# JuliaDiff/FiniteDiff.jl

Hardware: AMD Instinct MI355X
Metric: Jacobian columns/s (coloured sparse finite-difference Jacobian; headline config N=10^7 tridiagonal forward) (higher is better)
Workload: dtype f64; 1 GPU; N=10000000 tridiagonal CSC (nnz=3N-2), colorvec=mod1(i,3), forward, f!=second difference, x~U(0,1) seed 4; fdtype=forward, colors=3, parallelism=columns x1, output=nzval in HBM, eps_reduction=replicated, x_layout=replicated, gather_in_step=False

## Files before the change

### finitediff.jl_amd/csrc/fdjac_api.hip

```cpp
#include <algorithm>
#include <cmath>
#include <cstring>
#include <limits>
#include <new>

#include <atomic>
#include <thread>
#include <string>

#include "fdjac_internal.h"
#include "fdjac_eps_dev.h"

namespace fdjac {

#ifndef FDJAC_F32
static thread_local char g_err[512] = "";
#endif

int launch_eps(fd_plan *p, const real_t *x, double relstep, double absstep, double dir);
int launch_eps_groups(fd_plan *p, const real_t *x, int g0, int ng, bool final, double relstep, double absstep, double dir);
int launch_eps_final(fd_plan *p, double relstep, double absstep, double dir);
int launch_eps_flags(fd_plan *p, const real_t *x, const FusedEps &fz);
constexpr int kMaxEpsShards = kEpsGroups;
int launch_eps_perturb_small(fd_plan *p, const real_t *x, double relstep, double absstep, double dir, int pmode,
                             int base_row);
int launch_perturb(fd_plan *p, const real_t *x, int c_lo, int B);
int launch_decompress(fd_plan *p, const real_t *fx, int c_lo, int c_hi, real_t *const *outs, int mode);
int launch_fill(fd_ctx *ctx, real_t *ptr, int64_t n, real_t v);
int launch_scale(fd_ctx *ctx, real_t *dst, const real_t *src, int64_t n, real_t factor);
int launch_stream_copy(fd_ctx *ctx, const void *src, void *dst, int64_t n16);
int balanced_grid(int64_t tiles, int64_t cap);

static inline int64_t load_idx(const void *p, int bytes, int64_t i)
{
    return bytes == 8 ? ((const int64_t *)p)[i] : (int64_t)((const int32_t *)p)[i];
}

static inline int64_t round_up(int64_t v, int64_t m) { return (v + m - 1) / m * m; }

template <typename T> static int dev_upload(T **dst, const std::vector<T> &src)
{
    *dst = nullptr;
    if (src.empty()) return FD_OK;
    FD_HIP_CHECK(hipMalloc((void **)dst, sizeof(T) * src.size()));
    FD_HIP_CHECK(hipMemcpy(*dst, src.data(), sizeof(T) * src.size(), hipMemcpyHostToDevice));
    return FD_OK;
}

template <typename T> static int dev_alloc(T **dst, int64_t nelem)
{
    *dst = nullptr;
    if (nelem <= 0) nelem = 1;
    hipError_t e = hipMalloc((void **)dst, sizeof(T) * (size_t)nelem);
    if (e == hipErrorOutOfMemory) {
        set_error("hipMalloc of %lld bytes failed: out of memory", (long long)(nelem * (int64_t)sizeof(T)));
        return FD_ERR_NOMEM;
    }
    FD_HIP_CHECK(e);
    return FD_OK;
}

static int ingest_colors(fd_plan *p, const void *colorvec, int color_bytes, std::vector<int32_t> &col0)
{
    FD_REQUIRE(colorvec != nullptr, FD_ERR_ARG, "colorvec is NULL");
    FD_REQUIRE(color_bytes == 4 || color_bytes == 8, FD_ERR_ARG, "color_bytes must be 4 or 8");
    const int64_t N = p->N;
    col0.resize((size_t)N);
    int64_t C = 0;
    for (int64_t j = 0; j < N; ++j) {
        const int64_t c = load_idx(colorvec, color_bytes, j);
        if (c > C) C = c;
        FD_REQUIRE(c <= std::numeric_limits<int32_t>::max(), FD_ERR_ARG, "colour %lld too large", (long long)c);
        col0[(size_t)j] = c >= 1 ? (int32_t)(c - 1) : -1;
    }
    p->C = C;
    p->color8 = C <= 253;
    return FD_OK;
}

static int upload_colors(fd_plan *p, const std::vector<int32_t> &col0, const std::vector<int32_t> &nzc)
{
    if (p->color8) {
        std::vector<uint8_t> a(col0.size()), b(nzc.size());
        for (size_t i = 0; i < col0.size(); ++i) a[i] = col0[i] < 0 ? 0xFF : (uint8_t)col0[i];
        for (size_t i = 0; i < nzc.size(); ++i) b[i] = nzc[i] == -2 ? 0xFE : nzc[i] < 0 ? 0xFF : (uint8_t)nzc[i];
        uint8_t *d = nullptr;
        int rc = dev_upload(&d, a);
        if (rc) return rc;
        p->d_color = d;
        rc = dev_upload(&d, b);
        if (rc) return rc;
        p->d_nzcolor = d;
    } else {
        int32_t *d = nullptr;
        int rc = dev_upload(&d, col0);
        if (rc) return rc;
        p->d_color = d;
        rc = dev_upload(&d, nzc);
        if (rc) return rc;
        p->d_nzcolor = d;
    }
    return FD_OK;
}

static thread_local bool t_lowered_cx = false;
struct LoweredScope {
    LoweredScope() { t_lowered_cx = true; }
    ~LoweredScope() { t_lowered_cx = false; }
};
constexpr int32_t kPlanKnownFlags = FD_PLAN_EPS_CONTIGUOUS | FD_PLAN_COMPLEX_X | FD_PLAN_FINGERPRINT | FD_PLAN_STORE_CSC | FD_PLAN_STORE_CSC_ALWAYS | FD_PLAN_STORE_CSC_ROWS | FD_PLAN_HANDOVER_ROWS;

static int apply_opts(fd_plan *p, const fd_plan_opts *opts)
{
    FD_REQUIRE(opts != nullptr, FD_ERR_ARG, "opts is NULL");
    FD_REQUIRE(opts->fdtype == FD_FORWARD || opts->fdtype == FD_CENTRAL || opts->fdtype == FD_COMPLEX,
               FD_ERR_UNSUPPORTED,
               "Unrecognized fdtype: valid values are Val{:forward}, Val{:central} and Val{:complex}.");
    FD_REQUIRE((opts->flags & ~kPlanKnownFlags) == 0, FD_ERR_ARG, "unknown fd_plan_opts.flags bits 0x%x (zero the struct before filling it)",
               (unsigned)(opts->flags & ~kPlanKnownFlags));
    FD_REQUIRE(!(opts->flags & FD_PLAN_HANDOVER_ROWS) || (opts->flags & FD_PLAN_STORE_CSC_ROWS), FD_ERR_ARG,
               "fd_plan_opts.flags bits 0x%x: FD_PLAN_HANDOVER_ROWS needs FD_PLAN_STORE_CSC_ROWS (the row-wise hand-over kernel walks the plan's row lists)",
               (unsigned)opts->flags);
    FD_REQUIRE(!(opts->flags & FD_PLAN_COMPLEX_X), FD_ERR_UNSUPPORTED,
               "complex-valued x (FD_PLAN_COMPLEX_X) reaches this plan kind through its lowering only");
    p->fdtype = opts->fdtype;
    p->col0 = 0;
    p->col1 = p->N;
    if (!(opts->col_begin == 0 && opts->col_end == 0)) {
        FD_REQUIRE(opts->col_begin >= 0 && opts->col_begin <= opts->col_end && opts->col_end <= p->N, FD_ERR_ARG,
                   "column window [%lld,%lld) outside [0,%lld)", (long long)opts->col_begin,
                   (long long)opts->col_end, (long long)p->N);
        p->col0 = opts->col_begin;
        p->col1 = opts->col_end;
    }
    p->x0 = 0;
    p->x1 = p->N;
    if (!(opts->x_begin == 0 && opts->x_end == 0)) {
        FD_REQUIRE(opts->x_begin >= 0 && opts->x_begin <= opts->x_end && opts->x_end <= p->N, FD_ERR_ARG,
                   "x window [%lld,%lld) outside [0,%lld)", (long long)opts->x_begin, (long long)opts->x_end,
                   (long long)p->N);
        p->x0 = opts->x_begin;
        p->x1 = opts->x_end;
    }
    p->scratch_bytes = opts->scratch_bytes > 0 ? opts->scratch_bytes : ((int64_t)64 << 30);
    auto env_int = [](const char *name, int dflt) { const char *v = fdjac::test_switch(name); return (v && *v) ? atoi(v) : dflt; };
    p->small_ok = env_int("FDJAC_SMALL", 1) != 0;
    p->cx = t_lowered_cx;
    if (p->cx) p->small_ok = false;
    p->eps_nt = true;
    { const char *v = fdjac::test_switch("FDJAC_FUSED_MAX_N"); if (v && *v) p->fz_max_n = atoll(v); }
    p->fz_shared_ok = env_int("FDJAC_FUSED_SHARED", 0) != 0;
    p->fz_flags_ok = env_int("FDJAC_EPS_FLAGS", 1) != 0;
    p->lazy_diff = env_int("FDJAC_LAZY_DIFF", 1) != 0;
    p->bd_allowed = env_int("FDJAC_BAND_DESC", 1) != 0;
    p->store_allowed = env_int("FDJAC_LAZY_STORE", 1) != 0;
    p->want_store_csc = (opts->flags & FD_PLAN_STORE_CSC) != 0;
    p->want_store_rows = (opts->flags & FD_PLAN_STORE_CSC_ROWS) != 0;
    p->want_handover_rows = (opts->flags & FD_PLAN_HANDOVER_ROWS) != 0;
    p->store_csc_always = (opts->flags & FD_PLAN_STORE_CSC_ALWAYS) != 0;
    p->own_c0 = 0;
    p->own_c1 = -1;
    if (!(opts->color_begin == 0 && opts->color_end == 0)) {
        FD_REQUIRE(opts->color_begin >= 0 && opts->color_begin <= opts->color_end, FD_ERR_ARG,
                   "colour range [%lld,%lld) is not a range", (long long)opts->color_begin, (long long)opts->color_end);
        p->own_c0 = opts->color_begin;
        p->own_c1 = opts->color_end;
    }
    return FD_OK;
}

static int finish_fingerprint(int rc, fd_plan **out, const fd_plan_opts *opts, int idx_kind, const void *a, int64_t len_a, const void *b,
                              int64_t len_b, int idx_bytes, int idx_base, const void *colorvec, int color_bytes, int64_t len_color,
                              int memkind, int64_t N)
{
    if (rc || !opts || !(opts->flags & FD_PLAN_FINGERPRINT) || !out || !*out) return rc;
    fd_pattern_arrays src;
    memset(&src, 0, sizeof src);
    src.idx_a = a; src.len_a = len_a; src.idx_b = b; src.len_b = len_b; src.colorvec = colorvec; src.len_color = len_color;
    src.idx_bytes = idx_bytes ? idx_bytes : 8; src.idx_base = idx_base; src.color_bytes = color_bytes; src.memkind = memkind;
    const bool all = opts->col_begin == 0 && opts->col_end == 0;
    rc = plan_record_fingerprint(*out, idx_kind, &src, all ? 0 : opts->col_begin, all ? N : opts->col_end);
    if (rc) {
        fd_plan_destroy(*out);
        *out = nullptr;
    }
    return rc;
}

static int alloc_scratch(fd_plan *p, const std::vector<int32_t> &col0)
{
    p->cplx = p->fdtype == FD_COMPLEX ? 2 : 1;
    p->pts = p->fdtype == FD_CENTRAL ? 2 : 1;
    p->ldx = round_up(p->N, 32);
    p->ldf = round_up(p->M, 32);
    const int64_t per_color = (int64_t)p->pts * p->cplx * (int64_t)sizeof(real_t) * (p->ldx + p->ldf);
    int64_t B = p->C > 0 ? p->scratch_bytes / std::max<int64_t>(per_color, 1) : 1;
    B = std::max<int64_t>(1, std::min<int64_t>(B, std::max<int64_t>(p->C, 1)));
    B = std::min<int64_t>(B, 32768);
    p->chunkB = B;
    p->nchunks = p->C > 0 ? (p->C + B - 1) / B : 0;
    int rc;
    if ((rc = dev_alloc(&p->d_fx, p->ldf))) return rc;
    if ((rc = dev_alloc(&p->d_eps, std::max<int64_t>(p->C, 1)))) return rc;

    if (p->fdtype == FD_COMPLEX) {
        FD_HIP_CHECK(hipMemset(p->d_fx, 0, sizeof(real_t) * (size_t)p->ldf));
        p->d_zero = p->d_fx;
        FD_HIP_CHECK(hipStreamSynchronize(p->ctx->stream));
        int r2 = launch_fill(p->ctx, p->d_eps, std::max<int64_t>(p->C, 1), std::numeric_limits<real_t>::epsilon());
        if (r2) return r2;
    } else if (p->C > 0 && p->kind != K_DENSE) {
        if (p->C <= kRegColors) {
            if (!p->built_on_device) {
                const char *fc = fdjac::test_switch("FDJAC_EPS_CYCLIC");
                bool cyc = !(fc && *fc && atoi(fc) == 0) && p->N >= 1 && col0[0] >= 0;
                const int32_t sh = cyc ? col0[0] : 0;
                for (int64_t j = 0; j < p->N && cyc; ++j) cyc = col0[(size_t)j] == (int32_t)((j + sh) % p->C);
                p->cyc_C = cyc ? (int)p->C : 0;
                p->cyc_shift = cyc ? (int)sh : 0;
            }
            const int64_t tiles = (p->N + 2047) / 2048;
            const int64_t tpg = (tiles + kEpsGroups - 1) / kEpsGroups;
            const int64_t tpb = (tpg + kEpsBlocksPerGroup - 1) / kEpsBlocksPerGroup;
            FD_REQUIRE(tpg < ((int64_t)1 << 24), FD_ERR_UNSUPPORTED, "N too large for the step-size reduction's grid");
            p->eps_tpg = (int)tpg;
            p->eps_tpb = (int)tpb;
            p->eps_bpg = (int)((tpg + tpb - 1) / tpb);
            p->n_partial_blocks = kEpsGroups * p->eps_bpg;
            p->partial_cap = (int64_t)p->n_partial_blocks * kRegColors;
            if ((rc = dev_alloc(&p->d_partial, p->partial_cap))) return rc;
            if ((rc = dev_alloc(&p->d_gsum, (int64_t)2 * kEpsGroups * kRegColors))) return rc;
            if ((rc = dev_alloc(&p->d_tick, (int64_t)kEpsGroups + 1))) return rc;
            FD_HIP_CHECK(hipMemsetAsync(p->d_gsum, 0, sizeof(double) * 2 * kEpsGroups * kRegColors, p->ctx->stream));
            FD_HIP_CHECK(hipMemsetAsync(p->d_tick, 0, sizeof(unsigned) * (kEpsGroups + 1), p->ctx->stream));
        } else {
            std::vector<int64_t> cptr((size_t)p->C + 1, 0);
            for (int64_t j = 0; j < p->N; ++j)
                if (col0[(size_t)j] >= 0) cptr[(size_t)col0[(size_t)j] + 1]++;
            for (int64_t c = 0; c < p->C; ++c) cptr[(size_t)c + 1] += cptr[(size_t)c];
            std::vector<int32_t> perm((size_t)cptr[(size_t)p->C]);
            std::vector<int64_t> fillp(cptr.begin(), cptr.end() - 1);
            for (int64_t j = 0; j < p->N; ++j)
                if (col0[(size_t)j] >= 0) perm[(size_t)fillp[(size_t)col0[(size_t)j]]++] = (int32_t)j;
            if ((rc = dev_upload(&p->d_perm, perm))) return rc;
            if ((rc = dev_upload(&p->d_cptr, cptr))) return rc;
            int64_t chunks = (p->N / std::max<int64_t>(p->C, 1) + 511) / 512;
            p->seg_chunks = (int)std::max<int64_t>(1, std::min<int64_t>(chunks, 256));
            FD_REQUIRE((int64_t)p->C * p->seg_chunks < ((int64_t)1 << 31), FD_ERR_UNSUPPORTED, "too many colours");
            if ((rc = dev_alloc(&p->d_partial, (int64_t)p->seg_chunks * p->C))) return rc;
        }
    }
    return FD_OK;
}

static int ensure_values(fd_plan *p)
{
    if (p->d_FX) return FD_OK;
    return dev_alloc(&p->d_FX, (p->chunkB * p->pts + 1) * p->cplx * p->ldf);
}
static int ensure_points(fd_plan *p)
{
    if (p->d_X) return FD_OK;
    return dev_alloc(&p->d_X, (p->chunkB * p->pts + 1) * p->cplx * p->ldx);
}
static int ensure_stage(fd_plan *p, bool x, bool fin)
{
    int rc;
    if (x && !p->d_xstage && (rc = dev_alloc(&p->d_xstage, p->ldx))) return rc;
    if (fin && !p->d_finstage && (rc = dev_alloc(&p->d_finstage, p->ldf))) return rc;
    return FD_OK;
}

static int ensure_diff_scratch(fd_plan *p)
{
    int rc;
    if (!p->d_zero_own) {
        if ((rc = dev_alloc(&p->d_zero_own, p->ldf))) return rc;
        FD_HIP_CHECK(hipMemsetAsync(p->d_zero_own, 0, sizeof(real_t) * (size_t)p->ldf, p->ctx->stream));
        p->d_zero = p->d_zero_own;
    }
    if (p->fdtype == FD_CENTRAL && !p->d_eps2 && (rc = dev_alloc(&p->d_eps2, std::max<int64_t>(p->C, 1)))) return rc;
    return FD_OK;
}

static int new_plan(fd_ctx *ctx, int kind, int64_t M, int64_t N, fd_plan **out)
{
    FD_REQUIRE(ctx != nullptr && out != nullptr, FD_ERR_ARG, "ctx/out is NULL");
    FD_REQUIRE(M >= 0 && N >= 1, FD_ERR_SHAPE, "bad shape %lld x %lld", (long long)M, (long long)N);
    FD_REQUIRE(M < ((int64_t)1 << 31) && N < ((int64_t)1 << 31), FD_ERR_UNSUPPORTED,
               "dimensions >= 2^31 are not supported");
    FD_HIP_CHECK(hipSetDevice(ctx->device));
    fd_plan *p = new (std::nothrow) fd_plan();
    FD_REQUIRE(p != nullptr, FD_ERR_NOMEM, "out of host memory");
    p->ctx = ctx;
    p->kind = kind;
    p->M = M;
    p->N = N;
    *out = p;
    return FD_OK;
}

#define FD_TRY(expr)                 \
    do {                             \
        int _rc = (expr);            \
        if (_rc != FD_OK) {          \
// ... 24 lines not shown
int fd_ctx_create(int device, void *stream, fd_ctx **out)
{
    FD_REQUIRE(out != nullptr, FD_ERR_ARG, "out is NULL");
    *out = nullptr;
    int ndev = 0;
    hipError_t e = hipGetDeviceCount(&ndev);
    if (e != hipSuccess || ndev <= 0) {
        set_error("no HIP device available (%s)", e == hipSuccess ? "count = 0" : hipGetErrorString(e));
        return FD_ERR_NODEVICE;
    }
    FD_REQUIRE(device >= 0 && device < ndev, FD_ERR_ARG, "device %d out of range [0,%d)", device, ndev);
    FD_HIP_CHECK(hipSetDevice(device));
    hipDeviceProp_t prop;
    FD_HIP_CHECK(hipGetDeviceProperties(&prop, device));
    fd_ctx *c = new (std::nothrow) fd_ctx();
    FD_REQUIRE(c != nullptr, FD_ERR_NOMEM, "out of host memory");
    c->device = device;
    c->num_cus = prop.multiProcessorCount > 0 ? prop.multiProcessorCount : 256;
    if (stream == FD_STREAM_DEFAULT) {
        c->stream = nullptr;
        c->own_stream = false;
    } else if (stream) {
        c->stream = (hipStream_t)stream;
        c->own_stream = false;
    } else {
        hipError_t se = hipStreamCreateWithFlags(&c->stream, hipStreamNonBlocking);
        if (se != hipSuccess) {
            delete c;
            set_error("hipStreamCreate failed: %s", hipGetErrorString(se));
            return FD_ERR_HIP;
        }
        c->own_stream = true;
    }
    *out = c;
    return FD_OK;
}

int fd_ctx_destroy(fd_ctx *ctx)
{
    if (!ctx) return FD_OK;
    if (ctx->check_stream) { (void)hipStreamSynchronize(ctx->check_stream); (void)hipStreamDestroy(ctx->check_stream); }
    if (ctx->check_event) (void)hipEventDestroy(ctx->check_event);
    if (ctx->own_stream && ctx->stream) (void)hipStreamDestroy(ctx->stream);
    if (ctx->h_stale) (void)hipHostFree(ctx->h_stale);
    delete ctx;
    return FD_OK;
}

void *fd_ctx_stream(fd_ctx *ctx) { return ctx ? (void *)ctx->stream : nullptr; }

int fd_ctx_synchronize(fd_ctx *ctx)
{
    FD_REQUIRE(ctx != nullptr, FD_ERR_ARG, "ctx is NULL");
    FD_HIP_CHECK(hipStreamSynchronize(ctx->stream));
    if (ctx->check_stream) FD_HIP_CHECK(hipStreamSynchronize(ctx->check_stream));
    if (ctx->h_stale && *(volatile int *)ctx->h_stale) {
        *ctx->h_stale = 0;
        set_error("a deferred content check found that a plan no longer matches the caller's pattern / colour arrays (fd_plan_stale tells "
                  "which): results enqueued since that check are those of the old arrays");
        return FD_ERR_STALE;
    }
    return FD_OK;
}

#endif

int fd_plan_destroy(fd_plan *p)
{
    if (!p) return FD_OK;
    (void)hipSetDevice(p->ctx->device);
    (void)hipStreamSynchronize(p->ctx->stream);
    if (p->ctx->check_stream && p->d_fpx) (void)hipStreamSynchronize(p->ctx->check_stream);
    void *ptrs[] = {p->d_color, p->d_rowval, p->d_nzcolor, p->d_dest, p->d_spos, p->d_wtiles, p->d_wcode, p->d_w2desc, p->d_cr_rlo, p->d_cr_cnt, p->d_cr_off,
                    p->d_perm, p->d_cptr, p->d_X, p->d_FX, p->d_fx, p->d_eps, p->d_partial, p->d_gsum, p->d_tick, p->d_fpx, p->d_xstage,
                    p->d_finstage, p->d_outstage[0], p->d_outstage[1], p->d_outstage[2], p->d_zero_own, p->d_eps2, p->d_tile_order, p->d_fxwin, p->d_fp, p->d_sc_colptr, p->d_sc_rowval, p->d_sc_note, p->d_sr_ptr, p->d_sr_col, p->d_sr_slot, p->d_sr_order, p->d_sr_tile, p->d_sr_color, p->d_se_col, p->d_se_slot, p->d_se_info, p->d_split, p->d_bbb_off, p->d_bbb_blk, p->d_bbb_start, p->d_bbb_stride};
    for (void *q : ptrs)
        if (q) (void)hipFree(q);
    if (p->h_pstale) (void)hipHostFree(p->h_pstale);
    if (p->h_fz_err) (void)hipHostFree(p->h_fz_err);
    if (p->d_fz_part) (void)hipFree(p->d_fz_part);
    if (p->d_fz_eps) (void)hipFree(p->d_fz_eps);
    if (p->d_fz_trace) (void)hipFree(p->d_fz_trace);
    for (auto &sp : p->spans) {
        p->event_pool.push_back(sp.a);
        p->event_pool.push_back(sp.b);
    }
    for (hipEvent_t ev : p->event_pool) (void)hipEventDestroy(ev);
    delete p;
    return FD_OK;
}

#include "fdjac_plan_create.hip"

int fd_plan_row_lists(const fd_plan *p, const void **row_ptr_dev, const void **row_col_dev, const void **row_slot_dev, int64_t *entries, uint64_t *plan_serial)
{
    FD_REQUIRE(p != nullptr, FD_ERR_ARG, "plan is NULL");
    FD_REQUIRE(p->store_csc_ok && p->d_sr_ptr != nullptr, FD_ERR_UNSUPPORTED,
               "this plan keeps no row lists: create it with FD_PLAN_STORE_CSC | FD_PLAN_STORE_CSC_ROWS (a SparseMatrixCSC common-pattern plan that holds every column)");
    if (row_ptr_dev) *row_ptr_dev = p->d_sr_ptr;
    if (row_col_dev) *row_col_dev = p->d_sr_col;
    if (row_slot_dev) *row_slot_dev = p->d_sr_slot;
    if (entries) *entries = p->sc_entries;
    if (plan_serial) *plan_serial = p->sc_serial;
    return FD_OK;
}

int fd_plan_info(const fd_plan *p, int key, int64_t *value)
{
    FD_REQUIRE(p && value, FD_ERR_ARG, "NULL argument");
    switch (key) {
    case FD_INFO_M: *value = p->M; break;
    case FD_INFO_N: *value = p->N; break;
    case FD_INFO_NCOLORS: *value = p->C; break;
    case FD_INFO_NOUTS: *value = p->split_n ? p->split_n : p->nouts; break;
    case FD_INFO_OUT0_LEN: *value = p->split_n ? p->split_len[0] : p->out_len[0]; break;
    case FD_INFO_OUT1_LEN: *value = p->split_n ? p->split_len[1] : p->out_len[1]; break;
    case FD_INFO_OUT2_LEN: *value = p->split_n ? p->split_len[2] : p->out_len[2]; break;
    case FD_INFO_ROW_BEGIN: *value = p->row0; break;
    case FD_INFO_ROW_END: *value = p->row1; break;
    case FD_INFO_NCHUNKS: *value = p->nchunks; break;
    case FD_INFO_SCRATCH_BYTES:
        *value = (int64_t)sizeof(real_t) * (p->chunkB * p->pts * p->cplx * (p->ldx + p->ldf) + 2 * p->ldf + p->ldx);
        break;
    case FD_INFO_NNZ_LOCAL: *value = p->nnz_local; break;
    case FD_INFO_FCALLS_LAST: *value = p->fcalls_last; break;
    case FD_INFO_ENTRY_BEGIN: *value = p->entry_begin; break;
    case FD_INFO_SORTED_GATHER: *value = p->sorted_gather ? 1 : 0; break;
    case FD_INFO_LINES_DIRECT_X100: *value = (int64_t)(p->lines_direct * 100); break;
    case FD_INFO_LINES_SORTED_X100: *value = (int64_t)(p->lines_sorted * 100); break;
    case FD_INFO_WINDOW: *value = (p->window || p->tri_window) ? 1 : 0; break;
    case FD_INFO_WIN_OVERREAD_X100: *value = (int64_t)(p->win_overread * 100); break;
    case FD_INFO_WINDOW2D: *value = p->window2d ? 1 : 0; break;
    case FD_INFO_WIN_PERIOD: *value = p->win_per_P; break;
    case FD_INFO_COLRANGE_WG: *value = p->kind == K_COLRANGE ? 1 : 0; break;
    case FD_INFO_SMALL_FUSED:
        *value = (p->small_ok && p->N <= kSmallN && p->C > 0 && p->C <= kRegColors && p->kind != K_DENSE &&
                  p->fdtype != FD_COMPLEX) ? 1 : 0;
        break;
    case FD_INFO_EPS_CYCLIC: *value = p->cyc_C; break;
    case FD_INFO_EPS_NT: *value = !(store_active(p) || store_csc_active(p)) ? 1 : 0; break;
    case FD_INFO_BAND_DESC: *value = p->bd_t1 - p->bd_t0; break;
    case FD_INFO_LAZY_STORE:
        *value = (store_active(p) || store_csc_active(p)) ? 1 : 0;
        break;
    case FD_INFO_STORE_CSC:
        *value = p->store_csc_ok ? p->sc_entries : 0;
        break;
    case FD_INFO_STORE_LAUNCH: *value = p->store_launch; break;
    case FD_INFO_LAZY_DIFF:
        *value = (p->lazy_fn && (p->lazy_caps & FD_LAZY_CAP_DIFF) && p->lazy_diff && p->fdtype != FD_COMPLEX && p->kind != K_DENSE) ? 1 : 0;
        break;
    case FD_INFO_BUILT_ON_DEVICE: *value = p->built_on_device ? 1 : 0; break;
    case FD_INFO_HANDOVER_ROWS: *value = handover_rows_active(p) ? 1 : 0; break;
    default: set_error("unknown info key %d", key); return FD_ERR_ARG;
    }
    return FD_OK;
}

static hipEvent_t take_event(fd_plan *p)
{
    if (!p->event_pool.empty()) {
        hipEvent_t e = p->event_pool.back();
        p->event_pool.pop_back();
        return e;
    }
    hipEvent_t e = nullptr;
    (void)hipEventCreate(&e);
    return e;
}

struct Span {
    fd_plan *p;
    int idx = -1;
    Span(fd_plan *pl, int stage) : p(pl)
    {
        if (p->timing == 0) return;
        if (p->timing == 1 && stage != FD_STAGE_DECOMPRESS) return;
        if (p->timing == 1 && p->timing_stride > 1 && ((p->timing_calls - 1) % p->timing_stride) != 0) return;
        if (p->timing == 4 && stage == FD_STAGE_TOTAL) return;
        if (p->timing == 3 && stage != FD_STAGE_TOTAL) return;
        fdjac::TimedSpan s{stage, take_event(p), take_event(p)};
        (void)hipEventRecord(s.a, p->ctx->stream);
        p->spans.push_back(s);
        idx = (int)p->spans.size() - 1;
    }
    void stop()
    {
        if (idx >= 0) (void)hipEventRecord(p->spans[(size_t)idx].b, p->ctx->stream);
        idx = -1;
    }
    ~Span() { stop(); }
};

static constexpr size_t kMaxSpansInFlight = 4096;
static int collect_spans(fd_plan *p, bool blocking = true)
{
    if (p->spans.empty()) return FD_OK;
    if (!blocking && p->spans.size() >= kMaxSpansInFlight) blocking = true;
    if (blocking) FD_HIP_CHECK(hipStreamSynchronize(p->ctx->stream));
    size_t done = 0;
    for (auto &s : p->spans) {
        if (!blocking && hipEventQuery(s.b) != hipSuccess) {
            (void)hipGetLastError();
            break;
        }
        float ms = 0.f;
        if (hipEventElapsedTime(&ms, s.a, s.b) == hipSuccess) {
            p->ms_sum[s.stage] += ms;
            p->launches[s.stage] += 1;
            if (p->samples[s.stage].size() < 65536) p->samples[s.stage].push_back(ms);
        }
        p->event_pool.push_back(s.a);
        p->event_pool.push_back(s.b);
        ++done;
    }
    p->spans.erase(p->spans.begin(), p->spans.begin() + (ptrdiff_t)done);
    return FD_OK;
}

int fd_plan_enable_timing(fd_plan *p, int on)
{
    FD_REQUIRE(p, FD_ERR_ARG, "plan is NULL");
    int rc = collect_spans(p);
    if (rc) return rc;
    p->timing = on < 0 ? 0 : (on > 4 ? 4 : on);
    for (int i = 0; i < FD_NSTAGES; ++i) {
        p->ms_sum[i] = 0;
        p->launches[i] = 0;
        p->samples[i].clear();
    }
    return FD_OK;
}

int fd_plan_set_timing_stride(fd_plan *p, int stride)
{
    FD_REQUIRE(p && stride >= 1, FD_ERR_ARG, "bad argument");
    p->timing_stride = stride;
    p->timing_calls = 0;
    return FD_OK;
}

int fd_plan_get_timing_samples(fd_plan *p, int stage, double *ms_out, int64_t cap, int64_t *n_out)
{
    FD_REQUIRE(p && n_out && stage >= 0 && stage < FD_NSTAGES && (ms_out || cap == 0), FD_ERR_ARG, "bad argument");
    int rc = collect_spans(p);
    if (rc) return rc;
    const int64_t n = std::min<int64_t>((int64_t)p->samples[stage].size(), cap);
    for (int64_t k = 0; k < n; ++k) ms_out[k] = (double)p->samples[stage][(size_t)k];
    *n_out = (int64_t)p->samples[stage].size();
    return FD_OK;
}

int fd_plan_get_timings(fd_plan *p, double *ms_sum, int64_t *launches)
{
    FD_REQUIRE(p && ms_sum && launches, FD_ERR_ARG, "NULL argument");
    int rc = collect_spans(p);
    if (rc) return rc;
    for (int i = 0; i < FD_NSTAGES; ++i) {
        ms_sum[i] = p->ms_sum[i];
        launches[i] = p->launches[i];
    }
    return FD_OK;
}

static bool eps_shardable(const fd_plan *p)
{
    return p->fdtype != FD_COMPLEX && p->kind != K_DENSE && p->C > 0 && p->C <= kRegColors &&
           !(p->small_ok && p->N <= kSmallN) && p->d_partial != nullptr;
}

static void eps_shard_of(const fd_plan *p, int *W, int *r)
{
    if (p->p2p) { *W = fdjac_p2p_nranks(p->p2p); *r = fdjac_p2p_rank(p->p2p); }
    else { *W = fdjac_comm_nranks(p->comm); *r = fdjac_comm_rank(p->comm); }
}

static int eps_exchange(fd_plan *p, real_t *x_dev, int S, double relstep, double absstep, double dir)
{
    fd_p2p *mb = p->p2p ? p->p2p : (p->comm ? fdjac_comm_p2p(p->comm) : nullptr);
    if (mb && fdjac_p2p_nranks(mb) > 1) {
        fdjac_eps_final fin;
        fin.gsum = p->d_gsum; fin.ldp = kRegColors; fin.ngroups = kEpsGroups; fin.C = (int)p->C;
        fin.relstep = relstep; fin.absstep = absstep; fin.dir = dir; fin.is_forward = p->fdtype == FD_FORWARD ? 1 : 0;
        fin.eps = p->d_eps; fin.eps2 = p->d_eps2; fin.elem_bytes = (int)sizeof(real_t);
        const int rc = fdjac_p2p_step(mb, p->halo > 0 ? (void *)x_dev : nullptr, p->halo_own0, p->halo_own1, p->halo, (int)sizeof(real_t),
                                      p->d_gsum, (int64_t)S * kRegColors * (int64_t)sizeof(double), &fin);
        if (rc != FD_ERR_UNSUPPORTED) {
            if (!rc) p->eps2_fresh = p->d_eps2 != nullptr;
            return rc;
        }
    }
    int rc = FD_OK;
    if (p->comm) {
        if (p->halo > 0) rc = fd_comm_halo_exchange(p->comm, x_dev, p->halo_own0, p->halo_own1, p->halo, (int)sizeof(real_t));
        if (!rc) rc = fdjac_comm_allgather_f64(p->comm, p->d_gsum, (int64_t)S * kRegColors);
    }
    if (!rc) rc = launch_eps_final(p, relstep, absstep, dir);
    return rc;
}

static inline int call_f(const fd_plan *p, fd_f_launch f, void *fctx, void *fx, const void *x, int64_t nbatch, int64_t x_stride,
                         int64_t fx_stride, int64_t row_begin, int64_t row_end, int is_complex, void *stream)
{
    set_error("%s", "");
    if (!p->cx) return f(fctx, fx, x, nbatch, x_stride, fx_stride, row_begin, row_end, is_complex, stream);
    return f(fctx, fx, x, nbatch, x_stride / 2, fx_stride / 2, row_begin / 2, (row_end + 1) / 2, 1, stream);
}
#define FD_F_CHECK(rc)                                                                                                      \
    do {                                                                                                                    \
        if ((rc) != 0) {                                                                                                    \
            const std::string _why = fd_last_error();                                                                       \
            set_error("f! launcher returned %d%s%s", (int)(rc), _why.empty() ? "" : ": ", _why.c_str());                    \
            return FD_ERR_CALLBACK;                                                                                         \
        }                                                                                                                   \
    } while (0)

static int eps_sharded_classic(fd_plan *p, const real_t *x_dev, double relstep, double absstep, double dir)
{
    int W, r;
    eps_shard_of(p, &W, &r);
    const int S = (kEpsGroups + W - 1) / W;
    const int g0 = std::min(r * S, kEpsGroups), ng = std::min(S, kEpsGroups - g0);
    int rc = launch_eps_groups(p, x_dev, g0, ng, false, relstep, absstep, dir);
    if (!rc) {
        Span se(p, FD_STAGE_EXCHANGE);
        rc = eps_exchange(p, const_cast<real_t *>(x_dev), S, relstep, absstep, dir);
    }
    return rc;
}

static int fused_reset(fd_plan *p)
{
    const size_t np = 2 * (size_t)p->n_partial_blocks * kRegColors, ne = 2 * (size_t)kFzReplicas * kFzPitch;
    std::vector<unsigned long long> hp(np, kFzSentinel64);
    std::vector<rbits_t> he(ne, FzBits<real_t>::sentinel);
    FD_HIP_CHECK(hipStreamSynchronize(p->ctx->stream));
    FD_HIP_CHECK(hipMemcpy(p->d_fz_part, hp.data(), np * 8, hipMemcpyHostToDevice));
    FD_HIP_CHECK(hipMemcpy(p->d_fz_eps, he.data(), ne * sizeof(rbits_t), hipMemcpyHostToDevice));
    FD_HIP_CHECK(hipDeviceSynchronize());
    *p->h_fz_err = 0;
    p->fz_parity = 0;
    return FD_OK;
}
static int ensure_fused(fd_plan *p)
{
    if (p->d_fz_part) return FD_OK;
    FD_HIP_CHECK(hipHostMalloc((void **)&p->h_fz_err, sizeof(int), hipHostMallocMapped));
    *p->h_fz_err = 0;
    FD_HIP_CHECK(hipHostGetDevicePointer((void **)&p->d_fz_err, p->h_fz_err, 0));
    FD_HIP_CHECK(hipMalloc((void **)&p->d_fz_eps, 2 * (size_t)kFzReplicas * kFzPitch * sizeof(rbits_t)));
    FD_HIP_CHECK(hipMalloc((void **)&p->d_fz_part, 2 * (size_t)p->n_partial_blocks * kRegColors * sizeof(double)));
    { const char *v = fdjac::test_switch("FDJAC_FUSED_TRACE"); if (v && atoi(v) != 0) FD_HIP_CHECK(hipMalloc((void **)&p->d_fz_trace, 16 * sizeof(long long))); }
    return fused_reset(p);
}
static int64_t fused_timeout_ticks()
{
    const char *v = getenv("FDJAC_P2P_TIMEOUT_MS");
    const int64_t ms = (v && *v) ? atoll(v) : 2000;
    return (ms < 1 ? 1 : ms) * 100000;
}

static int jacobian_enqueue(fd_plan *p, fd_f_launch f, void *fctx, const real_t *x_dev, const real_t *fin_dev,
                            double relstep, double absstep, double dir, real_t *const *outs)
{
    fd_ctx *ctx = p->ctx;
    hipStream_t s = ctx->stream;
    FD_REQUIRE(f != nullptr, FD_ERR_ARG, "f launcher is NULL");
    if (!(relstep > 0)) {
        const real_t e = std::numeric_limits<real_t>::epsilon();
        relstep = p->fdtype == FD_FORWARD ? (double)std::sqrt(e) : p->fdtype == FD_CENTRAL ? (double)std::cbrt(e) : 1.0;
    }
    if (absstep < 0) absstep = relstep;
    p->relstep_last = relstep;
    p->absstep_last = absstep;
    p->fcalls_last = 0;
    if (collect_spans(p, false) != FD_OK) return FD_ERR_HIP;
    FD_REQUIRE(!(p->h_pstale && *(volatile int *)p->h_pstale), FD_ERR_STALE,
               "a deferred content check (fd_plan_matches_async) found that this plan no longer matches the caller's pattern / colour arrays");
    if (p->h_fz_err && *(volatile int *)p->h_fz_err) {
        const int what = *(volatile int *)p->h_fz_err;
        (void)fused_reset(p);
        FD_REQUIRE(false, FD_ERR_COMM, "the previous fused step of this plan timed out (%s never arrived; FDJAC_P2P_TIMEOUT_MS): its "
                   "output holds NaNs", what == 1 ? "a block sum of the step-size reduction" : "the step sizes");
    }
    {
        fd_p2p *mbq = p->p2p ? p->p2p : (p->comm ? fdjac_comm_p2p(p->comm) : nullptr);
        const int st = mbq ? fdjac_p2p_failed(mbq) : 0;
        FD_REQUIRE(st == 0, FD_ERR_COMM, "an earlier exchange through this plan's mailbox timed out (code %d: a peer's data never arrived; "
                   "fd_p2p_status / fd_comm_p2p_status; FDJAC_P2P_TIMEOUT_MS): step sizes and halo of that call are not to be trusted", st);
    }
    ++p->timing_calls;
    Span total(p, FD_STAGE_TOTAL);

    if (((uintptr_t)x_dev) & kPairMask) {
        { const int rc = ensure_stage(p, true, false); if (rc) return rc; }
        FD_HIP_CHECK(hipMemcpyAsync(p->d_xstage, x_dev, sizeof(real_t) * (size_t)p->N, hipMemcpyDeviceToDevice, s));
        x_dev = p->d_xstage;
    }

    const bool small_off = !p->small_ok;
    const bool full_colors = p->own_c0 == 0 && (p->own_c1 < 0 || p->own_c1 >= p->C);
    const bool small = !small_off && p->N <= kSmallN && p->C > 0 && p->C <= kRegColors && p->kind != K_DENSE &&
                       p->fdtype != FD_COMPLEX;
    const bool small_points = small && !p->lazy_fn && p->nchunks == 1 && full_colors;
    const bool base_in_batch = small_points && p->fdtype == FD_FORWARD && !fin_dev;
    p->fx_batch_row = nullptr;
    if (small_points) { int rc = ensure_points(p); if (!rc) rc = ensure_values(p); if (rc) return rc; }

    if (p->fdtype == FD_CENTRAL && p->lazy_fn && (p->lazy_caps & FD_LAZY_CAP_DIFF) && p->lazy_diff && p->kind != K_DENSE) {
        const int rc = ensure_diff_scratch(p);
        if (rc) return rc;
    }
    fd_p2p *fz_mb = p->p2p ? p->p2p : (p->comm ? fdjac_comm_p2p(p->comm) : nullptr);
    const bool shard_ctx = p->comm != nullptr || p->p2p != nullptr;
    bool fuse = !small && p->fdtype != FD_COMPLEX && p->C > 0 && p->C <= kRegColors && p->cyc_C > 0 && p->eps_mode == FD_EPS_COMPUTE &&
                p->lazy_fn && (p->lazy_caps & FD_LAZY_CAP_FUSED_EPS) && store_active(p) && p->store_ok &&
                (p->kind == K_CSC || p->kind == K_BANDED || p->kind == K_TRIDIAG) && p->nchunks == 1 && full_colors &&
                !(p->fdtype == FD_FORWARD && fin_dev) && p->d_partial != nullptr;
    if (shard_ctx && p->halo > 0) {
        int W = 1, r = 0;
        eps_shard_of(p, &W, &r);
        FD_REQUIRE(r == 0 || p->halo_own0 >= p->halo, FD_ERR_ARG, "no room for the lower halo: x[%lld - %lld, ...) starts before 0", (long long)p->halo_own0, (long long)p->halo);
        FD_REQUIRE(r + 1 >= W || p->halo_own1 + p->halo <= p->N, FD_ERR_ARG, "no room for the upper halo: x[..., %lld + %lld) ends behind N = %lld",
                   (long long)p->halo_own1, (long long)p->halo, (long long)p->N);
    }
    if (fuse) {
        hipStreamCaptureStatus cs = hipStreamCaptureStatusNone;
        if (hipStreamIsCapturing(s, &cs) != hipSuccess) { (void)hipGetLastError(); cs = hipStreamCaptureStatusNone; }
        if (cs != hipStreamCaptureStatusNone) fuse = false;
    }
    bool fuse_sharded = false;
    int fzW = 1, fzr = 0;
    if (fuse && shard_ctx) {
        if (fz_mb) { fzW = fdjac_p2p_nranks(fz_mb); fzr = fdjac_p2p_rank(fz_mb); }
        const bool halo_ok = p->halo == 0 || (p->halo == 2 && p->halo_own0 == p->col0 && p->halo_own1 == p->col1 && p->halo_own0 % 4 == 0 &&
                                              (p->halo_own1 % 4 == 0 || fzr == fzW - 1));
        fuse = fuse_sharded = fz_mb != nullptr && fzW > 1 && p->fz_sharded_ok && eps_shardable(p) && halo_ok &&
                              (int64_t)((kEpsGroups + fzW - 1) / fzW) * p->eps_tpg * 2048 <= p->fz_max_n &&
                              (!fdjac_p2p_shared_device(fz_mb) || p->fz_shared_ok);
    } else if (fuse) {
        fuse = p->N <= p->fz_max_n;
    }
    bool eps_flags = !fuse && p->fz_flags_ok && !small && !shard_ctx && p->fdtype != FD_COMPLEX && p->C > 0 && p->C <= kRegColors &&
                     p->kind != K_DENSE && p->eps_mode == FD_EPS_COMPUTE && p->d_partial != nullptr &&
                     p->n_partial_blocks == kEpsGroups * p->eps_bpg && p->n_partial_blocks <= kFzMaxBlocks;
    if (eps_flags) {
        hipStreamCaptureStatus cs = hipStreamCaptureStatusNone;
        if (hipStreamIsCapturing(s, &cs) != hipSuccess) { (void)hipGetLastError(); cs = hipStreamCaptureStatusNone; }
        if (cs != hipStreamCaptureStatusNone) eps_flags = false;
    }
    FusedEps fz_job;
    if (fuse || eps_flags) {
        const int rc = ensure_fused(p);
        if (rc) return rc;
        memset(&fz_job, 0, sizeof fz_job);
        fz_job.eg.tpg = p->eps_tpg; fz_job.eg.bpg = p->eps_bpg; fz_job.eg.tpb = p->eps_tpb; fz_job.eg.final_groups = kEpsGroups;
        fz_job.eg.C = (int)p->C; fz_job.eg.is_forward = p->fdtype == FD_FORWARD ? 1 : 0;
        fz_job.eg.relstep = relstep; fz_job.eg.absstep = absstep; fz_job.eg.dir = dir;
        fz_job.nranks = 1; fz_job.rank = 0; fz_job.g0 = 0; fz_job.ng = kEpsGroups;
        if (fuse_sharded) {
            const int S = (kEpsGroups + fzW - 1) / fzW;
            fz_job.nranks = fzW; fz_job.rank = fzr;
            fz_job.g0 = std::min(fzr * S, kEpsGroups); fz_job.ng = std::min(S, kEpsGroups - fz_job.g0);
            fdjac_p2p_fused mbv;
            const int rm = fdjac_p2p_fused_begin(fz_mb, &mbv);
            if (rm) return rm;
            fz_job.peer = mbv.peer; fz_job.local = mbv.local; fz_job.fz_off = mbv.fz_off; fz_job.buf = mbv.buf; fz_job.buf_reset = mbv.buf_reset;
            if (p->halo > 0) { fz_job.xw = const_cast<real_t *>(x_dev); fz_job.own_begin = p->halo_own0; fz_job.own_end = p->halo_own1; fz_job.halo = (int)p->halo; }
        }
        fz_job.nblocks = fz_job.ng * p->eps_bpg;
        fz_job.cyc_C = p->cyc_C; fz_job.cyc_shift = p->cyc_shift; fz_job.pair = p->cx ? 1 : 0;
        const size_t hp = (size_t)p->n_partial_blocks * kRegColors, he = (size_t)kFzReplicas * kFzPitch;
        fz_job.part = p->d_fz_part + (p->fz_parity ? hp : 0);
        fz_job.part_next = p->d_fz_part + (p->fz_parity ? 0 : hp);
        fz_job.epsr = (rbits_t *)p->d_fz_eps + (p->fz_parity ? he : 0);
        fz_job.epsr_next = (rbits_t *)p->d_fz_eps + (p->fz_parity ? 0 : he);
        fz_job.eps = p->d_eps; fz_job.eps2 = p->d_eps2;
        fz_job.err = fuse_sharded ? fdjac_p2p_err_word(fz_mb) : p->d_fz_err;
        fz_job.timeout_ticks = fused_timeout_ticks();
        fz_job.trace = p->d_fz_trace;
        if (p->d_fz_trace) {
            static const long long init[16] = {-1, 0, 0, 0, 0, -1, -1, 0, 0, 0, 0, 0, 0, 0, 0, 0};
            FD_HIP_CHECK(hipMemcpyAsync(p->d_fz_trace, init, sizeof init, hipMemcpyHostToDevice, s));
        }
    }
    if (p->eps_mode != FD_EPS_PRECOMPUTED) p->eps2_fresh = false;
    p->eps_nt = !(store_active(p) || store_csc_active(p));
    if (p->fdtype != FD_COMPLEX && p->C > 0 && p->eps_mode == FD_EPS_PRECOMPUTED) {
        FD_REQUIRE(!small_points, FD_ERR_UNSUPPORTED, "FD_EPS_PRECOMPUTED needs a plan whose reduction can be sharded");
    } else if (fuse) {
    } else if (eps_flags) {
        Span sp(p, FD_STAGE_EPS);
        const int rc = launch_eps_flags(p, x_dev, fz_job);
        if (rc) return rc;
        p->fz_parity ^= 1u;
    } else if (p->fdtype != FD_COMPLEX && p->C > 0) {
        Span sp(p, FD_STAGE_EPS);
        int rc;
        if (small) {
            rc = launch_eps_perturb_small(p, x_dev, relstep, absstep, dir, small_points ? p->fdtype : -1,
                                          base_in_batch ? (int)(p->C * p->pts) : -1);
        } else if ((p->comm || p->p2p) && eps_shardable(p)) {
            rc = eps_sharded_classic(p, x_dev, relstep, absstep, dir);
        } else {
            rc = launch_eps(p, x_dev, relstep, absstep, dir);
        }
        if (rc) return rc;
    }

    const real_t *fx = nullptr;
    bool base_pending = false;
    if (p->fdtype == FD_FORWARD) {
        if (fin_dev) {
            fx = fin_dev;
        } else if (base_in_batch) {
            fx = p->fx_batch_row = p->d_FX + (int64_t)p->C * p->pts * p->ldf;
        } else if (p->lazy_fn && p->nchunks > 0) {
            base_pending = true;
            fx = p->d_fx;
        } else {
            Span sp(p, FD_STAGE_F);
            const int rc = call_f(p, f, fctx, p->d_fx, x_dev, 1, p->N, p->ldf, p->row0, p->row1, 0, (void *)s);
            FD_F_CHECK(rc);
            p->fcalls_last += 1;
            fx = p->d_fx;
        }
    }

    if (p->kind == K_CSC_DENSE || p->kind == K_COO_DENSE || (p->kind == K_BBB && p->bbb_fill)) {
        FD_HIP_CHECK(hipMemsetAsync(outs[0], 0, sizeof(real_t) * (size_t)p->out_len[0], s));
    } else if (p->C == 0) {
        for (int k = 0; k < p->nouts; ++k)
            FD_HIP_CHECK(hipMemsetAsync(outs[k], 0, sizeof(real_t) * (size_t)p->out_len[k], s));
    }

    const int64_t oc0 = std::min<int64_t>(p->own_c0, p->C), oc1 = p->own_c1 < 0 ? p->C : std::min<int64_t>(p->own_c1, p->C);
    bool diff_base_counted = false;
    for (int64_t cl = oc0; cl < oc1; cl += p->chunkB) {
        const int c_lo = (int)cl;
        const int c_hi = (int)std::min<int64_t>(oc1, cl + p->chunkB);
        const int B = c_hi - c_lo;
        bool lazy_done = false, imag_only = false;
        bool want_diff = p->lazy_fn && (p->lazy_caps & FD_LAZY_CAP_DIFF) && p->lazy_diff && p->fdtype != FD_COMPLEX &&
                               !(p->fdtype == FD_FORWARD && !base_pending) && p->kind != K_DENSE;
        if (want_diff) { const int rc = ensure_diff_scratch(p); if (rc) return rc; }
        if (p->kind == K_BBB && store_active(p) && !(p->fdtype == FD_FORWARD && !base_pending)) {
            Span sp(p, FD_STAGE_DECOMPRESS);
            fd_bbb_store bb;
            memset(&bb, 0, sizeof bb);
            bb.out = outs[0]; bb.N = p->N; bb.nblk = p->bbb_nb; bb.block_size = p->bbb_bs;
            bb.bl = p->bbb_bl; bb.bu = p->bbb_bu; bb.lam = p->bbb_lam; bb.mu = p->bbb_mu;
            bb.start = (const long long *)p->d_bbb_start; bb.stride = (const long long *)p->d_bbb_stride;
            bb.color = p->d_color; bb.color_bytes = p->color8 ? 1 : 4; bb.C = (int)p->C; bb.elem_bytes = (int)sizeof(real_t);
            fd_lazy_points lp = {};
            lp.x = x_dev; lp.color = p->d_color; lp.eps = p->d_eps; lp.color_bytes = bb.color_bytes;
            lp.c_lo = c_lo; lp.ncolors = B; lp.pts = p->pts; lp.nparts = 1;
            lp.diff = (p->fdtype == FD_FORWARD && !diff_base_counted) ? 2 : 1;
            lp.store = &bb; lp.store_kind = FD_STORE_BBB;
            const int rc = p->lazy_fn(fctx, p->d_FX, &lp, p->ldf, p->row0, p->row1, (void *)s);
            FD_REQUIRE(rc == 0 || rc == FD_LAZY_DECLINED, FD_ERR_CALLBACK, "lazy f! launcher (BBB store) returned %d", rc);
            if (rc == 0) {
                p->fcalls_last += (int64_t)B * p->pts + (lp.diff == 2 ? 1 : 0);
                diff_base_counted = true;
                continue;
            }
        } else if (store_active(p) && !(p->fdtype == FD_FORWARD && !base_pending)) {
            Span sp(p, FD_STAGE_DECOMPRESS);
            fd_band_store bs;
            fd_stencil5_store s5;
            memset(&bs, 0, sizeof bs);
            memset(&s5, 0, sizeof s5);
            s5.out = outs[0];
            s5.nx = p->store5_nx; s5.ny = p->store5_ny; s5.entry_begin = p->entry_begin; s5.col_begin = p->col0; s5.col_end = p->col1;
            s5.color = p->d_color; s5.color_bytes = p->color8 ? 1 : 4; s5.C = (int)p->C; s5.elem_bytes = (int)sizeof(real_t);
            const bool stencil = !p->store_ok && p->store5_ok && p->kind == K_CSC;
            fd_colrange_store scr;
            memset(&scr, 0, sizeof scr);
            if (p->kind == K_COLRANGE) {
                scr.out = outs[0]; scr.M = p->M; scr.N = p->N; scr.col_begin = p->col0; scr.col_end = p->col1;
                scr.row_first = p->d_cr_rlo; scr.row_count = p->d_cr_cnt; scr.dest = (const long long *)p->d_cr_off;
                scr.color = p->d_color; scr.color_bytes = p->color8 ? 1 : 4; scr.C = (int)p->C; scr.elem_bytes = (int)sizeof(real_t);
                scr.pairs = p->cr_pairs ? 1 : 0; scr.nblk = p->cr_nblk; scr.block_size = p->cr_bs; scr.bl = p->cr_bl; scr.bu = p->cr_bu;
            }
            bs.M = p->M; bs.N = p->N; bs.entry_begin = p->entry_begin; bs.col_begin = p->col0; bs.col_end = p->col1;
            bs.l = p->store_l; bs.u = p->store_u; bs.C = p->store_C; bs.shift = p->store_shift;
            bs.elem_bytes = (int)sizeof(real_t);
            if (p->kind == K_TRIDIAG) {
                bs.layout = FD_BAND_TRIDIAGONAL;
                bs.out_dl = outs[0]; bs.out = outs[1]; bs.out_du = outs[2];
            } else {
                bs.layout = p->kind == K_BANDED ? FD_BAND_BANDED : FD_BAND_CSC;
                bs.out = outs[0];
            }
            fd_lazy_points lp = {};
            lp.x = x_dev;
            lp.color = p->d_color;
            lp.eps = p->d_eps;
            lp.color_bytes = p->color8 ? 1 : 4;
            lp.c_lo = c_lo;
            lp.ncolors = B;
            lp.pts = p->pts;
            lp.nparts = 1;
            lp.diff = p->fdtype == FD_COMPLEX ? 0 : ((p->fdtype == FD_FORWARD && !diff_base_counted) ? 2 : 1);
            lp.store = p->kind == K_COLRANGE ? (const void *)&scr : stencil ? (const void *)&s5 : (const void *)&bs;
            lp.store_kind = p->kind == K_COLRANGE ? FD_STORE_COLRANGE : stencil ? FD_STORE_STENCIL5 : FD_STORE_BAND;
            lp.is_complex = p->fdtype == FD_COMPLEX ? 1 : 0;
            lp.imag_only = lp.is_complex;
            lp.eps_job = fuse ? &fz_job : nullptr;
            int rc = p->lazy_fn(fctx, p->d_FX, &lp, p->ldf, p->row0, p->row1, (void *)s);
            if (fuse && rc == 0) {
                if (fuse_sharded) fdjac_p2p_fused_commit(fz_mb);
                p->fz_parity ^= 1u;
                p->eps2_fresh = p->d_eps2 != nullptr;
            } else if (fuse) {
                fuse = false;
                sp.stop();
                { Span se(p, FD_STAGE_EPS); const int re = fuse_sharded ? eps_sharded_classic(p, x_dev, relstep, absstep, dir) : launch_eps(p, x_dev, relstep, absstep, dir); if (re) return re; }
                Span sp2(p, FD_STAGE_DECOMPRESS);
                lp.eps_job = nullptr;
                if (rc == FD_LAZY_DECLINED) rc = p->lazy_fn(fctx, p->d_FX, &lp, p->ldf, p->row0, p->row1, (void *)s);
            }
            FD_REQUIRE(rc == 0 || rc == FD_LAZY_DECLINED, FD_ERR_CALLBACK, "lazy f! launcher (store) returned %d", rc);
            if (rc == 0) {
                p->fcalls_last += (int64_t)B * p->pts + (lp.diff == 2 ? 1 : 0);
                diff_base_counted = true;
                continue;
            }
        }
        if (store_csc_active(p)) {
            const bool own_base = base_pending && (p->lazy_caps & FD_LAZY_CAP_STORE_CSC_BASE) != 0;
            if (base_pending && !own_base) {
                Span sp(p, FD_STAGE_F);
                const int rc = call_f(p, f, fctx, p->d_fx, x_dev, 1, p->N, p->ldf, p->row0, p->row1, 0, (void *)s);
                FD_F_CHECK(rc);
                p->fcalls_last += 1;
                base_pending = false;
            }
            Span sp(p, FD_STAGE_DECOMPRESS);
            fd_csc_store sc;
            memset(&sc, 0, sizeof sc);
            sc.out = outs[0]; sc.M = p->M; sc.N = p->N; sc.col_begin = p->col0; sc.col_end = p->col1;
            sc.colptr = p->d_sc_colptr; sc.rowval = p->d_sc_rowval; sc.note = p->d_sc_note; sc.color = p->d_color; sc.fx_base = (p->fdtype == FD_FORWARD && !own_base) ? fx : nullptr;
            sc.color_bytes = p->color8 ? 1 : 4; sc.C = (int)p->C; sc.elem_bytes = (int)sizeof(real_t); sc.valid_coloring = p->sc_valid ? 1 : 0; sc.reach = p->sc_reach; sc.plan_serial = p->sc_serial;
            sc.row_ptr = p->d_sr_ptr; sc.row_col = p->d_sr_col; sc.row_slot = p->d_sr_slot; sc.row_pack = p->d_sr_order; sc.row_tile = p->d_sr_tile; sc.ent_col = p->d_se_col; sc.ent_slot = p->d_se_slot; sc.ent_info = p->d_se_info; sc.ent_tile_max = p->se_tile_max;
            fd_lazy_points lp = {};
            lp.x = x_dev;
            lp.color = p->d_color;
            lp.eps = p->d_eps;
            lp.color_bytes = sc.color_bytes;
            lp.c_lo = c_lo;
            lp.ncolors = B;
            lp.pts = p->pts;
            lp.nparts = 1;
            lp.diff = p->fdtype == FD_COMPLEX ? 0 : 1;
            lp.is_complex = p->fdtype == FD_COMPLEX ? 1 : 0;
            lp.imag_only = lp.is_complex;
            lp.store = &sc;
            lp.store_kind = FD_STORE_CSC;
            store_launch_note() = FD_STORE_LAUNCH_NONE;
            const int rc = p->lazy_fn(fctx, p->d_FX, &lp, p->ldf, p->row0, p->row1, (void *)s);
            FD_REQUIRE(rc == 0 || rc == FD_LAZY_DECLINED, FD_ERR_CALLBACK, "lazy f! launcher (column store) returned %d", rc);
            p->store_launch = rc == 0 ? store_launch_note() : FD_STORE_LAUNCH_NONE;
            if (rc == 0) {
                p->fcalls_last += (int64_t)B * p->pts + ((own_base && !diff_base_counted) ? 1 : 0);
                if (own_base) diff_base_counted = true;
                continue;
            }
            if (p->fdtype == FD_FORWARD && !own_base) want_diff = false;
        }
        if (fuse) {
            fuse = false;
            Span se(p, FD_STAGE_EPS);
            const int re = fuse_sharded ? eps_sharded_classic(p, x_dev, relstep, absstep, dir) : launch_eps(p, x_dev, relstep, absstep, dir);
            if (re) return re;
        }
        { const int rc = ensure_values(p); if (rc) return rc; }
        bool diff_done = false;
        if (p->lazy_fn) {
            Span sp(p, FD_STAGE_F);
            fd_lazy_points lp = {};
            lp.x = x_dev;
            lp.color = p->d_color;
            lp.eps = p->d_eps;
            lp.base_out = (base_pending && !want_diff) ? p->d_fx : nullptr;
            lp.diff = want_diff ? ((p->fdtype == FD_FORWARD && !diff_base_counted) ? 2 : 1) : 0;
            lp.store_kind = 0;
            lp.color_bytes = p->color8 ? 1 : 4;
            lp.c_lo = c_lo;
            lp.ncolors = B;
            lp.pts = p->pts;
            lp.is_complex = p->fdtype == FD_COMPLEX ? 1 : 0;
            lp.imag_only = (p->fdtype == FD_COMPLEX && (p->lazy_caps & FD_LAZY_CAP_IMAG_ONLY)) ? 1 : 0;
            lp.part = 0;
            lp.nparts = 1;
            imag_only = lp.imag_only != 0;
            const int rc = p->lazy_fn(fctx, p->d_FX, &lp, p->ldf, p->row0, p->row1, (void *)s);
            FD_REQUIRE(rc == 0 || rc == FD_LAZY_DECLINED, FD_ERR_CALLBACK, "lazy f! launcher returned %d", rc);
            if (rc == 0 && want_diff) {
                lazy_done = diff_done = true;
                p->fcalls_last += (int64_t)B * p->pts + (lp.diff == 2 ? 1 : 0);
                diff_base_counted = true;
            } else if (rc == 0) {
                lazy_done = true;
                p->fcalls_last += (int64_t)B * p->pts + (base_pending ? 1 : 0);
                base_pending = false;
            }
        }
        if (!lazy_done) {
            if (base_pending) {
                Span sp(p, FD_STAGE_F);
                const int rc = call_f(p, f, fctx, p->d_fx, x_dev, 1, p->N, p->ldf, p->row0, p->row1, 0, (void *)s);
                FD_F_CHECK(rc);
                p->fcalls_last += 1;
                base_pending = false;
            }
            { const int rc = ensure_points(p); if (rc) return rc; }
            if (!small_points) {
                Span sp(p, FD_STAGE_PERTURB);
                int rc = launch_perturb(p, x_dev, c_lo, B);
                if (rc) return rc;
            }
            Span sp(p, FD_STAGE_F);
            const int64_t npts = (int64_t)B * p->pts + (base_in_batch ? 1 : 0);
            const int rc = call_f(p, f, fctx, p->d_FX, p->d_X, npts, p->ldx, p->ldf, p->row0, p->row1,
                             p->fdtype == FD_COMPLEX ? 1 : 0, (void *)s);
            FD_F_CHECK(rc);
            p->fcalls_last += npts;
        }
        {
            Span sp(p, FD_STAGE_DECOMPRESS);
            const bool io = lazy_done && imag_only;
            int rc;
            if (diff_done) {
                real_t *eps_plain = p->d_eps;
                if (p->fdtype == FD_CENTRAL) {
                    if (!p->eps2_fresh && (rc = launch_scale(p->ctx, p->d_eps2 + c_lo, p->d_eps + c_lo, B, (real_t)2))) return rc;
                    p->d_eps = p->d_eps2;
                }
                rc = launch_decompress(p, p->d_zero, c_lo, c_hi, outs, (int)FD_FORWARD);
                p->d_eps = eps_plain;
            } else {
                rc = launch_decompress(p, io ? p->d_fx : fx, c_lo, c_hi, outs, io ? (int)FD_FORWARD : p->fdtype);
            }
            if (rc) return rc;
        }
    }
    return FD_OK;
}

static int jacobian_split(fd_plan *p, bool async, fd_f_launch f, void *fctx, const void *x, int x_kind, const void *f_in, int f_in_kind, double relstep,
                          double absstep, double dir, void *const *outs, int out_kind)
{
    for (int k = 0; k < p->split_n; ++k) FD_REQUIRE(outs[k] || p->split_len[k] == 0, FD_ERR_ARG, "outs[%d] is NULL", k);
    FD_HIP_CHECK(hipSetDevice(p->ctx->device));
    if (!p->d_split) { const int rc = dev_alloc(&p->d_split, p->out_len[0]); if (rc) return rc; }
    void *one[3] = {p->d_split, nullptr, nullptr};
    const int n = p->split_n;
    p->split_n = 0;
    const int rc = async ? fd_jacobian_async(p, f, fctx, x, f_in, relstep, absstep, dir, one)
                         : fd_jacobian(p, f, fctx, x, x_kind, f_in, f_in_kind, relstep, absstep, dir, one, FD_DEVICE);
    p->split_n = n;
    if (rc) return rc;
    int64_t off = 0;
    for (int k = 0; k < n; ++k) {
        if (p->split_len[k] > 0)
            FD_HIP_CHECK(hipMemcpyAsync(outs[k], p->d_split + off, sizeof(real_t) * (size_t)p->split_len[k],
                                        out_kind == FD_HOST ? hipMemcpyDeviceToHost : hipMemcpyDeviceToDevice, p->ctx->stream));
        off += p->split_len[k];
// ... 325 lines not shown
```

### finitediff.jl_amd/csrc/fdjac_eps_dev.h

```cpp
#pragma once
#include "fdjac_internal.h"
#include "fdjac_dotx.h"

namespace fdjac {

template <typename CT> __device__ __forceinline__ void load_color_pair(const CT *p, int &c0, int &c1);
template <> __device__ __forceinline__ void load_color_pair<uint8_t>(const uint8_t *p, int &c0, int &c1)
{
    const unsigned v = *reinterpret_cast<const uint16_t *>(p);
    c0 = (int)(v & 0xFF);
    c1 = (int)(v >> 8);
}
template <> __device__ __forceinline__ void load_color_pair<int32_t>(const int32_t *p, int &c0, int &c1)
{
    const int2 v = *reinterpret_cast<const int2 *>(p);
    c0 = v.x;
    c1 = v.y;
}

template <typename CT, bool CYC>
__device__ __forceinline__ int eps_color_of(const CT *__restrict__ color, int64_t i, int cyc_C, int cyc_shift, int pair)
{
    if (pair) i &= ~(int64_t)1;
    return CYC ? (int)((i + cyc_shift) % cyc_C) : (int)color[i];
}

template <typename CT, bool CYC>
__device__ __noinline__ double eps_rescan_norm_wave(const real_t *__restrict__ x, const CT *__restrict__ color, int64_t n, int cyc_C,
                                                       int cyc_shift, int pair, int cc, int k)
{
    const double sc = k < 0 ? 0x1p-600 : 0x1p600, unsc = k < 0 ? 0x1p600 : 0x1p-600;
    double acc = 0.0;
    for (int64_t i = threadIdx.x & 63; i < n; i += 64)
        if (eps_color_of<CT, CYC>(color, i, cyc_C, cyc_shift, pair) == cc) {
            const double v = (double)x[i] * sc;
            acc += v * v;
        }
    acc = wave_sum(acc);
    return sqrt(__shfl(acc, 0, 64)) * unsc;
}

constexpr int kEpsU = 4;

struct EpsGrid {
    int tpg, bpg, tpb;
    int final_groups;
    int C, is_forward;
    double relstep, absstep, dir;
};

template <typename CT, int NC, bool CYC, bool NT, bool PIPE = true>
__device__ __forceinline__ bool eps_block_sum(const real_t *__restrict__ x, const CT *__restrict__ color, int64_t n, int cyc_C, int cyc_shift,
                                              int gblock, const EpsGrid &eg, int pair, double (*red)[NC], double &s)
{
    const int grp = gblock / eg.bpg, kb = gblock - grp * eg.bpg;
    double acc[NC];
#pragma unroll
    for (int c = 0; c < NC; ++c) acc[c] = 0.0;

    const int64_t tile = (int64_t)kEpsU * kBlock * 2;
    const int64_t t0 = (int64_t)grp * eg.tpg + (int64_t)kb * eg.tpb;
    int64_t t1 = t0 + eg.tpb;
    if (t1 > (int64_t)(grp + 1) * eg.tpg) t1 = (int64_t)(grp + 1) * eg.tpg;
    const int64_t base0 = t0 * tile;
    int64_t base_end = t1 * tile;
    if (base_end > n) base_end = n;
    int rc = 0, du = 0;
    if (CYC) {
        rc = (int)((base0 + threadIdx.x * 2 + cyc_shift) % cyc_C);
        du = (kBlock * 2) % cyc_C;
    }
    auto load_tile = [&](int64_t base, r2_t (&v)[kEpsU], int (&c0)[kEpsU], int (&c1)[kEpsU]) {
        if (base + tile <= n) {
#pragma unroll
            for (int u = 0; u < kEpsU; ++u) {
                const int64_t i = base + (int64_t)u * kBlock * 2 + threadIdx.x * 2;
                if (CYC) {
                    c0[u] = rc;
                    c1[u] = rc + 1 == cyc_C ? 0 : rc + 1;
                    rc += du;
                    rc = rc >= cyc_C ? rc - cyc_C : rc;
                }
                const r2_t *pv = reinterpret_cast<const r2_t *>(x + i);
                v[u] = NT ? __builtin_nontemporal_load(pv) : *pv;
                if (!CYC) load_color_pair<CT>(color + i, c0[u], c1[u]);
            }
            return;
        }
#pragma unroll
        for (int u = 0; u < kEpsU; ++u) {
            const int64_t i = base + (int64_t)u * kBlock * 2 + threadIdx.x * 2;
            if (CYC) {
                c0[u] = rc;
                c1[u] = rc + 1 == cyc_C ? 0 : rc + 1;
                rc += du;
                rc = rc >= cyc_C ? rc - cyc_C : rc;
            }
            if (i + 1 < n) {
                if (NT) v[u] = __builtin_nontemporal_load(reinterpret_cast<const r2_t *>(x + i));
                else v[u] = *reinterpret_cast<const r2_t *>(x + i);
                if (!CYC) load_color_pair<CT>(color + i, c0[u], c1[u]);
            } else if (i < n) {
                v[u] = r2_t{x[i], 0.0};
                if (!CYC) c0[u] = color[i];
                c1[u] = -2;
            } else {
                v[u] = r2_t{0.0, 0.0};
                c0[u] = c1[u] = -2;
            }
        }
    };
    r2_t va[kEpsU], vb[kEpsU];
    int a0[kEpsU], a1[kEpsU], b0[kEpsU], b1[kEpsU];
    auto accumulate = [&](const r2_t (&v)[kEpsU], int (&c0)[kEpsU], int (&c1)[kEpsU]) {
#pragma unroll
        for (int u = 0; u < kEpsU; ++u) {
            if (pair) c1[u] = c0[u];
            const double s0 = (double)v[u].x * (double)v[u].x, s1 = (double)v[u].y * (double)v[u].y;
#pragma unroll
            for (int c = 0; c < NC; ++c) {
                acc[c] += (c0[u] == c) ? s0 : 0.0;
                acc[c] += (c1[u] == c) ? s1 : 0.0;
            }
        }
    };
    if (!PIPE) {
        for (int64_t base = base0; base < base_end; base += tile) {
            load_tile(base, va, a0, a1);
            accumulate(va, a0, a1);
        }
    } else {
    if (base0 < base_end) load_tile(base0, va, a0, a1);
    for (int64_t base = base0; base < base_end; base += 2 * tile) {
        const bool more1 = base + tile < base_end;
        if (more1) load_tile(base + tile, vb, b0, b1);
        accumulate(va, a0, a1);
        if (!more1) break;
        if (base + 2 * tile < base_end) load_tile(base + 2 * tile, va, a0, a1);
        accumulate(vb, b0, b1);
    }
    }

    const int lane = threadIdx.x & 63, wave = threadIdx.x >> 6;
#pragma unroll
    for (int c = 0; c < NC; ++c) {
        const double w = wave_sum(acc[c]);
        if (lane == 0) red[wave][c] = w;
    }
    __syncthreads();
    if (wave != 0) return false;
    s = 0.0;
    if (lane < NC) {
#pragma unroll
        for (int w = 0; w < kBlock / 64; ++w) s += red[w][lane];
    }
    return true;
}

constexpr int kFzReplicas = 64;
constexpr int kFzPitch = 32;

template <typename T> struct FzBits;
template <> struct FzBits<double> {
    typedef unsigned long long u_t;
    static constexpr u_t sentinel = kFzSentinel64, halo_sentinel = kFzSentinelHalo64;
};
template <> struct FzBits<float> {
    typedef unsigned u_t;
    static constexpr u_t sentinel = kFzSentinel32, halo_sentinel = kFzSentinel32;
};
typedef FzBits<real_t>::u_t rbits_t;
__device__ __forceinline__ real_t fz_from_bits(rbits_t b)
{
    real_t r;
    __builtin_memcpy(&r, &b, sizeof r);
    return r;
}
__device__ __forceinline__ rbits_t fz_to_bits(real_t r)
{
    rbits_t b;
    __builtin_memcpy(&b, &r, sizeof r);
    return b;
}

struct FusedEps {
    EpsGrid eg;
    int nblocks;
    int cyc_C, cyc_shift, pair;
    double *part, *part_next;
    rbits_t *epsr, *epsr_next;
    real_t *eps, *eps2;
    int *err;
    long long timeout_ticks;
    long long *trace;
    int nranks, rank, g0, ng;
    char *const *peer;
    char *local;
    long long fz_off;
    int buf, buf_reset;
    real_t *xw;
    long long own_begin, own_end;
    int halo;
};
__device__ __forceinline__ char *fz_cells(char *mailbox, const FusedEps &fz, int buf) { return mailbox + fz.fz_off + (long long)buf * kFzBufBytes; }
__device__ __forceinline__ void fz_mark_min(const FusedEps &fz, int k)
{
    if (fz.trace && (threadIdx.x & 63) == 0 && ((blockIdx.x & 31) < 2 || blockIdx.x < kRegColors)) atomicMin((unsigned long long *)fz.trace + k, (unsigned long long)wall_clock64());
}
__device__ __forceinline__ void fz_mark_max(const FusedEps &fz, int k)
{
    if (fz.trace && (threadIdx.x & 63) == 0 && ((blockIdx.x & 31) < 2 || blockIdx.x < kRegColors)) atomicMax((unsigned long long *)fz.trace + k, (unsigned long long)wall_clock64());
}

__device__ __forceinline__ void fz_load8_agent(const unsigned long long *const (&p)[8], unsigned long long *v)
{
    asm volatile("global_load_dwordx2 %0, %8, off sc1\n\t"
                 "global_load_dwordx2 %1, %9, off sc1\n\t"
                 "global_load_dwordx2 %2, %10, off sc1\n\t"
                 "global_load_dwordx2 %3, %11, off sc1\n\t"
                 "global_load_dwordx2 %4, %12, off sc1\n\t"
                 "global_load_dwordx2 %5, %13, off sc1\n\t"
                 "global_load_dwordx2 %6, %14, off sc1\n\t"
                 "global_load_dwordx2 %7, %15, off sc1\n\t"
                 "s_waitcnt vmcnt(0)"
                 : "=&v"(v[0]), "=&v"(v[1]), "=&v"(v[2]), "=&v"(v[3]), "=&v"(v[4]), "=&v"(v[5]), "=&v"(v[6]), "=&v"(v[7])
                 : "v"(p[0]), "v"(p[1]), "v"(p[2]), "v"(p[3]), "v"(p[4]), "v"(p[5]), "v"(p[6]), "v"(p[7])
                 : "memory");
}

template <int NC, bool PIPE, typename CT = uint8_t, bool CYC = true, bool NT = false>
__device__ __forceinline__ void fused_eps_block(const real_t *__restrict__ x, int64_t n, const FusedEps &fz, int gblock, double (*red)[NC],
                                                const CT *__restrict__ color = nullptr)
{
    double s;
    if (threadIdx.x == 0) fz_mark_min(fz, 0);
    if (!eps_block_sum<CT, NC, CYC, NT, PIPE>(x, color, n, fz.cyc_C, fz.cyc_shift, fz.g0 * fz.eg.bpg + gblock, fz.eg, fz.pair, red, s)) return;
    const int lane = threadIdx.x & 63;
    if (lane < fz.eg.C) __hip_atomic_store(fz.part + (int64_t)lane * fz.nblocks + gblock, s, __ATOMIC_RELAXED, __HIP_MEMORY_SCOPE_AGENT);
    fz_mark_max(fz, 1);
}

constexpr int kFzMaxBlocks = kEpsGroups * kEpsBlocksPerGroup;
template <typename CT = uint8_t, bool CYC = true>
__device__ __forceinline__ void fused_finisher(const FusedEps &fz, int c, double *lds, const real_t *__restrict__ x, int64_t n,
                                               const CT *__restrict__ color = nullptr)
{
    const int t = threadIdx.x, lane = t & 63, wave = t >> 6, nb = fz.nblocks, bpg = fz.eg.bpg;
    const bool sharded = fz.nranks > 1;
    double *gs_peer = lds + kFzMaxBlocks;
    int *s_bad = reinterpret_cast<int *>(gs_peer + kEpsGroups);
    if (t == 0) *s_bad = 0;
    double gs = 0.0;
    int ok = 1;
    const long long t0 = wall_clock64();
    if (wave == 0) {
        const unsigned long long *src = reinterpret_cast<const unsigned long long *>(fz.part + (int64_t)c * nb);
        if (t == 0) fz_mark_max(fz, 2);
        const unsigned long long my_peer = (sharded && lane < fz.nranks) ? (unsigned long long)fz.peer[lane] : 0ull;
        for (int m0 = 0; m0 * 64 < nb; m0 += 8) {
            unsigned long long v[8];
            const unsigned long long *q[8];
#pragma unroll
            for (int u = 0; u < 8; ++u) q[u] = src + ((lane + 64 * (m0 + u) < nb) ? lane + 64 * (m0 + u) : 0);
            for (;;) {
                fz_load8_agent(q, v);
                bool all = true;
#pragma unroll
                for (int u = 0; u < 8; ++u) all = all && v[u] != kFzSentinel64;
                if (__all(all)) break;
                if (wall_clock64() - t0 > fz.timeout_ticks) { ok = 0; break; }
                __builtin_amdgcn_s_sleep(1);
            }
#pragma unroll
            for (int u = 0; u < 8; ++u)
                if (lane + 64 * (m0 + u) < nb) lds[lane + 64 * (m0 + u)] = __longlong_as_double((long long)v[u]);
        }
        __builtin_amdgcn_wave_barrier();
        if (t == 0) fz_mark_max(fz, 3);
        {
            const bool own = lane >= fz.g0 && lane < fz.g0 + fz.ng;
#pragma unroll
            for (int k0 = 0; k0 < kEpsBlocksPerGroup; k0 += 8) {
                double w[8];
#pragma unroll
                for (int k = 0; k < 8; ++k) w[k] = (own && k0 + k < bpg) ? lds[(lane - fz.g0) * bpg + k0 + k] : 0.0;
#pragma unroll
                for (int k = 0; k < 8; ++k) gs += w[k];
            }
            if (sharded)
                for (int b = 0; b < fz.nranks; ++b) {
                    char *pb = reinterpret_cast<char *>(__shfl((unsigned long long)my_peer, b, 64));
                    if (own && b != fz.rank)
                        __hip_atomic_store(reinterpret_cast<double *>(fz_cells(pb, fz, fz.buf)) + c * kEpsGroups + lane, gs, __ATOMIC_RELAXED,
                                           __HIP_MEMORY_SCOPE_SYSTEM);
                }
        }
    } else if (wave == 1) {
        if (sharded) {
            const bool own = lane >= fz.g0 && lane < fz.g0 + fz.ng;
            const unsigned long long *cell = reinterpret_cast<const unsigned long long *>(fz_cells(fz.local, fz, fz.buf)) + c * kEpsGroups + lane;
            unsigned long long w = 0;
            for (;;) {
                w = __hip_atomic_load(cell, __ATOMIC_RELAXED, __HIP_MEMORY_SCOPE_SYSTEM);
                if (__all(own || w != kFzSentinel64)) break;
                if (wall_clock64() - t0 > fz.timeout_ticks) { ok = 0; break; }
                __builtin_amdgcn_s_sleep(1);
            }
            gs_peer[lane] = __longlong_as_double((long long)w);
        }
    } else {
        const int u = t - 128;
        if (sharded && c == 0 && fz.xw && u < 2 * fz.halo) {
            const int h = u % fz.halo, up = u / fz.halo;
            const int target = up ? fz.rank + 1 : fz.rank - 1;
            if (target >= 0 && target < fz.nranks) {
                const real_t v = up ? fz.xw[fz.own_end - fz.halo + h] : fz.xw[fz.own_begin + h];
                rbits_t *cell = reinterpret_cast<rbits_t *>(fz_cells(fz.peer[target], fz, fz.buf) + kFzGsumBytes + (up ? 0 : kFzHaloBytes)) + h;
                __hip_atomic_store(cell, fz_to_bits(v), __ATOMIC_RELAXED, __HIP_MEMORY_SCOPE_SYSTEM);
            }
        }
        unsigned long long *pn = reinterpret_cast<unsigned long long *>(fz.part_next + (int64_t)c * nb);
        for (int i = u; i < nb; i += 128) __hip_atomic_store(pn + i, kFzSentinel64, __ATOMIC_RELAXED, __HIP_MEMORY_SCOPE_AGENT);
        if (u < kFzReplicas) __hip_atomic_store(fz.epsr_next + u * kFzPitch + c, FzBits<real_t>::sentinel, __ATOMIC_RELAXED, __HIP_MEMORY_SCOPE_AGENT);
        if (sharded && fz.buf_reset >= 0) {
            unsigned long long *cells = reinterpret_cast<unsigned long long *>(fz_cells(fz.local, fz, fz.buf_reset));
            if (u < kEpsGroups) __hip_atomic_store(cells + c * kEpsGroups + u, kFzSentinel64, __ATOMIC_RELAXED, __HIP_MEMORY_SCOPE_SYSTEM);
            if (c == 0 && u >= 64 && u < 64 + (int)(2 * kFzHaloBytes / 8))
                __hip_atomic_store(cells + kFzGsumBytes / 8 + (u - 64), kFzSentinelHalo64, __ATOMIC_RELAXED, __HIP_MEMORY_SCOPE_SYSTEM);
        }
    }
    if (!ok) *s_bad = 1;
    asm volatile("s_waitcnt lgkmcnt(0)\n\ts_barrier" ::: "memory");
    if (wave != 0) return;
    const bool bad = *s_bad != 0;
    if (!(lane >= fz.g0 && lane < fz.g0 + fz.ng)) gs = gs_peer[lane];
    gs_peer[lane] = gs;
    __builtin_amdgcn_wave_barrier();
    double tot = 0.0;
#pragma unroll
    for (int k0 = 0; k0 < kEpsGroups; k0 += 16) {
        double w[16];
#pragma unroll
        for (int k = 0; k < 16; ++k) w[k] = gs_peer[k0 + k];
#pragma unroll
        for (int k = 0; k < 16; ++k) tot += w[k];
    }
    double nrm = sqrt(tot);
    const int k = sharded || bad ? 0 : eps_rescale_exp(tot, fz.eg.relstep, fz.eg.absstep);
    if (k != 0) nrm = eps_rescan_norm_wave<CT, CYC>(x, color, n, fz.cyc_C, fz.cyc_shift, fz.pair, c, k);
    real_t e = eps_rule_norm<real_t>(nrm, fz.eg.relstep, fz.eg.absstep, fz.eg.dir, fz.eg.is_forward);
    if (bad || fz_to_bits(e) == FzBits<real_t>::sentinel) e = fz_from_bits(FzBits<real_t>::sentinel ^ 1);
    __hip_atomic_store(fz.epsr + lane * kFzPitch + c, fz_to_bits(e), __ATOMIC_RELAXED, __HIP_MEMORY_SCOPE_AGENT);
    if (t == 0) {
        if (bad) __hip_atomic_store(fz.err, 1, __ATOMIC_RELAXED, __HIP_MEMORY_SCOPE_SYSTEM);
        fz.eps[c] = e;
        if (fz.eps2) fz.eps2[c] = (real_t)2 * e;
        fz_mark_max(fz, 4);
    }
}

__device__ __forceinline__ real_t fused_halo(const FusedEps &fz, int which, int h)
{
    const rbits_t *cell = reinterpret_cast<const rbits_t *>(fz_cells(fz.local, fz, fz.buf) + kFzGsumBytes + (which ? kFzHaloBytes : 0)) + h;
    const long long t0 = wall_clock64();
    rbits_t b;
    for (;;) {
        b = __hip_atomic_load(cell, __ATOMIC_RELAXED, __HIP_MEMORY_SCOPE_SYSTEM);
        if (b != FzBits<real_t>::halo_sentinel) break;
        if (wall_clock64() - t0 > fz.timeout_ticks) {
            __hip_atomic_store(fz.err, 3, __ATOMIC_RELAXED, __HIP_MEMORY_SCOPE_SYSTEM);
            b = FzBits<real_t>::sentinel ^ 1;
            break;
        }
        __builtin_amdgcn_s_sleep(1);
    }
    const real_t v = fz_from_bits(b);
    fz.xw[which ? fz.own_end + h : fz.own_begin - fz.halo + h] = v;
    return v;
}

__device__ __forceinline__ void fused_wait_eps(const FusedEps &fz, int wg_id, real_t *s_eps)
{
    const int lane = threadIdx.x & 63;
    const rbits_t *E = fz.epsr + (wg_id & (kFzReplicas - 1)) * kFzPitch;
    const int c = lane < fz.eg.C ? lane : 0;
    long long t0 = 0;
    rbits_t b = 0;
    fz_mark_min(fz, 5);
    fz_mark_max(fz, 9);
    for (int spin = 0;; ++spin) {
        b = __hip_atomic_load(E + c, __ATOMIC_RELAXED, __HIP_MEMORY_SCOPE_AGENT);
        if (__all(b != FzBits<real_t>::sentinel)) break;
// ... 15 lines not shown
```

### finitediff.jl_amd/csrc/fdjac_f_tridiag.hip

```cpp

template <typename T, bool NL> __device__ __forceinline__ T tridiag_row(T xm, T xi, T xp)
{
    T v = (xm - kTwo * xi) + xp;
    if (NL) v = v + (xi * xi) * xp;
    return v;
}

template <typename CT, int MODE, bool NL>
__global__ void __launch_bounds__(kBlock)
k_f_tridiag_lazy(real_t *__restrict__ fx, int64_t fs, real_t *__restrict__ base_out, const real_t *__restrict__ x,
                 const CT *__restrict__ color, const real_t *__restrict__ eps, int c_lo, int B, int64_t n, int64_t r0,
                 int64_t r1, int imag_only, int diff)
{
    const int64_t stride = (int64_t)gridDim.x * kBlock * 2;
    for (int64_t i = r0 + ((int64_t)blockIdx.x * kBlock + threadIdx.x) * 2; i < r1; i += stride) {
        real_t xv[4];
        int cv[4];
#pragma unroll
        for (int k = 0; k < 4; ++k) {
            const int64_t j = i - 1 + k;
            const bool in = (j >= 0) & (j < n);
            xv[k] = in ? x[in ? j : 0] : 0.0;
            const int c = in ? (int)color[in ? j : 0] : -1;
            cv[k] = (c == (int)(CT)(-1) || c < 0) ? -1 : c - c_lo;
        }
        const bool two = i + 1 < n;
        real_t b0 = 0.0, b1 = 0.0;
        if (base_out || (diff && MODE == 0)) {
            b0 = tridiag_row<real_t, NL>(xv[0], xv[1], xv[2]);
            if (two) b1 = tridiag_row<real_t, NL>(xv[1], xv[2], xv[3]);
        }
        if (base_out) {
            if (two) *reinterpret_cast<r2_t *>(base_out + i) = r2_t{b0, b1};
            else base_out[i] = b0;
        }
        for (int b = 0; b < B; ++b) {
            const real_t e = eps[c_lo + b];
            real_t d[4];
#pragma unroll
            for (int k = 0; k < 4; ++k) d[k] = (cv[k] == b) ? e : 0.0;
            if (MODE == 2) {
                cd p[4];
#pragma unroll
                for (int k = 0; k < 4; ++k) p[k] = cd{xv[k], d[k]};
                const cd v0 = tridiag_row<cd, NL>(p[0], p[1], p[2]);
                if (imag_only) {
                    real_t *dst = fx + (int64_t)b * fs + i;
                    if (two) {
                        const cd v1 = tridiag_row<cd, NL>(p[1], p[2], p[3]);
                        *reinterpret_cast<r2_t *>(dst) = r2_t{v0.im, v1.im};
                    } else {
                        dst[0] = v0.im;
                    }
                } else {
                    real_t *dst = fx + ((int64_t)b * fs + i) * 2;
                    *reinterpret_cast<r2_t *>(dst) = r2_t{v0.re, v0.im};
                    if (two) {
                        const cd v1 = tridiag_row<cd, NL>(p[1], p[2], p[3]);
                        *reinterpret_cast<r2_t *>(dst + 2) = r2_t{v1.re, v1.im};
                    }
                }
            } else if (diff) {
                real_t p[4], q[4];
#pragma unroll
                for (int k = 0; k < 4; ++k) { p[k] = xv[k] + d[k]; q[k] = xv[k] - d[k]; }
                const real_t s0 = MODE == 1 ? tridiag_row<real_t, NL>(q[0], q[1], q[2]) : b0;
                const real_t v0 = sub_exact(tridiag_row<real_t, NL>(p[0], p[1], p[2]), s0);
                real_t v1 = 0.0;
                if (two) {
                    const real_t s1 = MODE == 1 ? tridiag_row<real_t, NL>(q[1], q[2], q[3]) : b1;
                    v1 = sub_exact(tridiag_row<real_t, NL>(p[1], p[2], p[3]), s1);
                }
                real_t *dst = fx + (int64_t)b * fs + i;
                if (two) *reinterpret_cast<r2_t *>(dst) = r2_t{v0, v1};
                else dst[0] = v0;
            } else {
#pragma unroll
                for (int sgn = 0; sgn < (MODE == 1 ? 2 : 1); ++sgn) {
                    real_t p[4];
#pragma unroll
                    for (int k = 0; k < 4; ++k) p[k] = sgn == 0 ? xv[k] + d[k] : xv[k] - d[k];
                    const real_t v0 = tridiag_row<real_t, NL>(p[0], p[1], p[2]);
                    real_t *dst = fx + (int64_t)(sgn * B + b) * fs + i;
                    if (two) {
                        const real_t v1 = tridiag_row<real_t, NL>(p[1], p[2], p[3]);
                        *reinterpret_cast<r2_t *>(dst) = r2_t{v0, v1};
                    } else {
                        dst[0] = v0;
                    }
                }
            }
        }
    }
}

__device__ __forceinline__ r2_t ld_pair_guarded(const real_t *__restrict__ x, int64_t a, int64_t n)
{
    if (a >= 0 && a + 1 < n) return *reinterpret_cast<const r2_t *>(x + a);
    r2_t v = {0, 0};
    if (a >= 0 && a < n) v.x = x[a];
    return v;
}

template <int MODE, bool NL>
__device__ __forceinline__ real_t tridiag_quotient(const real_t *xv, real_t e, int k)
{
    const real_t ed = MODE == 1 ? 2 * e : e;
    real_t p[3], m[3];
#pragma unroll
    for (int i = 0; i < 3; ++i) { const real_t dlt = k + i == 2 ? e : (real_t)0; p[i] = xv[k + i] + dlt; m[i] = xv[k + i] - dlt; }
    const real_t plus = tridiag_row<real_t, NL>(p[0], p[1], p[2]);
    const real_t sub = MODE == 1 ? tridiag_row<real_t, NL>(m[0], m[1], m[2]) : tridiag_row<real_t, NL>(xv[k], xv[k + 1], xv[k + 2]);
    return sub_exact(plus, sub) / ed;
}

template <int MODE, bool NL>
__device__ __forceinline__ void tridiag_pair_quotients(const r2_t &L, const r2_t &Cc, const r2_t &R, real_t ea, real_t eb, real_t (&q)[6])
{
    const real_t xv[6] = {L.x, L.y, Cc.x, Cc.y, R.x, R.y};
#pragma unroll
    for (int o = 0; o < 2; ++o)
#pragma unroll
        for (int k = 0; k < 3; ++k) q[3 * o + k] = tridiag_quotient<MODE, NL>(xv + o, o == 0 ? ea : eb, k);
}
template <int MODE, bool NL>
__device__ __forceinline__ real_t tridiag_next_quotient(const r2_t &Cc, const r2_t &R, real_t en)
{
    const real_t xv[3] = {Cc.x, Cc.y, R.x};
    return tridiag_quotient<MODE, NL>(xv, en, 0);
}

__device__ __forceinline__ int tridiag_wave_color(int64_t jw, const fd_band_store &bst)
{
    const int64_t m = (jw + bst.shift) % bst.C;
    return (int)(m < 0 ? m + bst.C : m);
}

template <int MODE, bool NL>
__global__ void __launch_bounds__(kBlock)
k_f_tridiag_store_wave(const real_t *__restrict__ x, const real_t *__restrict__ eps, int64_t n, fd_band_store bst, int64_t jstart, int lines)
{
    __shared__ __attribute__((aligned(16))) real_t s_win[kBlock / 64][FD_BAND_WAVE_LDS(3)];
    const int lane = threadIdx.x & 63, wave = threadIdx.x >> 6;
    const int64_t nwaves = (bst.col_end - jstart + 127) / 128;
    const int64_t gw = (int64_t)blockIdx.x * (kBlock / 64) + wave;
    if (gw >= nwaves) return;
    const int64_t jw = jstart + gw * 128;
    const int64_t j = jw + 2 * lane;
    const r2_t Cc = ld_pair_guarded(x, j, n), L = ld_pair_guarded(x, j - 2, n), R = ld_pair_guarded(x, j + 2, n);
    const int c0w = tridiag_wave_color(jw, bst);
    const int c0 = (int)((uint32_t)(c0w + 2 * lane) % (uint32_t)bst.C);
    const int c1 = c0 + 1 == bst.C ? 0 : c0 + 1;
    const real_t ea = eps[c0], eb = eps[c1];
    const real_t en = lines ? eps[(uint32_t)(c0w + 128) % (uint32_t)bst.C] : (real_t)0;
    real_t q[6];
    tridiag_pair_quotients<MODE, NL>(L, Cc, R, ea, eb, q);
    if (lines) {
        real_t qn = 0;
        if (lane == 63) qn = tridiag_next_quotient<MODE, NL>(Cc, R, en);
        fd_band_emit_wave_lines<real_t, true>(&bst, s_win[wave], jw, q, qn);
        return;
    }
    fd_band_emit_wave<real_t, 3, true>(&bst, s_win[wave], jw, q);
}

template <int MODE, bool NL, int NC, bool PIPE>
__global__ void __launch_bounds__(kBlock)
k_f_tridiag_fused(const real_t *__restrict__ x, int64_t n, fd_band_store bst, int64_t jstart, int lines, FusedEps fz)
{
    constexpr int kWinBytes = (kBlock / 64) * FD_BAND_WAVE_LDS(3) * (int)sizeof(real_t);
    constexpr int kLdsBytes = kWinBytes + 64 > (kFzMaxBlocks + 2 * kEpsGroups) * 8 ? kWinBytes + 64 : (kFzMaxBlocks + 2 * kEpsGroups) * 8;
    __shared__ __attribute__((aligned(16))) char s_lds[kLdsBytes];
    real_t (*s_win)[FD_BAND_WAVE_LDS(3)] = reinterpret_cast<real_t (*)[FD_BAND_WAVE_LDS(3)]>(s_lds);
    double *s_red = reinterpret_cast<double *>(s_lds);
    const int b = (int)blockIdx.x, nfin = fz.eg.C;
    if (b < nfin) { fused_finisher(fz, b, s_red, x, n); return; }
    if (b < nfin + fz.nblocks) { fused_eps_block<NC, PIPE>(x, n, fz, b - nfin, reinterpret_cast<double (*)[NC]>(s_red)); return; }
    const int lane = threadIdx.x & 63, wave = threadIdx.x >> 6;
    const int cb = b - nfin - fz.nblocks;
    const int64_t nwaves = (bst.col_end - jstart + 127) / 128;
    const int64_t gstride = (int64_t)((int)gridDim.x - nfin - fz.nblocks) * (kBlock / 64);
    int64_t gw = (int64_t)cb * (kBlock / 64) + wave;
    int64_t jw = jstart + gw * 128;
    r2_t Cc = {0, 0}, L = {0, 0}, R = {0, 0};
    auto load_x = [&](int64_t jt, r2_t &c_, r2_t &l_, r2_t &r_) {
        const int64_t j = jt + 2 * lane;
        c_ = ld_pair_guarded(x, j, n); l_ = ld_pair_guarded(x, j - 2, n); r_ = ld_pair_guarded(x, j + 2, n);
        if (fz.xw && fz.nranks > 1) {
            if (j == fz.own_begin && fz.rank > 0) { l_.x = fused_halo(fz, 0, 0); l_.y = fused_halo(fz, 0, 1); }
            if (j + 2 == fz.own_end && fz.rank + 1 < fz.nranks) { r_.x = fused_halo(fz, 1, 0); r_.y = fused_halo(fz, 1, 1); }
        }
    };
    if (gw < nwaves) load_x(jw, Cc, L, R);
    real_t *s_eps = reinterpret_cast<real_t *>(s_lds + kWinBytes);
    if (wave == 0) fused_wait_eps(fz, cb, s_eps);
    __syncthreads();
    for (; gw < nwaves; gw += gstride) {
        const int c0w = tridiag_wave_color(jw, bst);
        const int c0 = (int)((uint32_t)(c0w + 2 * lane) % (uint32_t)bst.C);
        const int c1 = c0 + 1 == bst.C ? 0 : c0 + 1;
        real_t q[6];
        tridiag_pair_quotients<MODE, NL>(L, Cc, R, s_eps[c0], s_eps[c1], q);
        if (lines) {
            real_t qn = 0;
            if (lane == 63) qn = tridiag_next_quotient<MODE, NL>(Cc, R, s_eps[(uint32_t)(c0w + 128) % (uint32_t)bst.C]);
            fd_band_emit_wave_lines<real_t, true>(&bst, s_win[wave], jw, q, qn);
        } else {
            fd_band_emit_wave<real_t, 3, true>(&bst, s_win[wave], jw, q);
        }
        jw = jstart + (gw + gstride) * 128;
        if (gw + gstride < nwaves) load_x(jw, Cc, L, R);
    }
    if (fz.trace && (blockIdx.x & 31) < 2) { asm volatile("s_waitcnt vmcnt(0)" ::: "memory"); fz_mark_max(fz, 8); }
}

#ifdef FDJAC_F32
typedef real_t r4_t __attribute__((ext_vector_type(4)));
__device__ __forceinline__ r4_t ld_quad_guarded(const real_t *__restrict__ x, int64_t a, int64_t n)
{
    if (a >= 0 && a + 3 < n) return *reinterpret_cast<const r4_t *>(x + a);
    r4_t v = {0, 0, 0, 0};
    if (a >= 0 && a < n) v.x = x[a];
    if (a + 1 >= 0 && a + 1 < n) v.y = x[a + 1];
    if (a + 2 >= 0 && a + 2 < n) v.z = x[a + 2];
    if (a + 3 >= 0 && a + 3 < n) v.w = x[a + 3];
    return v;
}
template <int MODE, bool NL>
__device__ __forceinline__ void tridiag_quad_quotients(const r4_t &L, const r4_t &Cc, const r4_t &R, const real_t (&ev)[4], real_t (&q)[12])
{
    const real_t xv[8] = {L.z, L.w, Cc.x, Cc.y, Cc.z, Cc.w, R.x, R.y};
#pragma unroll
    for (int o = 0; o < 4; ++o) {
        const real_t e = ev[o];
        const real_t ed = MODE == 1 ? 2 * e : e;
        real_t p[5], m[5];
#pragma unroll
        for (int k = 0; k < 5; ++k) { const real_t dlt = k == 2 ? e : (real_t)0; p[k] = xv[o + k] + dlt; m[k] = xv[o + k] - dlt; }
#pragma unroll
        for (int k = 0; k < 3; ++k) {
            const real_t plus = tridiag_row<real_t, NL>(p[k], p[k + 1], p[k + 2]);
            const real_t sub = MODE == 1 ? tridiag_row<real_t, NL>(m[k], m[k + 1], m[k + 2])
                                         : tridiag_row<real_t, NL>(xv[o + k], xv[o + k + 1], xv[o + k + 2]);
            q[3 * o + k] = sub_exact(plus, sub) / ed;
        }
    }
}
template <int MODE, bool NL>
__global__ void __launch_bounds__(kBlock)
k_f_tridiag_store_wave4(const real_t *__restrict__ x, const real_t *__restrict__ eps, int64_t n, fd_band_store bst, int64_t jstart)
{
    __shared__ __attribute__((aligned(16))) real_t s_win[kBlock / 64][FD_BAND_WAVE4_LDS(3)];
    const int lane = threadIdx.x & 63, wave = threadIdx.x >> 6;
    const int64_t nwaves = (bst.col_end - jstart + 255) / 256;
    const int64_t gw = (int64_t)blockIdx.x * (kBlock / 64) + wave;
    if (gw >= nwaves) return;
    const int64_t jw = jstart + gw * 256;
    const int64_t j = jw + 4 * lane;
    const r4_t Cc = ld_quad_guarded(x, j, n), L = ld_quad_guarded(x, j - 4, n), R = ld_quad_guarded(x, j + 4, n);
    const int c0w = (int)((jw + bst.shift) % bst.C);
    int cc = (int)((uint32_t)(c0w + 4 * lane) % (uint32_t)bst.C);
    real_t ev[4];
#pragma unroll
    for (int o = 0; o < 4; ++o) { ev[o] = eps[cc]; cc = cc + 1 == bst.C ? 0 : cc + 1; }
    real_t q[12];
    tridiag_quad_quotients<MODE, NL>(L, Cc, R, ev, q);
    fd_band_emit_wave4<real_t, 3, true>(&bst, s_win[wave], jw, q);
}
template <int MODE, bool NL, int NC, bool PIPE>
__global__ void __launch_bounds__(kBlock)
k_f_tridiag_fused4(const real_t *__restrict__ x, int64_t n, fd_band_store bst, int64_t jstart, FusedEps fz)
{
    constexpr int kWinBytes = (kBlock / 64) * FD_BAND_WAVE4_LDS(3) * (int)sizeof(real_t);
    constexpr int kLdsBytes = kWinBytes + 64 > (kFzMaxBlocks + 2 * kEpsGroups) * 8 ? kWinBytes + 64 : (kFzMaxBlocks + 2 * kEpsGroups) * 8;
    __shared__ __attribute__((aligned(16))) char s_lds[kLdsBytes];
    real_t (*s_win)[FD_BAND_WAVE4_LDS(3)] = reinterpret_cast<real_t (*)[FD_BAND_WAVE4_LDS(3)]>(s_lds);
    double *s_red = reinterpret_cast<double *>(s_lds);
    const int b = (int)blockIdx.x, nfin = fz.eg.C;
    if (b < nfin) { fused_finisher(fz, b, s_red, x, n); return; }
    if (b < nfin + fz.nblocks) { fused_eps_block<NC, PIPE>(x, n, fz, b - nfin, reinterpret_cast<double (*)[NC]>(s_red)); return; }
    const int lane = threadIdx.x & 63, wave = threadIdx.x >> 6;
    const int cb = b - nfin - fz.nblocks;
    const int64_t nwaves = (bst.col_end - jstart + 255) / 256;
    const int64_t gstride = (int64_t)((int)gridDim.x - nfin - fz.nblocks) * (kBlock / 64);
    int64_t gw = (int64_t)cb * (kBlock / 64) + wave;
    int64_t jw = jstart + gw * 256;
    r4_t Cc = {0, 0, 0, 0}, L = {0, 0, 0, 0}, R = {0, 0, 0, 0};
    auto load_x = [&](int64_t jt, r4_t &c_, r4_t &l_, r4_t &r_) {
        const int64_t j = jt + 4 * lane;
        c_ = ld_quad_guarded(x, j, n); l_ = ld_quad_guarded(x, j - 4, n); r_ = ld_quad_guarded(x, j + 4, n);
        if (fz.xw && fz.nranks > 1) {
            if (j == fz.own_begin && fz.rank > 0) { l_.z = fused_halo(fz, 0, 0); l_.w = fused_halo(fz, 0, 1); }
            if (j + 4 == fz.own_end && fz.rank + 1 < fz.nranks) { r_.x = fused_halo(fz, 1, 0); r_.y = fused_halo(fz, 1, 1); }
        }
    };
    if (gw < nwaves) load_x(jw, Cc, L, R);
    real_t *s_eps = reinterpret_cast<real_t *>(s_lds + kWinBytes);
    if (wave == 0) fused_wait_eps(fz, cb, s_eps);
    __syncthreads();
    for (; gw < nwaves; gw += gstride) {
        const int c0w = (int)((jw + bst.shift) % bst.C);
        int c = (int)((uint32_t)(c0w + 4 * lane) % (uint32_t)bst.C);
        real_t ev[4];
#pragma unroll
        for (int o = 0; o < 4; ++o) { ev[o] = s_eps[c]; c = c + 1 == bst.C ? 0 : c + 1; }
        real_t q[12];
        tridiag_quad_quotients<MODE, NL>(L, Cc, R, ev, q);
        fd_band_emit_wave4<real_t, 3, true>(&bst, s_win[wave], jw, q);
        jw = jstart + (gw + gstride) * 256;
        if (gw + gstride < nwaves) load_x(jw, Cc, L, R);
    }
    if (fz.trace && (blockIdx.x & 31) < 2) { asm volatile("s_waitcnt vmcnt(0)" ::: "memory"); fz_mark_max(fz, 8); }
}
#endif

__device__ __forceinline__ int band_colptr32(int j, int l, int u, int M)
{
    const int w = l + u + 1;
    const int nt = j < u ? j : u;
    const int top = nt * u - nt * (nt - 1) / 2;
    const int b0 = M - l, f0 = b0 > 0 ? b0 : 0;
    int bot = 0;
    if (j > f0) { const int nn = j - f0, a = f0 - b0 + 1; bot = nn * a + nn * (nn - 1) / 2; }
    return w * j - top - bot;
}
template <typename CT, int MODE, bool NL, int BS>
__global__ void __launch_bounds__(BS)
k_f_tridiag_lazy_store(const real_t *__restrict__ x, const CT *__restrict__ color, const real_t *__restrict__ eps, int c_lo, int B,
                       int n, int r0, int r1, real_t *__restrict__ outp, int M, int N, int eb, int cb, int ce, int l, int u, int C,
                       int shift, int pitch, uint64_t mw, uint64_t mc)
{
    extern __shared__ real_t s_val[];
    real_t *s_ed = s_val + (size_t)B * pitch;
    const int R0 = r0 + (int)blockIdx.x * (2 * BS);
    if (R0 >= r1) return;
    const int R1 = R0 + 2 * BS < r1 ? R0 + 2 * BS : r1;
    const int w = l + u + 1, top_full = u * (u + 1) / 2;
    if ((int)threadIdx.x < B) {
        const real_t e = eps[c_lo + threadIdx.x];
        s_ed[threadIdx.x] = MODE == 1 ? 2 * e : e;
    }
    const int i = R0 + 2 * (int)threadIdx.x;
    if (i < R1) {
        real_t xv[4];
        int cv[4];
#pragma unroll
        for (int k = 0; k < 4; ++k) {
            const int j = i - 1 + k;
            const bool in = (j >= 0) & (j < n);
            xv[k] = in ? x[in ? j : 0] : 0.0;
            const int c = in ? (int)color[in ? j : 0] : -1;
            cv[k] = (c == (int)(CT)(-1) || c < 0) ? -1 : c - c_lo;
        }
        real_t b0 = 0.0, b1 = 0.0;
        if (MODE == 0) {
            b0 = tridiag_row<real_t, NL>(xv[0], xv[1], xv[2]);
            b1 = tridiag_row<real_t, NL>(xv[1], xv[2], xv[3]);
        }
        for (int b = 0; b < B; ++b) {
            const real_t e = eps[c_lo + b];
            real_t p[4], q[4];
#pragma unroll
            for (int k = 0; k < 4; ++k) { const real_t d = (cv[k] == b) ? e : 0.0; p[k] = xv[k] + d; q[k] = xv[k] - d; }
            const real_t s0 = MODE == 1 ? tridiag_row<real_t, NL>(q[0], q[1], q[2]) : b0;
            const real_t s1 = MODE == 1 ? tridiag_row<real_t, NL>(q[1], q[2], q[3]) : b1;
            *reinterpret_cast<r2_t *>(s_val + b * pitch + 2 * (int)threadIdx.x) =
                r2_t{sub_exact(tridiag_row<real_t, NL>(p[0], p[1], p[2]), s0), sub_exact(tridiag_row<real_t, NL>(p[1], p[2], p[3]), s1)};
        }
    }
    __syncthreads();
    const int jlo = R0 - l > cb ? R0 - l : cb, jhi = R1 - 1 + u < ce - 1 ? R1 - 1 + u : ce - 1;
    if (jhi < jlo) return;
    const int plo = (band_colptr32(jlo, l, u, M) - eb) & ~1, phi = band_colptr32(jhi + 1, l, u, M) - eb;
    const bool interior = jlo >= u && jhi + l <= M - 1;
    const bool vec = ((((uintptr_t)outp) & kPairMask) == 0);
    auto column_of = [&](int g) -> int {
        int j = (int)fd_div31((uint32_t)(g + top_full), mw);
        if (j >= N) j = N - 1;
        while (j > 0 && band_colptr32(j, l, u, M) > g) --j;
        while (j + 1 < N && band_colptr32(j + 1, l, u, M) <= g) ++j;
        return j;
    };
    for (int pp = plo + 2 * (int)threadIdx.x; pp < phi; pp += 2 * BS) {
        real_t qv[2];
        bool wr[2];
#pragma unroll
        for (int h = 0; h < 2; ++h) {
            const int g = pp + h + eb;
            int j, row;
            if (interior) {
                const uint32_t Q = (uint32_t)(g + top_full);
                const uint32_t jq = fd_div31(Q, mw);
                j = (int)jq;
                row = j - u + (int)(Q - jq * (uint32_t)w);
            } else {
                const int gg = g < phi + eb ? g : phi + eb - 1;
                j = column_of(gg);
                row = (j - u > 0 ? j - u : 0) + (gg - band_colptr32(j, l, u, M));
            }
            const uint32_t cj = (uint32_t)(j + shift);
            const int b = (int)(cj - fd_div31(cj, mc) * (uint32_t)C) - c_lo;
            const bool live = pp + h >= 0 && pp + h < phi && row >= R0 && row < R1 && b >= 0 && b < B && j >= cb && j < ce;
            const int at = live ? b * pitch + (row - R0) : 0;
            qv[h] = s_val[at] / s_ed[live ? b : 0];
            wr[h] = live;
        }
        if (wr[0] & wr[1] & vec) *reinterpret_cast<r2_t *>(outp + pp) = r2_t{qv[0], qv[1]};
        else {
            if (wr[0]) outp[pp] = qv[0];
            if (wr[1]) outp[pp + 1] = qv[1];
        }
    }
}

template <typename K>
static unsigned fused_grid(K kernel, unsigned tiles_wg, int prefix)
{
    static const int cus = [] { int dev = 0, n = 256; if (hipGetDevice(&dev) == hipSuccess) (void)hipDeviceGetAttribute(&n, hipDeviceAttributeMultiprocessorCount, dev); return n > 0 ? n : 256; }();
    static std::mutex mu;
    static std::unordered_map<const void *, int> per_cu;
    int occ = 0;
    {
        std::lock_guard<std::mutex> lock(mu);
        auto it = per_cu.find((const void *)kernel);
        if (it == per_cu.end()) {
            int nb = 0;
            if (hipOccupancyMaxActiveBlocksPerMultiprocessor(&nb, kernel, kBlock, 0) != hipSuccess || nb < 1) nb = 4;
            (void)hipGetLastError();
            it = per_cu.emplace((const void *)kernel, nb).first;
        }
        occ = it->second;
    }
    const int64_t room = (int64_t)cus * occ - prefix;
    const int64_t cap = room > cus ? room : cus;
    if ((int64_t)tiles_wg <= cap) return (unsigned)prefix + tiles_wg;
    const int64_t rounds = ((int64_t)tiles_wg + cap - 1) / cap;
    return (unsigned)prefix + (unsigned)(((int64_t)tiles_wg + rounds - 1) / rounds);
}

static bool tridiag_lines_jstart(const fd_band_store &bst, int64_t *jstart)
{
    if (sizeof(real_t) != 8 || bst.layout != FD_BAND_CSC) return false;
    const char *sw = fdjac::test_switch("FDJAC_STORE_LINES");
    if (sw && *sw && atoi(sw) == 0) return false;
    const uintptr_t o = (uintptr_t)bst.out;
    if (o & 7) return false;
    const int64_t r = (int64_t)(((uint64_t)bst.entry_begin - (uint64_t)(o >> 3)) & 15);
    const int64_t want = (11 * r) & 15;
    if (want & 1) return false;
    *jstart -= (*jstart - want) & 15;
    return true;
}

template <typename CT>
static int lazy_tridiag_launch(BuiltinF *b, void *fx, const fd_lazy_points *lp, int64_t fs, int64_t r0, int64_t r1,
                               hipStream_t s)
{
    const int64_t r0e = r0 & ~(int64_t)1;
    int64_t g = ((r1 - r0e + 1) / 2 + kBlock - 1) / kBlock;
    if (g < 1) g = 1;
    const bool nl = b->family == FD_F_TRIDIAG_NL;
    const int mode = lp->is_complex ? 2 : (lp->pts == 2 ? 1 : 0);
    const auto pick_store = [&](auto &&launch) {
        fd_pick<0, 1>(mode == 0 ? 0 : 1, [&](auto M) { fd_pick<false, true>(nl, [&](auto NL) { launch(M, NL); }); });
    };
    if (lp->store) {
        if (lp->store_kind != FD_STORE_BAND) return FD_LAZY_DECLINED;
        const fd_band_store bst = *(const fd_band_store *)lp->store;
        if (bst.elem_bytes != (int)sizeof(real_t) || mode == 2) return FD_LAZY_DECLINED;
        if (bst.N != b->prm[0] || bst.M != b->prm[0]) return FD_LAZY_DECLINED;
        const int wband = bst.l + bst.u + 1;
        const bool wave_ok = bst.l == 1 && bst.u == 1 && bst.M == bst.N && lp->c_lo == 0 &&
                             lp->ncolors == bst.C && bst.C >= 3 && (((uintptr_t)lp->x) & kPairMask) == 0 && bst.col_end > bst.col_begin;
#ifdef FDJAC_F32
        if (wave_ok && (((uintptr_t)lp->x) & 15) == 0) {
            const int64_t jstart = bst.col_begin & ~(int64_t)3;
            const int64_t nwaves = (bst.col_end - jstart + 255) / 256;
            const unsigned gw = (unsigned)((nwaves + kBlock / 64 - 1) / (kBlock / 64));
            if (lp->eps_job) {
                const FusedEps fz = *(const FusedEps *)lp->eps_job;
                pick_store([&](auto M, auto NL) {
                    fd_pick<4, kRegColors>(fz.eg.C <= 4 ? 4 : kRegColors, [&](auto NC) {
                        fd_pick<false, true>(fz.eg.tpb > 2, [&](auto PIPE) {
                            const auto k = k_f_tridiag_fused4<M(), NL(), NC(), PIPE()>;
                            hipLaunchKernelGGL(k, dim3(fused_grid(k, gw, fz.eg.C + fz.nblocks)), dim3(kBlock), 0, s, (const real_t *)lp->x,
                                               b->prm[0], bst, jstart, fz);
                        });
                    });
                });
                return launch_rc();
            }
            pick_store([&](auto M, auto NL) {
                hipLaunchKernelGGL((k_f_tridiag_store_wave4<M(), NL()>), dim3(gw), dim3(kBlock), 0, s, (const real_t *)lp->x,
                                   (const real_t *)lp->eps, b->prm[0], bst, jstart);
            });
            return launch_rc();
        }
#endif
        if (wave_ok) {
            int64_t jstart = bst.col_begin & ~(int64_t)1;
            const int lines = tridiag_lines_jstart(bst, &jstart) ? 1 : 0;
            const int64_t nwaves = (bst.col_end - jstart + 127) / 128;
            const unsigned gw = (unsigned)((nwaves + kBlock / 64 - 1) / (kBlock / 64));
            if (lp->eps_job) {
                const FusedEps fz = *(const FusedEps *)lp->eps_job;
                pick_store([&](auto M, auto NL) {
                    fd_pick<4, kRegColors>(fz.eg.C <= 4 ? 4 : kRegColors, [&](auto NC) {
                        fd_pick<false, true>(fz.eg.tpb > 2, [&](auto PIPE) {
                            const auto k = k_f_tridiag_fused<M(), NL(), NC(), PIPE()>;
                            hipLaunchKernelGGL(k, dim3(fused_grid(k, gw, fz.eg.C + fz.nblocks)), dim3(kBlock), 0, s, (const real_t *)lp->x,
                                               b->prm[0], bst, jstart, lines, fz);
                        });
                    });
                });
                return launch_rc();
            }
            pick_store([&](auto M, auto NL) {
                hipLaunchKernelGGL((k_f_tridiag_store_wave<M(), NL()>), dim3(gw), dim3(kBlock), 0, s, (const real_t *)lp->x,
                                   (const real_t *)lp->eps, b->prm[0], bst, jstart, lines);
            });
            return launch_rc();
        }
        if (lp->eps_job) return FD_LAZY_DECLINED;
        if (bst.layout != FD_BAND_CSC) return FD_LAZY_DECLINED;
        const int bs = kBlock;
        const int pitch = 2 * bs + 2;
        const size_t shm = sizeof(real_t) * ((size_t)lp->ncolors * (size_t)pitch + (size_t)lp->ncolors + 2);
        const int64_t nnz_all = fd_band_colptr(&bst, bst.N);
        if (shm > (size_t)60 * 1024 || nnz_all + (int64_t)wband * wband + 64 >= ((int64_t)1 << 31) || bst.N + bst.C + 64 >= ((int64_t)1 << 31) ||
            bst.M + wband + 64 >= ((int64_t)1 << 31) || lp->ncolors > kBlock) return FD_LAZY_DECLINED;
        const unsigned gs = (unsigned)((r1 - r0e + 2 * bs - 1) / (2 * bs));
        pick_store([&](auto M, auto NL) {
            hipLaunchKernelGGL((k_f_tridiag_lazy_store<CT, M(), NL(), kBlock>), dim3(gs), dim3(kBlock), shm, s, (const real_t *)lp->x,
                               (const CT *)lp->color, (const real_t *)lp->eps, lp->c_lo, lp->ncolors, (int)b->prm[0], (int)r0e, (int)r1,
                               (real_t *)bst.out, (int)bst.M, (int)bst.N, (int)bst.entry_begin, (int)bst.col_begin, (int)bst.col_end,
                               bst.l, bst.u, bst.C, bst.shift, pitch, fd_magic31((uint32_t)wband), fd_magic31((uint32_t)bst.C));
        });
        return launch_rc();
    }
    fd_pick<0, 1, 2>(mode, [&](auto M) {
        fd_pick<false, true>(nl, [&](auto NL) {
            hipLaunchKernelGGL((k_f_tridiag_lazy<CT, M(), NL()>), dim3((unsigned)g), dim3(kBlock), 0, s, (real_t *)fx, fs,
                               (real_t *)lp->base_out, (const real_t *)lp->x, (const CT *)lp->color, (const real_t *)lp->eps, lp->c_lo,
                               lp->ncolors, b->prm[0], r0e, r1, lp->imag_only, mode != 2 ? lp->diff : 0);
        });
    });
    return launch_rc();
}
```

### finitediff.jl_amd/csrc/fdjac_internal.h

```cpp
#pragma once
#include <hip/hip_runtime.h>

#ifdef FDJAC_F32
#define FDJAC_REAL float
#define fdjac fdjac32
#define fd_plan fd32_plan
#define fd_jvp_plan fd32_jvp_plan
#define fd_plan_create_csc fd32_plan_create_csc
#define fd_plan_create_csc_device fd32_plan_create_csc_device
#define fd_plan_checksum fd32_plan_checksum
#define fd_plan_create_csc_dense fd32_plan_create_csc_dense
#define fd_plan_create_coo_dense fd32_plan_create_coo_dense
#define fd_plan_create_entries fd32_plan_create_entries
#define fd_plan_create_dense fd32_plan_create_dense
#define fd_plan_create_tridiagonal fd32_plan_create_tridiagonal
#define fd_plan_create_banded fd32_plan_create_banded
#define fd_plan_create_blockbanded fd32_plan_create_blockbanded
#define fd_plan_create_bandedblockbanded fd32_plan_create_bandedblockbanded
#define fd_plan_destroy fd32_plan_destroy
#define fd_plan_matches fd32_plan_matches
#define fd_plan_matches_async fd32_plan_matches_async
#define fd_plan_stale fd32_plan_stale
#define fd_plan_info fd32_plan_info
#define fd_plan_row_lists fd32_plan_row_lists
// ... 292 lines not shown
        return m;
    }
    void release(M *m)
    {
        if (!m) return;
        std::lock_guard<std::mutex> lock(mutex);
        if (--m->refs > 0) return;
        map.erase(m->key);
        delete m;
    }
};

}

struct fd_fingerprint {
    bool valid = false;
    int idx_kind = 0;
    uint64_t h_a = 0, h_b = 0, h_color = 0;
    int64_t len_a = 0, len_b = 0, len_color = 0;
    int64_t a0 = 0, an = 0, b0 = 0, bn = 0;
};

struct fd_ctx {
    int device = 0;
    hipStream_t stream = nullptr;
    bool own_stream = false;
    int num_cus = 256;
    int *h_stale = nullptr, *d_stale = nullptr;
    hipStream_t check_stream = nullptr;
    hipEvent_t check_event = nullptr;
};

struct fd_plan {
    fd_ctx *ctx = nullptr;
    int kind = 0;
    int fdtype = 0;
    int64_t M = 0, N = 0;
    int64_t C = 0;
    bool color8 = true;
    int64_t col0 = 0, col1 = 0, x0 = 0, x1 = 0, row0 = 0, row1 = 0;
    int64_t own_c0 = 0, own_c1 = -1;
    bool tri_window = false;
    bool small_ok = true;
    bool eps_nt = true;
    int eps_tpg = 0, eps_bpg = 0, eps_tpb = 0;
    bool cx = false;
    int cyc_C = 0, cyc_shift = 0;

    void *d_color = nullptr;
    int32_t *d_rowval = nullptr;
    void *d_nzcolor = nullptr;
    int64_t *d_dest = nullptr;
    bool sorted_gather = false;
    uint16_t *d_spos = nullptr;
    bool has_none = false;
    bool built_on_device = false;
    double lines_direct = 0, lines_sorted = 0;
    bool window = false;
    int4 *d_wtiles = nullptr;
    int win_tile = 0;
    bool window2d = false;
    int *d_w2desc = nullptr;
    int64_t band_off = 0, band_C = 0;
    int band_w = 0, band_u = 0, band_shift = 0;
    uint64_t band_mw = 0, band_mc = 0;
    bool store_allowed = true, store_ok = false;
    int store_l = 0, store_u = 0, store_C = 0, store_shift = 0;
    bool store5_ok = false;
    int64_t store5_nx = 0, store5_ny = 0;
    bool want_store_csc = false, store_csc_always = false, store_csc_ok = false;
    int64_t bbb_nb = 0;
    int bbb_bl = 0, bbb_bu = 0, bbb_lam = 0, bbb_mu = 0;
    bool bbb_fill = false;
    bool store_bbb_ok = false;
    int64_t bbb_bs = 0;
    int32_t *d_bbb_off = nullptr;
    int32_t *d_bbb_blk = nullptr;
    int64_t *d_bbb_start = nullptr;
    int64_t *d_bbb_stride = nullptr;
    int32_t *d_sc_colptr = nullptr, *d_sc_rowval = nullptr;
    bool want_store_rows = false;
    int32_t *d_sr_ptr = nullptr, *d_sr_col = nullptr, *d_sr_slot = nullptr, *d_sr_order = nullptr, *d_sr_tile = nullptr;
    bool want_handover_rows = false;
    void *d_sr_color = nullptr;
    int se_tile_max = 0;
    int32_t *d_se_col = nullptr, *d_se_slot = nullptr, *d_se_info = nullptr;
    unsigned long long *d_sc_note = nullptr;
    unsigned long long sc_serial = 0;
    int64_t sc_entries = 0;
    int64_t sc_reach = -1;
    bool sc_valid = false;
    bool store_cr_ok = false;
    int64_t cr_nblk = 0, cr_bs = 0;
    int cr_bl = 0, cr_bu = 0;
    bool bd_allowed = true;
    int64_t bd_t0 = 0, bd_t1 = 0;
    int64_t w2_ntiles = 0;
    int64_t w2_codes = 0;
    uint16_t *d_wcode = nullptr;
    int win_pairs = 0;
    int win_ncol = 0;
    int win_per_P = 0, win_per_S = 0, win_per_magic = 0;
    double win_overread = 0;
    int64_t nnz_local = 0;
    int64_t entry_begin = 0;
    int64_t l = 0, u = 0;
    int32_t *d_cr_rlo = nullptr;
    int32_t *d_cr_cnt = nullptr;
    int64_t *d_cr_off = nullptr;
    bool cr_pairs = false;
    int32_t *d_perm = nullptr;
    int64_t *d_cptr = nullptr;
    int seg_chunks = 1;

    int64_t ldx = 0, ldf = 0;
    int64_t chunkB = 0, nchunks = 0;
    int pts = 1;
    int cplx = 0;
    fdjac::real_t *d_X = nullptr, *d_FX = nullptr, *d_fx = nullptr, *d_eps = nullptr;
    int32_t *d_fxwin = nullptr;
    int32_t *d_tile_order = nullptr;
    double *d_partial = nullptr;
    double *d_gsum = nullptr;
    unsigned *d_tick = nullptr;
    int64_t halo = 0, halo_own0 = 0, halo_own1 = 0;
    fdjac::real_t *d_xstage = nullptr, *d_finstage = nullptr;
    int n_partial_blocks = 0;
    int64_t scratch_bytes = 0;

    int nouts = 1;
    int64_t out_len[3] = {0, 0, 0};
    int split_n = 0;
    int64_t split_len[3] = {0, 0, 0};
    fdjac::real_t *d_split = nullptr;
    fdjac::real_t *d_outstage[3] = {nullptr, nullptr, nullptr};

    const fdjac::real_t *fx_batch_row = nullptr;
    fd_f_launch_lazy lazy_fn = nullptr;
    int lazy_caps = 0;
    bool lazy_diff = true;
    fdjac::real_t *d_zero_own = nullptr;
    const fdjac::real_t *d_zero = nullptr;
    fdjac::real_t *d_eps2 = nullptr;
    bool eps2_fresh = false;
    double *d_fz_part = nullptr;
    void *d_fz_eps = nullptr;
    int *h_fz_err = nullptr, *d_fz_err = nullptr;
    unsigned fz_parity = 0;
    long long *d_fz_trace = nullptr;
    bool fz_sharded_ok = true;
    bool fz_flags_ok = true;
    bool fz_shared_ok = false;
    int64_t fz_max_n = (int64_t)1 << 21;
    fd_comm *comm = nullptr;
    fd_p2p *p2p = nullptr;
    int eps_mode = 0;
    int64_t partial_cap = 0;
    int64_t fcalls_last = 0;
    int store_launch = 0;
    double relstep_last = 0, absstep_last = 0;

    fd_fingerprint fp;
    unsigned long long *d_fp = nullptr;
    unsigned long long *d_fpx = nullptr;
    int *h_pstale = nullptr, *d_pstale = nullptr;

    int timing = 0;
    int timing_stride = 1;
    int64_t timing_calls = 0;
    std::vector<fdjac::TimedSpan> spans;
    std::vector<hipEvent_t> event_pool;
    double ms_sum[FD_NSTAGES] = {};
    int64_t launches[FD_NSTAGES] = {};
    std::vector<float> samples[FD_NSTAGES];
};

struct fd_jvp_plan {
    fd_ctx *ctx = nullptr;
    int fdtype = 0;
    int64_t M = 0, N = 0, ldx = 0, ldf = 0;
    fdjac::real_t *d_X = nullptr, *d_FX = nullptr, *d_fx = nullptr, *d_eps = nullptr;
    double *d_partial = nullptr;
    fdjac::real_t *d_xs = nullptr, *d_vs = nullptr, *d_fin = nullptr, *d_out = nullptr;
    int nparts = 1;
    bool small_ok = true;
    fd_f_launch_lazy_jvp lazy_fn = nullptr;
    int lazy_caps = 0;
    bool lazy_diff = true;
};

namespace fdjac {
struct JvpHooks {
    bool have_partials;
    bool fin_is_base;
    void *user;
    int (*close)(void *user, const real_t *a, const real_t *b, const real_t *eps, int central);
};
int jvp_enqueue_hooked(fd_jvp_plan *p, fd_f_launch f, void *fctx, const real_t *x, const real_t *v, const real_t *f_in, double relstep,
                       double absstep, double dir, real_t *out, const JvpHooks *hk);
}

namespace fdjac {
int plan_record_fingerprint(fd_plan *p, int idx_kind, const fd_pattern_arrays *src, int64_t col0, int64_t col1);
}

static inline bool store_csc_active(const fd_plan *p)
{
    return p->lazy_fn && (p->lazy_caps & FD_LAZY_CAP_STORE_CSC) && p->store_csc_ok && p->kind == fdjac::K_CSC &&
           (p->fdtype != FD_COMPLEX || (p->lazy_caps & FD_LAZY_CAP_STORE_CSC_COMPLEX)) && p->store_allowed;
}
static inline bool handover_rows_active(const fd_plan *p)
{
    return p->want_handover_rows && p->kind == fdjac::K_CSC && p->d_sr_color && p->d_sr_order && p->d_sr_tile && p->d_sr_ptr && p->d_sr_slot;
}
static inline bool store_active(const fd_plan *p)
{
    if (!(p->lazy_fn && (p->lazy_caps & FD_LAZY_CAP_STORE)) || p->has_none) return false;
    if (p->kind == fdjac::K_COLRANGE) return p->store_cr_ok && (p->fdtype == FD_COMPLEX || (p->lazy_caps & FD_LAZY_CAP_STORE_COLRANGE) != 0);
    if (p->kind == fdjac::K_BBB) return p->store_bbb_ok && p->fdtype != FD_COMPLEX && p->store_allowed && p->nchunks == 1 && p->own_c0 == 0 &&
                                        (p->own_c1 < 0 || p->own_c1 >= p->C);
    return (p->store_ok || (p->store5_ok && p->kind == fdjac::K_CSC)) && p->fdtype != FD_COMPLEX &&
           (p->kind == fdjac::K_CSC || p->kind == fdjac::K_BANDED || p->kind == fdjac::K_TRIDIAG);
}

struct PbTimer {
    bool on;
    hipStream_t s;
    double t0;
    static double now() { struct timespec ts; clock_gettime(CLOCK_MONOTONIC, &ts); return ts.tv_sec * 1e3 + ts.tv_nsec * 1e-6; }
    PbTimer(hipStream_t st) : s(st) { const char *v = getenv("FDJAC_PLAN_TIMING"); on = v && *v && atoi(v) != 0; t0 = on ? now() : 0; }
    void mark(const char *what) { if (!on) return; (void)hipStreamSynchronize(s); const double t = now(); fprintf(stderr, "[fdjac plan] %-28s %8.3f ms\n", what, t - t0); t0 = t; }
};
```

### finitediff.jl_amd/lib.py

```python
import ctypes as C
import os
import subprocess

_HERE = os.path.dirname(os.path.abspath(__file__))
SO_PATH = os.path.join(_HERE, "lib", "libfdjac.so")
CSRC = os.path.join(_HERE, "csrc")

FD_OK = 0
FD_ERR_COMM = 8
COMM_ID_BYTES = 128
P2P_HANDLE_BYTES = 64
EPS_COMPUTE, EPS_PRECOMPUTED = 0, 1
TRI_DIAGONALS, TRI_CSC = 0, 1
FORWARD, CENTRAL, COMPLEX = 0, 1, 2
HESS_DENSE, HESS_CSC, HESS_BANDED = 0, 1, 2
HESS_INFO_NNZ, HESS_INFO_BANDWIDTH, HESS_INFO_UPPER, HESS_INFO_LIST_LEN, HESS_INFO_OUT_LEN = range(5)
HOST, DEVICE = 0, 1
FDTYPES = {"forward": FORWARD, "central": CENTRAL, "complex": COMPLEX}
STAGES = ("eps", "perturb", "f", "decompress", "total", "exchange")
(INFO_M, INFO_N, INFO_NCOLORS, INFO_NOUTS, INFO_OUT0_LEN, INFO_OUT1_LEN, INFO_OUT2_LEN, INFO_ROW_BEGIN,
 INFO_ROW_END, INFO_NCHUNKS, INFO_SCRATCH_BYTES, INFO_NNZ_LOCAL, INFO_FCALLS_LAST, INFO_ENTRY_BEGIN,
 INFO_SORTED_GATHER, INFO_LINES_DIRECT_X100, INFO_LINES_SORTED_X100, INFO_WINDOW,
 INFO_WIN_OVERREAD_X100, INFO_WINDOW2D, INFO_WIN_PERIOD, INFO_COLRANGE_WG, INFO_SMALL_FUSED, _INFO_23,
 INFO_EPS_CYCLIC, INFO_EPS_NT, _INFO_26, INFO_BUILT_ON_DEVICE, _INFO_28, INFO_LAZY_DIFF, _INFO_30, INFO_BAND_DESC, INFO_LAZY_STORE, INFO_STORE_CSC, INFO_STORE_LAUNCH, INFO_HANDOVER_ROWS) = range(36)
STORE_LAUNCH_NONE, STORE_LAUNCH_COLS, STORE_LAUNCH_COLS_WIN, STORE_LAUNCH_ROWS, STORE_LAUNCH_ENTS, STORE_LAUNCH_FAMILY = range(6)
LAZY_CAP_IMAG_ONLY, LAZY_CAP_ROW_WINDOW, LAZY_CAP_DIFF, LAZY_CAP_STORE, LAZY_CAP_STORE_CSC, LAZY_CAP_STORE_CSC_BASE, LAZY_CAP_STORE_CSC_COMPLEX, LAZY_CAP_FUSED_EPS, LAZY_CAP_STORE_COLRANGE = 1, 2, 4, 8, 16, 32, 64, 128, 256
PLAN_EPS_CONTIGUOUS, PLAN_COMPLEX_X, PLAN_FINGERPRINT, PLAN_STORE_CSC, PLAN_STORE_CSC_ALWAYS, PLAN_STORE_CSC_ROWS = 1, 2, 4, 8, 16, 32
PLAN_HANDOVER_ROWS = 64
LAZY_JVP_CAP_QUOTIENT = 1
(F_TRIDIAG, F_TRIDIAG_NL, F_LAP5, F_CLAMP5, F_BLOCKCOUPLED, F_NONSQUARE, F_LAP5_NL, F_LAP7, F_SPARSE) = range(9)
FAMILIES = {"tridiag": F_TRIDIAG, "tridiag_nl": F_TRIDIAG_NL, "lap5": F_LAP5, "clamp5": F_CLAMP5,
            "blockcoupled": F_BLOCKCOUPLED, "nonsquare": F_NONSQUARE, "lap5_nl": F_LAP5_NL, "lap7": F_LAP7}

F_LAUNCH = C.CFUNCTYPE(C.c_int, C.c_void_p, C.c_void_p, C.c_void_p, C.c_int64, C.c_int64, C.c_int64, C.c_int64,
                       C.c_int64, C.c_int, C.c_void_p)

class LazyPoints(C.Structure):
    _fields_ = [("x", C.c_void_p), ("color", C.c_void_p), ("eps", C.c_void_p), ("base_out", C.c_void_p),
                ("color_bytes", C.c_int32), ("c_lo", C.c_int32), ("ncolors", C.c_int32), ("pts", C.c_int32),
                ("is_complex", C.c_int32), ("imag_only", C.c_int32), ("part", C.c_int32), ("nparts", C.c_int32),
                ("diff", C.c_int32), ("store_kind", C.c_int32), ("store", C.c_void_p), ("eps_job", C.c_void_p)]


F_LAUNCH_LAZY = C.CFUNCTYPE(C.c_int, C.c_void_p, C.c_void_p, C.POINTER(LazyPoints), C.c_int64, C.c_int64, C.c_int64,
                            C.c_void_p)

class LazyJvpPoints(C.Structure):
    _fields_ = [("x", C.c_void_p), ("v", C.c_void_p), ("eps", C.c_void_p), ("base_out", C.c_void_p), ("central", C.c_int),
                ("reserved0", C.c_int), ("quotient_out", C.c_void_p)]


F_LAUNCH_LAZY_JVP = C.CFUNCTYPE(C.c_int, C.c_void_p, C.c_void_p, C.POINTER(LazyJvpPoints), C.c_int64, C.c_void_p)

EXPORTS = (
    "fd_version", "fd_last_error", "fd_ctx_create", "fd_ctx_destroy", "fd_ctx_stream", "fd_ctx_synchronize",
    "fd_plan_create_csc", "fd_plan_create_csc_dense", "fd_plan_create_coo_dense", "fd_plan_create_entries",
    "fd_plan_create_dense", "fd_plan_create_tridiagonal", "fd_plan_create_banded", "fd_plan_create_blockbanded",
    "fd_plan_create_bandedblockbanded", "fd_plan_destroy",
    "fd_plan_info", "fd_jacobian", "fd_jacobian_async", "fd_jacobian_owned_async", "fd_plan_get_epsilons", "fd_plan_fused_trace", "fd_plan_enable_timing", "fd_plan_set_timing_stride",
    "fd_plan_get_timings", "fd_builtin_f_create", "fd_builtin_f_destroy", "fd_builtin_f_counts", "fd_builtin_f_info",
    "fd_stream_copy_gbps", "fd_plan_set_lazy_f", "fd_builtin_f_lazy", "fd_plan_set_lazy_caps", "fd_builtin_f_lazy_caps",
    "fd_jvp_plan_create", "fd_jvp_plan_destroy", "fd_jvp", "fd_jvp_async", "fd_jvp_get_epsilon",
    "fd_jvp_plan_set_lazy_f", "fd_builtin_f_lazy_jvp", "fd_jvp_plan_set_lazy_caps", "fd_builtin_f_lazy_jvp_caps",
    "fd_color_columns_greedy", "fd_color_banded", "fd_color_columns_device", "fd_color_check_device",
    "fd_comm_unique_id", "fd_comm_create", "fd_comm_destroy", "fd_comm_info", "fd_comm_library", "fd_comm_allgather",
    "fd_comm_gatherv", "fd_comm_allreduce_sum", "fd_comm_broadcast", "fd_comm_halo_exchange", "fd_comm_enable_p2p", "fd_comm_p2p_status", "fd_comm_disable_p2p", "fd_f_compile_rows", "fd_f_link_rows_bitcode", "fd_f_compiled_destroy", "fd_f_compiled_counts", "fd_f_compile_log", "fd_f_compile_terms", "fd_f_compiled_row_stores", "fd_plan_row_lists",
    "fd_p2p_create", "fd_p2p_create_loopback", "fd_p2p_loopback_fill", "fd_p2p_loopback_fill_fused", "fd_p2p_local_handle", "fd_p2p_connect", "fd_p2p_destroy", "fd_p2p_info", "fd_p2p_status", "fd_p2p_allgather",
    "fd_p2p_halo_exchange",
    "fd_plan_set_comm", "fd_plan_set_p2p", "fd_plan_set_halo", "fd_plan_eps_partials", "fd_plan_eps_finalize", "fd_plan_set_eps_mode",
    "fd_tridiag_solver_create", "fd_tridiag_solver_destroy", "fd_tridiag_solve_async", "fd_tridiag_solve_interface",
    "fd_tridiag_solve_finish", "fd_plan_create_csc_device", "fd_plan_checksum", "fd_plan_get_timing_samples",
    "fd_plan_eps_shard_range", "fd_plan_matches", "fd_plan_matches_async", "fd_plan_stale", "fd_builtin_f_create_sparse", "fd_tridiag_solver_status", "fd_tridiag_solver_set_policy", "fd_tridiag_solver_set_pivoting",
    "fd_banded_solver_create", "fd_banded_solver_destroy", "fd_banded_solver_set_policy", "fd_banded_solver_status", "fd_banded_solve_async",
    "fd_blocktridiag_solver_create", "fd_blocktridiag_solver_destroy", "fd_blocktridiag_solver_set_policy", "fd_blocktridiag_solver_status",
    "fd_blocktridiag_solve_async",
    "fd_csc_solver_create", "fd_csc_solver_destroy", "fd_csc_matvec_async", "fd_csc_solver_set_options", "fd_csc_solver_set_policy", "fd_csc_solve_async", "fd_csc_solve_from_async", "fd_csc_solver_status", "fd_csc_solver_row_lists",
    "fd_csc_solver_set_preconditioner", "fd_csc_solver_block_inverses", "fd_csc_solver_set_block_ilu", "fd_csc_solver_ilu_levels", "fd_csc_solver_ilu_factors", "fd_csc_solver_set_method", "fd_csc_solver_gmres_basis",
    "fd_csc_solver_factor_async", "fd_csc_solver_apply_async", "fd_csc_solver_factor_status",
    "fd_csc_lsq_create", "fd_csc_lsq_destroy", "fd_csc_lsq_matvec_async", "fd_csc_lsq_set_options", "fd_csc_lsq_set_policy", "fd_csc_lsq_solve_async", "fd_csc_lsq_status", "fd_csc_lsq_row_lists", "fd_csc_lsq_long_columns",
    "fd_csc_tr_create", "fd_csc_tr_destroy", "fd_csc_tr_set_options", "fd_csc_tr_set_policy", "fd_csc_tr_matvec_async", "fd_csc_tr_step_async", "fd_csc_tr_status",
    "fd_jfnk_solver_create", "fd_jfnk_solver_destroy", "fd_jfnk_solver_set_options", "fd_jfnk_solver_set_policy", "fd_jfnk_solver_set_steps", "fd_jfnk_solver_set_lazy_f",
    "fd_jfnk_solver_set_diagonal", "fd_jfnk_solver_set_csc_preconditioner", "fd_jfnk_apply_async", "fd_jfnk_solve_async", "fd_jfnk_solve_from_async", "fd_jfnk_solver_status", "fd_jfnk_solver_counts", "fd_jfnk_solver_basis",
    "fd_jftr_create", "fd_jftr_destroy", "fd_jftr_set_options", "fd_jftr_set_policy", "fd_jftr_set_steps", "fd_jftr_set_lazy_f", "fd_jftr_set_diagonal",
    "fd_jftr_apply_async", "fd_jftr_step_async", "fd_jftr_status", "fd_jftr_counts",
    "fd_objective_compile", "fd_objective_destroy", "fd_objective_counts", "fd_hess_plan_create", "fd_hess_plan_destroy",
    "fd_hess_plan_info", "fd_hess_plan_pattern", "fd_hessian_async", "fd_hessian", "fd_gradient_async", "fd_gradient",
)


TYPED = (
    "fd_plan_create_csc", "fd_plan_create_csc_dense", "fd_plan_create_coo_dense", "fd_plan_create_entries",
    "fd_plan_create_dense", "fd_plan_create_tridiagonal", "fd_plan_create_banded", "fd_plan_create_blockbanded",
    "fd_plan_create_bandedblockbanded", "fd_plan_destroy", "fd_plan_info", "fd_plan_row_lists", "fd_jacobian", "fd_jacobian_async", "fd_jacobian_owned_async", "fd_plan_set_lazy_f", "fd_plan_set_lazy_caps",
    "fd_plan_get_epsilons", "fd_plan_fused_trace", "fd_plan_enable_timing", "fd_plan_set_timing_stride", "fd_plan_get_timings", "fd_builtin_f_create", "fd_builtin_f_destroy",
    "fd_builtin_f_counts", "fd_builtin_f_info", "fd_builtin_f_lazy", "fd_builtin_f_lazy_caps", "fd_jvp_plan_create", "fd_jvp_plan_destroy",
    "fd_jvp", "fd_jvp_async", "fd_jvp_get_epsilon", "fd_jvp_plan_set_lazy_f", "fd_builtin_f_lazy_jvp",
    "fd_jvp_plan_set_lazy_caps", "fd_builtin_f_lazy_jvp_caps",
    "fd_plan_set_comm", "fd_plan_set_p2p", "fd_plan_set_halo", "fd_plan_eps_partials", "fd_plan_eps_finalize", "fd_plan_set_eps_mode",
    "fd_tridiag_solver_create", "fd_tridiag_solver_destroy", "fd_tridiag_solve_async", "fd_tridiag_solve_interface",
    "fd_tridiag_solve_finish", "fd_plan_create_csc_device", "fd_plan_checksum", "fd_plan_get_timing_samples",
    "fd_plan_eps_shard_range", "fd_plan_matches", "fd_plan_matches_async", "fd_plan_stale", "fd_builtin_f_create_sparse", "fd_tridiag_solver_status", "fd_tridiag_solver_set_policy", "fd_tridiag_solver_set_pivoting",
    "fd_banded_solver_create", "fd_banded_solver_destroy", "fd_banded_solver_set_policy", "fd_banded_solver_status", "fd_banded_solve_async",
    "fd_blocktridiag_solver_create", "fd_blocktridiag_solver_destroy", "fd_blocktridiag_solver_set_policy", "fd_blocktridiag_solver_status",
    "fd_blocktridiag_solve_async",
    "fd_csc_solver_create", "fd_csc_solver_destroy", "fd_csc_matvec_async", "fd_csc_solver_set_options", "fd_csc_solver_set_policy", "fd_csc_solve_async", "fd_csc_solve_from_async", "fd_csc_solver_status", "fd_csc_solver_row_lists",
    "fd_csc_solver_set_preconditioner", "fd_csc_solver_block_inverses", "fd_csc_solver_set_block_ilu", "fd_csc_solver_ilu_levels", "fd_csc_solver_ilu_factors", "fd_csc_solver_set_method", "fd_csc_solver_gmres_basis",
    "fd_csc_solver_factor_async", "fd_csc_solver_apply_async", "fd_csc_solver_factor_status",
    "fd_csc_lsq_create", "fd_csc_lsq_destroy", "fd_csc_lsq_matvec_async", "fd_csc_lsq_set_options", "fd_csc_lsq_set_policy", "fd_csc_lsq_solve_async", "fd_csc_lsq_status", "fd_csc_lsq_row_lists", "fd_csc_lsq_long_columns",
)
EXPORTS = EXPORTS + tuple("fd32_" + n[3:] for n in TYPED)


class TypedLib:

    def __init__(self, L, f32):
        self._L, self._f32 = L, bool(f32)

    def __getattr__(self, name):
        if self._f32 and name in TYPED:
            return getattr(self._L, "fd32_" + name[3:])
        return getattr(self._L, name)


def typed(L, dtype):
    import numpy as np
    return TypedLib(L, np.dtype(dtype) == np.float32)


class PlanOpts(C.Structure):
    _fields_ = [("fdtype", C.c_int32), ("flags", C.c_int32), ("col_begin", C.c_int64), ("col_end", C.c_int64),
                ("x_begin", C.c_int64), ("x_end", C.c_int64), ("scratch_bytes", C.c_int64),
                ("color_begin", C.c_int64), ("color_end", C.c_int64)]


class PatternArrays(C.Structure):
    _fields_ = [("idx_a", C.c_void_p), ("len_a", C.c_int64), ("idx_b", C.c_void_p), ("len_b", C.c_int64),
                ("colorvec", C.c_void_p), ("len_color", C.c_int64), ("idx_bytes", C.c_int32), ("idx_base", C.c_int32),
                ("color_bytes", C.c_int32), ("memkind", C.c_int32)]


class FdError(RuntimeError):
    def __init__(self, code, msg):
        super().__init__("libfdjac error %d: %s" % (code, msg))
        self.code = code


def build(force=False):
    args = ["make", "-C", CSRC, "-s", "-j4"]
    if force:
        subprocess.check_call(["make", "-C", CSRC, "-s", "clean"])
    subprocess.check_call(args)
    return SO_PATH


_lib = None


def load():
    global _lib
    if _lib is not None:
        return _lib
    if not os.path.exists(SO_PATH):
        raise FileNotFoundError(
            "%s is missing: build it with `make -C %s` (hipcc, gfx950). There is no CPU fallback." % (SO_PATH, CSRC))
    try:
        import torch
    except Exception:
        pass
    L = C.CDLL(SO_PATH)
    vp, i64, i32, dbl = C.c_void_p, C.c_int64, C.c_int, C.c_double
    pp = C.POINTER(C.c_void_p)
    L.fd_version.restype = i32
    L.fd_last_error.restype = C.c_char_p
    L.fd_ctx_create.argtypes = [i32, vp, pp]
    L.fd_ctx_destroy.argtypes = [vp]
    L.fd_ctx_stream.argtypes = [vp]
    L.fd_ctx_stream.restype = vp
# ... 192 lines not shown
```

### include/fdjac.h

```cpp
#ifndef FDJAC_H
#define FDJAC_H

#include <stddef.h>
#include <stdint.h>

#ifdef __cplusplus
extern "C" {
#endif

#define FDJAC_VERSION 500

typedef struct fd_ctx fd_ctx;
typedef struct fd_plan fd_plan;

enum fd_status {
    FD_OK = 0,
    FD_ERR_ARG = 1,
    FD_ERR_SHAPE = 2,
    FD_ERR_UNSUPPORTED = 3,
    FD_ERR_HIP = 4,
    FD_ERR_CALLBACK = 5,
    FD_ERR_NOMEM = 6,
    FD_ERR_NODEVICE = 7,
    FD_ERR_COMM = 8,
    FD_ERR_STALE = 9
};

enum fd_fdtype { FD_FORWARD = 0, FD_CENTRAL = 1, FD_COMPLEX = 2 };
enum fd_memkind { FD_HOST = 0, FD_DEVICE = 1 };

typedef int (*fd_f_launch)(void *fctx, void *fx, const void *x, int64_t nbatch, int64_t x_stride,
                           int64_t fx_stride, int64_t row_begin, int64_t row_end, int is_complex,
                           void *stream);

typedef struct fd_lazy_points {
    const void *x;
    const void *color;
    const void *eps;
    void *base_out;
    int32_t color_bytes;
    int32_t c_lo;
    int32_t ncolors;
    int32_t pts;
    int32_t is_complex;
    int32_t imag_only;
    int32_t part;
    int32_t nparts;
    int32_t diff;
    int32_t store_kind;
    const void *store;
    const void *eps_job;
} fd_lazy_points;
typedef int (*fd_f_launch_lazy)(void *fctx, void *fx, const fd_lazy_points *points, int64_t fx_stride,
                                int64_t row_begin, int64_t row_end, void *stream);
#define FD_LAZY_DECLINED 100

typedef struct fd_plan_opts {
    int32_t fdtype;
    int32_t flags;
    int64_t col_begin;
    int64_t col_end;
    int64_t x_begin;
    int64_t x_end;
    int64_t scratch_bytes;
    int64_t color_begin;
    int64_t color_end;
} fd_plan_opts;
#define FD_PLAN_EPS_CONTIGUOUS 1

#define FD_PLAN_COMPLEX_X 2

#define FD_PLAN_STORE_CSC 8
#define FD_PLAN_STORE_CSC_ALWAYS 16
#define FD_PLAN_STORE_CSC_ROWS 32
#define FD_PLAN_HANDOVER_ROWS 64
#define FD_PLAN_FINGERPRINT 4

#define FD_STREAM_DEFAULT ((void *)(uintptr_t)1)
int fd_ctx_create(int device, void *stream, fd_ctx **out);
int fd_ctx_destroy(fd_ctx *ctx);
void *fd_ctx_stream(fd_ctx *ctx);
int fd_ctx_synchronize(fd_ctx *ctx);
const char *fd_last_error(void);
int fd_version(void);

int fd_plan_create_csc(fd_ctx *ctx, int64_t M, int64_t N, const void *colptr, const void *rowval,
                       int idx_bytes, int idx_base, const void *colorvec, int color_bytes,
                       const fd_plan_opts *opts, fd_plan **out);
int fd_plan_create_csc_device(fd_ctx *ctx, int64_t M, int64_t N, const void *colptr_dev, const void *rowval_dev,
                              int idx_bytes, int idx_base, const void *colorvec_dev, int color_bytes,
                              const fd_plan_opts *opts, fd_plan **out);
int fd_plan_checksum(fd_plan *plan, uint64_t *checksum_out);
int fd_plan_create_csc_dense(fd_ctx *ctx, int64_t M, int64_t N, const void *colptr,
                             const void *rowval, int idx_bytes, int idx_base, const void *colorvec,
                             int color_bytes, const fd_plan_opts *opts, fd_plan **out);
int fd_plan_create_coo_dense(fd_ctx *ctx, int64_t M, int64_t N, const void *rows_index,
                             const void *cols_index, int64_t nnz, int idx_bytes, int idx_base,
                             const void *colorvec, int color_bytes, const fd_plan_opts *opts,
                             fd_plan **out);
int fd_plan_create_entries(fd_ctx *ctx, int64_t M, int64_t N, const void *rows_index,
                           const void *cols_index, const int64_t *dest, int64_t nnz,
                           int64_t out_len, int idx_bytes, int idx_base, const void *colorvec,
                           int color_bytes, const fd_plan_opts *opts, fd_plan **out);
int fd_plan_create_dense(fd_ctx *ctx, int64_t M, int64_t N, int64_t ncols, const fd_plan_opts *opts,
                         fd_plan **out);
int fd_plan_create_tridiagonal(fd_ctx *ctx, int64_t N, const void *colorvec, int color_bytes,
                               const fd_plan_opts *opts, fd_plan **out);
int fd_plan_create_banded(fd_ctx *ctx, int64_t M, int64_t N, int64_t l, int64_t u,
                          const void *colorvec, int color_bytes, const fd_plan_opts *opts,
                          fd_plan **out);
int fd_plan_create_blockbanded(fd_ctx *ctx, int64_t nblk, const void *blk_sizes, int64_t bl,
                               int64_t bu, const void *block_starts, const void *block_strides,
                               int idx_bytes, int idx_base, const void *colorvec, int color_bytes,
                               const fd_plan_opts *opts, fd_plan **out);
int fd_plan_create_bandedblockbanded(fd_ctx *ctx, int64_t nblk, const void *blk_sizes, int64_t bl, int64_t bu, int64_t lam, int64_t mu,
                                     const void *block_starts, const void *block_strides, int64_t data_len, int idx_bytes, int idx_base,
                                     const void *colorvec, int color_bytes, const fd_plan_opts *opts, fd_plan **out);
int fd_plan_destroy(fd_plan *plan);

typedef struct fd_pattern_arrays {
    const void *idx_a;
    int64_t len_a;
    const void *idx_b;
    int64_t len_b;
    const void *colorvec;
    int64_t len_color;
    int32_t idx_bytes;
    int32_t idx_base;
    int32_t color_bytes;
    int32_t memkind;
} fd_pattern_arrays;
int fd_plan_matches(fd_plan *plan, const fd_pattern_arrays *now, int *matches_out);
int fd_plan_matches_async(fd_plan *plan, const fd_pattern_arrays *now);
int fd_plan_stale(fd_plan *plan, int *stale_out);

enum fd_plan_info_key {
    FD_INFO_M = 0, FD_INFO_N = 1, FD_INFO_NCOLORS = 2, FD_INFO_NOUTS = 3,
    FD_INFO_OUT0_LEN = 4, FD_INFO_OUT1_LEN = 5, FD_INFO_OUT2_LEN = 6,
    FD_INFO_ROW_BEGIN = 7, FD_INFO_ROW_END = 8, FD_INFO_NCHUNKS = 9, FD_INFO_SCRATCH_BYTES = 10,
    FD_INFO_NNZ_LOCAL = 11, FD_INFO_FCALLS_LAST = 12, FD_INFO_ENTRY_BEGIN = 13,
    FD_INFO_SORTED_GATHER = 14,
    FD_INFO_LINES_DIRECT_X100 = 15,
    FD_INFO_LINES_SORTED_X100 = 16,
    FD_INFO_WINDOW = 17,
    FD_INFO_WIN_OVERREAD_X100 = 18,
    FD_INFO_WINDOW2D = 19,
    FD_INFO_WIN_PERIOD = 20,
    FD_INFO_COLRANGE_WG = 21,
    FD_INFO_SMALL_FUSED = 22,
    FD_INFO_EPS_CYCLIC = 24,
    FD_INFO_EPS_NT = 25,
    FD_INFO_BAND_DESC = 31,
    FD_INFO_LAZY_STORE = 32,
    FD_INFO_LAZY_DIFF = 29,
    FD_INFO_BUILT_ON_DEVICE = 27,
    FD_INFO_STORE_CSC = 33,
    FD_INFO_STORE_LAUNCH = 34,
    FD_INFO_HANDOVER_ROWS = 35
};
enum fd_store_launch {
    FD_STORE_LAUNCH_NONE = 0,
    FD_STORE_LAUNCH_COLS = 1,
    FD_STORE_LAUNCH_COLS_WIN = 2,
    FD_STORE_LAUNCH_ROWS = 3,
    FD_STORE_LAUNCH_ENTS = 4,
    FD_STORE_LAUNCH_FAMILY = 5
};
int fd_plan_info(const fd_plan *plan, int key, int64_t *value);
int fd_plan_row_lists(const fd_plan *plan, const void **row_ptr_dev, const void **row_col_dev, const void **row_slot_dev, int64_t *entries,
                      uint64_t *plan_serial);

int fd_jacobian(fd_plan *plan, fd_f_launch f, void *fctx, const void *x, int x_kind,
                const void *f_in, int f_in_kind, double relstep, double absstep, double dir,
                void *const *outs, int out_kind);
int fd_jacobian_async(fd_plan *plan, fd_f_launch f, void *fctx, const void *x, const void *f_in,
                      double relstep, double absstep, double dir, void *const *outs);

int fd_plan_set_lazy_f(fd_plan *plan, fd_f_launch_lazy lazy);
#define FD_LAZY_CAP_IMAG_ONLY 1
#define FD_LAZY_CAP_ROW_WINDOW 2
#define FD_LAZY_CAP_DIFF 4
#define FD_LAZY_CAP_STORE 8
#define FD_LAZY_CAP_STORE_CSC 16
#define FD_LAZY_CAP_STORE_CSC_BASE 32
#define FD_LAZY_CAP_STORE_CSC_COMPLEX 64
#define FD_LAZY_CAP_STORE_COLRANGE 256
#define FD_LAZY_CAP_FUSED_EPS 128
int fd_plan_set_lazy_caps(fd_plan *plan, int caps);

int fd_plan_get_epsilons(fd_plan *plan, double *eps_out);
int fd_plan_fused_trace(fd_plan *plan, long long *marks16);

enum fd_stage { FD_STAGE_EPS = 0, FD_STAGE_PERTURB = 1, FD_STAGE_F = 2, FD_STAGE_DECOMPRESS = 3,
                FD_STAGE_TOTAL = 4, FD_STAGE_EXCHANGE = 5 ,
                FD_NSTAGES = 6 };
int fd_plan_enable_timing(fd_plan *plan, int on);
int fd_plan_get_timings(fd_plan *plan, double *ms_sum , int64_t *launches );
int fd_plan_set_timing_stride(fd_plan *plan, int stride);
int fd_plan_get_timing_samples(fd_plan *plan, int stage, double *ms_out, int64_t cap, int64_t *n_out);

enum fd_builtin_family {
    FD_F_TRIDIAG = 0,
    FD_F_TRIDIAG_NL = 1,
    FD_F_LAP5 = 2,
    FD_F_CLAMP5 = 3,
    FD_F_BLOCKCOUPLED = 4,
    FD_F_NONSQUARE = 5,
    FD_F_LAP5_NL = 6,
    FD_F_LAP7 = 7,
    FD_F_SPARSE = 8
};
int fd_builtin_f_create(fd_ctx *ctx, int family, const int64_t *params, int nparams,
                        fd_f_launch *fn_out, void **fctx_out);
int fd_builtin_f_create_sparse(fd_ctx *ctx, int64_t M, int64_t N, const void *colptr, const void *rowval, int idx_bytes, int idx_base,
                               fd_f_launch *fn_out, void **fctx_out);
int fd_builtin_f_destroy(void *fctx);
int fd_builtin_f_counts(void *fctx, int64_t *launches, int64_t *points);
enum fd_builtin_f_info_key { FD_F_INFO_ROW_STORES = 1 };
int fd_builtin_f_info(void *fctx, int key, int64_t *value);
int fd_builtin_f_lazy(void *fctx, fd_f_launch_lazy *fn_out);
int fd_builtin_f_lazy_caps(void *fctx, int *caps_out);

typedef struct fd_jvp_plan fd_jvp_plan;
int fd_jvp_plan_create(fd_ctx *ctx, int64_t M, int64_t N, int fdtype, fd_jvp_plan **out);
int fd_jvp_plan_destroy(fd_jvp_plan *plan);
int fd_jvp(fd_jvp_plan *plan, fd_f_launch f, void *fctx, const void *x, const void *v, int xv_kind,
           const void *f_in, int f_in_kind, double relstep, double absstep, double dir, void *jvp_out,
           int out_kind);
int fd_jvp_async(fd_jvp_plan *plan, fd_f_launch f, void *fctx, const void *x, const void *v, const void *f_in,
                 double relstep, double absstep, double dir, void *jvp_out);
int fd_jvp_get_epsilon(fd_jvp_plan *plan, double *eps_out);

typedef struct fd_lazy_jvp_points {
    const void *x;
    const void *v;
    const void *eps;
    void *base_out;
    int central;
    int reserved0;
    void *quotient_out;
} fd_lazy_jvp_points;
typedef int (*fd_f_launch_lazy_jvp)(void *fctx, void *fx_out, const fd_lazy_jvp_points *pts, int64_t fx_stride,
                                    void *stream);
int fd_jvp_plan_set_lazy_f(fd_jvp_plan *plan, fd_f_launch_lazy_jvp lazy);
#define FD_LAZY_JVP_CAP_QUOTIENT 1
int fd_jvp_plan_set_lazy_caps(fd_jvp_plan *plan, int caps);
int fd_builtin_f_lazy_jvp_caps(void *fctx, int *caps_out);
int fd_builtin_f_lazy_jvp(void *fctx, fd_f_launch_lazy_jvp *fn_out);

int fd_color_columns_greedy(int64_t M, int64_t N, const void *colptr, const void *rowval, int idx_bytes,
                            int idx_base, int64_t *colorvec_out, int64_t *ncolors_out);
int fd_color_banded(int64_t N, int64_t l, int64_t u, int64_t *colorvec_out, int64_t *ncolors_out);
int fd_color_columns_device(fd_ctx *ctx, int64_t M, int64_t N, const void *colptr_dev, const void *rowval_dev, int idx_bytes,
                            int idx_base, void *colorvec_dev_out, int color_bytes, int64_t *ncolors_out);
int fd_color_check_device(fd_ctx *ctx, int64_t M, int64_t N, const void *colptr_dev, const void *rowval_dev, int idx_bytes,
                          int idx_base, const void *colorvec_dev, int color_bytes, int64_t *bad_rows_out);

typedef struct fd_comm fd_comm;
#define FD_COMM_ID_BYTES 128
int fd_comm_unique_id(void *id_out );
int fd_comm_create(fd_ctx *ctx, int nranks, int rank, const void *id, fd_comm **out);
int fd_comm_destroy(fd_comm *comm);
int fd_comm_info(const fd_comm *comm, int *nranks, int *rank, int *rccl_version);
const char *fd_comm_library(void);
int fd_comm_allgather(fd_comm *comm, void *buf, int64_t slot_elems, int elem_bytes);
int fd_comm_gatherv(fd_comm *comm, const void *send, int64_t send_elems, void *recv, const int64_t *counts,
                    const int64_t *displs, int elem_bytes, int root);
int fd_comm_allreduce_sum(fd_comm *comm, void *buf, int64_t n, int elem_bytes);
int fd_jacobian_owned_async(fd_plan *plan, fd_comm *comm, fd_f_launch f, void *fctx, const void *x, const void *f_in,
                            double relstep, double absstep, double dir, void *const *outs);
int fd_comm_broadcast(fd_comm *comm, void *buf, int64_t n, int elem_bytes, int root);
int fd_comm_halo_exchange(fd_comm *comm, void *buf, int64_t own_begin, int64_t own_end, int64_t halo, int elem_bytes);

typedef struct fd_p2p fd_p2p;
#define FD_P2P_HANDLE_BYTES 64
int fd_p2p_create(fd_ctx *ctx, int nranks, int rank, int64_t slot_bytes , fd_p2p **out);
int fd_p2p_local_handle(fd_p2p *p2p, void *handle_out );
int fd_p2p_connect(fd_p2p *p2p, const void *handles );
int fd_p2p_destroy(fd_p2p *p2p);
int fd_p2p_create_loopback(fd_ctx *ctx, int nranks, int rank, int64_t slot_bytes, fd_p2p **out);
int fd_p2p_loopback_fill(fd_p2p *p2p, int sender, int64_t offset, const void *data, int64_t bytes);
int fd_p2p_loopback_fill_fused(fd_p2p *p2p, const void *gsum64x8, const void *halo_lo, const void *halo_hi, int64_t halo_bytes);
int fd_p2p_info(const fd_p2p *p2p, int *nranks, int *rank, int64_t *slot_bytes, int *uncached);
int fd_p2p_status(const fd_p2p *p2p, int *timed_out_rank_plus_1);
int fd_p2p_allgather(fd_p2p *p2p, void *buf, int64_t bytes);
int fd_p2p_halo_exchange(fd_p2p *p2p, void *buf, int64_t own_begin, int64_t own_end, int64_t halo, int elem_bytes);
int fd_comm_enable_p2p(fd_comm *comm, int64_t slot_bytes);
int fd_comm_p2p_status(const fd_comm *comm, int *enabled, int *timed_out_rank_plus_1);
int fd_comm_disable_p2p(fd_comm *comm);

int fd_plan_set_comm(fd_plan *plan, fd_comm *comm);
int fd_plan_set_p2p(fd_plan *plan, fd_p2p *p2p);
int fd_plan_set_halo(fd_plan *plan, int64_t own_begin, int64_t own_end, int64_t halo);
enum fd_eps_mode { FD_EPS_COMPUTE = 0, FD_EPS_PRECOMPUTED = 1 };
int fd_plan_eps_partials(fd_plan *plan, const void *x_dev, int shard, int nshards, void **partials_out,
                         int64_t *slot_doubles_out);
int fd_plan_eps_finalize(fd_plan *plan, double relstep, double absstep, double dir);
int fd_plan_set_eps_mode(fd_plan *plan, int mode);
int fd_plan_eps_shard_range(fd_plan *plan, int shard, int nshards, int64_t *x_begin, int64_t *x_end);

typedef struct fd_tridiag_solver fd_tridiag_solver;
enum fd_tridiag_layout { FD_TRI_DIAGONALS = 0, FD_TRI_CSC = 1 };
int fd_tridiag_solver_create(fd_ctx *ctx, int64_t N, int64_t row_begin, int64_t row_end, int layout,
                             fd_tridiag_solver **out);
int fd_tridiag_solver_destroy(fd_tridiag_solver *solver);
int fd_tridiag_solver_set_policy(fd_tridiag_solver *solver, int trust_non_dominant);
int fd_tridiag_solver_status(fd_tridiag_solver *solver, int *flags_out);
int fd_tridiag_solver_set_pivoting(fd_tridiag_solver *solver, int on);
int fd_tridiag_solve_async(fd_tridiag_solver *solver, double alpha, double beta, const void *const *J, const void *b,
                           void *y, fd_comm *comm);
int fd_tridiag_solve_interface(fd_tridiag_solver *solver, double alpha, double beta, const void *const *J, const void *b,
                               void *packet_dev);
int fd_tridiag_solve_finish(fd_tridiag_solver *solver, double alpha, double beta, const void *const *J, const void *b,
                            const void *packets_dev, int rank, int nranks, void *y);

typedef struct fd_banded_solver fd_banded_solver;
enum fd_banded_solve_layout { FD_BAND_SOLVE_BANDED = 0, FD_BAND_SOLVE_CSC = 1 };
int fd_banded_solver_create(fd_ctx *ctx, int64_t N, int l, int u, int layout, fd_banded_solver **out);
int fd_banded_solver_destroy(fd_banded_solver *solver);
// ... 292 lines not shown
```

Before: 153.1 billion columns/s.

## Add read-once fused eps+tridiagonal kernel holding x tiles in registers across grid sync

Adds a read-once path for large forward tridiagonal Jacobians. Each block loads its slice of x once, keeping four tiles in registers and a fifth in LDS. It computes the per-colour norm partials, publishes them, waits for the global eps reduction, and then computes the quotients from the held values instead of reading x from HBM a second time. The path is enabled by default when N exceeds the old fused limit. This relies on all blocks being co-resident, so the launch is capped by an occupancy check and falls back to the flags path when declined. The cost is higher register and LDS pressure and a grid-wide wait.

Result: slower. 109.6 billion columns/s (-28.4%).

```diff
diff --git a/finitediff.jl_amd/csrc/fdjac_api.hip b/finitediff.jl_amd/csrc/fdjac_api.hip
--- a/finitediff.jl_amd/csrc/fdjac_api.hip
+++ b/finitediff.jl_amd/csrc/fdjac_api.hip
@@ -151,6 +151,7 @@
     { const char *v = fdjac::test_switch("FDJAC_FUSED_MAX_N"); if (v && *v) p->fz_max_n = atoll(v); }
     p->fz_shared_ok = env_int("FDJAC_FUSED_SHARED", 0) != 0;
     p->fz_flags_ok = env_int("FDJAC_EPS_FLAGS", 1) != 0;
+    p->ro_mode = env_int("FDJAC_READONCE", 1);
     p->lazy_diff = env_int("FDJAC_LAZY_DIFF", 1) != 0;
     p->bd_allowed = env_int("FDJAC_BAND_DESC", 1) != 0;
     p->store_allowed = env_int("FDJAC_LAZY_STORE", 1) != 0;
@@ -481,6 +482,7 @@
         break;
     case FD_INFO_BUILT_ON_DEVICE: *value = p->built_on_device ? 1 : 0; break;
     case FD_INFO_HANDOVER_ROWS: *value = handover_rows_active(p) ? 1 : 0; break;
+    case FD_INFO_STEP_FORM: *value = p->step_form; break;
     default: set_error("unknown info key %d", key); return FD_ERR_ARG;
     }
     return FD_OK;
@@ -767,12 +769,15 @@
         fuse = fuse_sharded = fz_mb != nullptr && fzW > 1 && p->fz_sharded_ok && eps_shardable(p) && halo_ok &&
                               (int64_t)((kEpsGroups + fzW - 1) / fzW) * p->eps_tpg * 2048 <= p->fz_max_n &&
                               (!fdjac_p2p_shared_device(fz_mb) || p->fz_shared_ok);
-    } else if (fuse) {
-        fuse = p->N <= p->fz_max_n;
-    }
-    bool eps_flags = !fuse && p->fz_flags_ok && !small && !shard_ctx && p->fdtype != FD_COMPLEX && p->C > 0 && p->C <= kRegColors &&
+    }
+    const bool readonce = fuse && !shard_ctx && p->ro_mode != 0 && !p->ro_declined && p->fdtype == FD_FORWARD && !p->cx && p->col0 == 0 &&
+                          p->col1 == p->N && p->eps_tpb <= kRoTiles && p->n_partial_blocks == kEpsGroups * p->eps_bpg &&
+                          p->n_partial_blocks <= kFzMaxBlocks && (p->ro_mode >= 2 || (p->N > p->fz_max_n && sizeof(real_t) == 8));
+    if (fuse && !shard_ctx && !readonce) fuse = p->N <= p->fz_max_n;
+    const bool flags_able = p->fz_flags_ok && !small && !shard_ctx && p->fdtype != FD_COMPLEX && p->C > 0 && p->C <= kRegColors &&
                      p->kind != K_DENSE && p->eps_mode == FD_EPS_COMPUTE && p->d_partial != nullptr &&
                      p->n_partial_blocks == kEpsGroups * p->eps_bpg && p->n_partial_blocks <= kFzMaxBlocks;
+    bool eps_flags = !fuse && flags_able;
     if (eps_flags) {
         hipStreamCaptureStatus cs = hipStreamCaptureStatusNone;
         if (hipStreamIsCapturing(s, &cs) != hipSuccess) { (void)hipGetLastError(); cs = hipStreamCaptureStatusNone; }
@@ -808,11 +813,13 @@
         fz_job.err = fuse_sharded ? fdjac_p2p_err_word(fz_mb) : p->d_fz_err;
         fz_job.timeout_ticks = fused_timeout_ticks();
         fz_job.trace = p->d_fz_trace;
+        fz_job.readonce = readonce ? 1 : 0;
         if (p->d_fz_trace) {
             static const long long init[16] = {-1, 0, 0, 0, 0, -1, -1, 0, 0, 0, 0, 0, 0, 0, 0, 0};
             FD_HIP_CHECK(hipMemcpyAsync(p->d_fz_trace, init, sizeof init, hipMemcpyHostToDevice, s));
         }
     }
+    p->step_form = 0;
     if (p->eps_mode != FD_EPS_PRECOMPUTED) p->eps2_fresh = false;
     p->eps_nt = !(store_active(p) || store_csc_active(p));
     if (p->fdtype != FD_COMPLEX && p->C > 0 && p->eps_mode == FD_EPS_PRECOMPUTED) {
@@ -941,8 +948,19 @@
                 if (fuse_sharded) fdjac_p2p_fused_commit(fz_mb);
                 p->fz_parity ^= 1u;
                 p->eps2_fresh = p->d_eps2 != nullptr;
+                p->step_form = readonce ? FD_STEP_FORM_READONCE : FD_STEP_FORM_FUSED;
+            } else if (fuse && readonce && rc == FD_LAZY_DECLINED && flags_able) {
+                fuse = false;
+                p->ro_declined = true;
+                sp.stop();
+                { Span se(p, FD_STAGE_EPS); const int re = launch_eps_flags(p, x_dev, fz_job); if (re) return re; }
+                p->fz_parity ^= 1u;
+                Span sp2(p, FD_STAGE_DECOMPRESS);
+                lp.eps_job = nullptr;
+                rc = p->lazy_fn(fctx, p->d_FX, &lp, p->ldf, p->row0, p->row1, (void *)s);
             } else if (fuse) {
                 fuse = false;
+                if (readonce) p->ro_declined = true;
                 sp.stop();
                 { Span se(p, FD_STAGE_EPS); const int re = fuse_sharded ? eps_sharded_classic(p, x_dev, relstep, absstep, dir) : launch_eps(p, x_dev, relstep, absstep, dir); if (re) return re; }
                 Span sp2(p, FD_STAGE_DECOMPRESS);
diff --git a/finitediff.jl_amd/csrc/fdjac_eps_dev.h b/finitediff.jl_amd/csrc/fdjac_eps_dev.h
--- a/finitediff.jl_amd/csrc/fdjac_eps_dev.h
+++ b/finitediff.jl_amd/csrc/fdjac_eps_dev.h
@@ -49,81 +49,117 @@
     double relstep, absstep, dir;
 };
 
-template <typename CT, int NC, bool CYC, bool NT, bool PIPE = true>
-__device__ __forceinline__ bool eps_block_sum(const real_t *__restrict__ x, const CT *__restrict__ color, int64_t n, int cyc_C, int cyc_shift,
-                                              int gblock, const EpsGrid &eg, int pair, double (*red)[NC], double &s)
+__device__ __forceinline__ void eps_cyc_next(int &rc, int du, int cyc_C, int &c0, int &c1)
+{
+    c0 = rc;
+    c1 = rc + 1 == cyc_C ? 0 : rc + 1;
+    rc += du;
+    rc = rc >= cyc_C ? rc - cyc_C : rc;
+}
+
+template <typename CT, bool CYC, bool NT>
+__device__ __forceinline__ void eps_load_tile(const real_t *__restrict__ x, const CT *__restrict__ color, int64_t n, int64_t base, int cyc_C,
+                                              int &rc, int du, r2_t (&v)[kEpsU], int (&c0)[kEpsU], int (&c1)[kEpsU])
+{
+    const int64_t tile = (int64_t)kEpsU * kBlock * 2;
+    if (base + tile <= n) {
+#pragma unroll
+        for (int u = 0; u < kEpsU; ++u) {
+            const int64_t i = base + (int64_t)u * kBlock * 2 + threadIdx.x * 2;
+            if (CYC) eps_cyc_next(rc, du, cyc_C, c0[u], c1[u]);
+            const r2_t *pv = reinterpret_cast<const r2_t *>(x + i);
+            v[u] = NT ? __builtin_nontemporal_load(pv) : *pv;
+            if (!CYC) load_color_pair<CT>(color + i, c0[u], c1[u]);
+        }
+        return;
+    }
+#pragma unroll
+    for (int u = 0; u < kEpsU; ++u) {
+        const int64_t i = base + (int64_t)u * kBlock * 2 + threadIdx.x * 2;
+        if (CYC) eps_cyc_next(rc, du, cyc_C, c0[u], c1[u]);
+        if (i + 1 < n) {
+            if (NT) v[u] = __builtin_nontemporal_load(reinterpret_cast<const r2_t *>(x + i));
+            else v[u] = *reinterpret_cast<const r2_t *>(x + i);
+            if (!CYC) load_color_pair<CT>(color + i, c0[u], c1[u]);
+        } else if (i < n) {
+            v[u] = r2_t{x[i], 0.0};
+            if (!CYC) c0[u] = color[i];
+            c1[u] = -2;
+        } else {
+            v[u] = r2_t{0.0, 0.0};
+            c0[u] = c1[u] = -2;
+        }
+    }
+}
+
+template <int NC>
+__device__ __forceinline__ void eps_accumulate_tile(double (&acc)[NC], const r2_t (&v)[kEpsU], int (&c0)[kEpsU], int (&c1)[kEpsU], int pair)
+{
+#pragma unroll
+    for (int u = 0; u < kEpsU; ++u) {
+        if (pair) c1[u] = c0[u];
+        const double s0 = (double)v[u].x * (double)v[u].x, s1 = (double)v[u].y * (double)v[u].y;
+#pragma unroll
+        for (int c = 0; c < NC; ++c) {
+            acc[c] += (c0[u] == c) ? s0 : 0.0;
+            acc[c] += (c1[u] == c) ? s1 : 0.0;
+        }
+    }
+}
+
+template <int NC>
+__device__ __forceinline__ bool eps_block_tail(const double (&acc)[NC], double (*red)[NC], double &s)
+{
+    const int lane = threadIdx.x & 63, wave = threadIdx.x >> 6;
+#pragma unroll
+    for (int c = 0; c < NC; ++c) {
+        const double w = wave_sum(acc[c]);
+        if (lane == 0) red[wave][c] = w;
+    }
+    __syncthreads();
+    if (wave != 0) return false;
+    s = 0.0;
+    if (lane < NC) {
+#pragma unroll
+        for (int w = 0; w < kBlock / 64; ++w) s += red[w][lane];
+    }
+    return true;
+}
+
+__device__ __forceinline__ void eps_block_range(int gblock, const EpsGrid &eg, int64_t n, int64_t &base0, int64_t &base_end)
 {
     const int grp = gblock / eg.bpg, kb = gblock - grp * eg.bpg;
-    double acc[NC];
-#pragma unroll
-    for (int c = 0; c < NC; ++c) acc[c] = 0.0;
-
     const int64_t tile = (int64_t)kEpsU * kBlock * 2;
     const int64_t t0 = (int64_t)grp * eg.tpg + (int64_t)kb * eg.tpb;
     int64_t t1 = t0 + eg.tpb;
     if (t1 > (int64_t)(grp + 1) * eg.tpg) t1 = (int64_t)(grp + 1) * eg.tpg;
-    const int64_t base0 = t0 * tile;
-    int64_t base_end = t1 * tile;
+    base0 = t0 * tile;
+    base_end = t1 * tile;
     if (base_end > n) base_end = n;
+}
+
+template <typename CT, int NC, bool CYC, bool NT, bool PIPE = true>
+__device__ __forceinline__ bool eps_block_sum(const real_t *__restrict__ x, const CT *__restrict__ color, int64_t n, int cyc_C, int cyc_shift,
+                                              int gblock, const EpsGrid &eg, int pair, double (*red)[NC], double &s)
+{
+    double acc[NC];
+#pragma unroll
+    for (int c = 0; c < NC; ++c) acc[c] = 0.0;
+
+    const int64_t tile = (int64_t)kEpsU * kBlock * 2;
+    int64_t base0, base_end;
+    eps_block_range(gblock, eg, n, base0, base_end);
     int rc = 0, du = 0;
     if (CYC) {
         rc = (int)((base0 + threadIdx.x * 2 + cyc_shift) % cyc_C);
         du = (kBlock * 2) % cyc_C;
     }
     auto load_tile = [&](int64_t base, r2_t (&v)[kEpsU], int (&c0)[kEpsU], int (&c1)[kEpsU]) {
-        if (base + tile <= n) {
-#pragma unroll
-            for (int u = 0; u < kEpsU; ++u) {
-                const int64_t i = base + (int64_t)u * kBlock * 2 + threadIdx.x * 2;
-                if (CYC) {
-                    c0[u] = rc;
-                    c1[u] = rc + 1 == cyc_C ? 0 : rc + 1;
-                    rc += du;
-                    rc = rc >= cyc_C ? rc - cyc_C : rc;
-                }
-                const r2_t *pv = reinterpret_cast<const r2_t *>(x + i);
-                v[u] = NT ? __builtin_nontemporal_load(pv) : *pv;
-                if (!CYC) load_color_pair<CT>(color + i, c0[u], c1[u]);
-            }
-            return;
-        }
-#pragma unroll
-        for (int u = 0; u < kEpsU; ++u) {
-            const int64_t i = base + (int64_t)u * kBlock * 2 + threadIdx.x * 2;
-            if (CYC) {
-                c0[u] = rc;
-                c1[u] = rc + 1 == cyc_C ? 0 : rc + 1;
-                rc += du;
-                rc = rc >= cyc_C ? rc - cyc_C : rc;
-            }
-            if (i + 1 < n) {
-                if (NT) v[u] = __builtin_nontemporal_load(reinterpret_cast<const r2_t *>(x + i));
-                else v[u] = *reinterpret_cast<const r2_t *>(x + i);
-                if (!CYC) load_color_pair<CT>(color + i, c0[u], c1[u]);
-            } else if (i < n) {
-                v[u] = r2_t{x[i], 0.0};
-                if (!CYC) c0[u] = color[i];
-                c1[u] = -2;
-            } else {
-                v[u] = r2_t{0.0, 0.0};
-                c0[u] = c1[u] = -2;
-            }
-        }
+        eps_load_tile<CT, CYC, NT>(x, color, n, base, cyc_C, rc, du, v, c0, c1);
     };
     r2_t va[kEpsU], vb[kEpsU];
     int a0[kEpsU], a1[kEpsU], b0[kEpsU], b1[kEpsU];
-    auto accumulate = [&](const r2_t (&v)[kEpsU], int (&c0)[kEpsU], int (&c1)[kEpsU]) {
-#pragma unroll
-        for (int u = 0; u < kEpsU; ++u) {
-            if (pair) c1[u] = c0[u];
-            const double s0 = (double)v[u].x * (double)v[u].x, s1 = (double)v[u].y * (double)v[u].y;
-#pragma unroll
-            for (int c = 0; c < NC; ++c) {
-                acc[c] += (c0[u] == c) ? s0 : 0.0;
-                acc[c] += (c1[u] == c) ? s1 : 0.0;
-            }
-        }
-    };
+    auto accumulate = [&](const r2_t (&v)[kEpsU], int (&c0)[kEpsU], int (&c1)[kEpsU]) { eps_accumulate_tile<NC>(acc, v, c0, c1, pair); };
     if (!PIPE) {
         for (int64_t base = base0; base < base_end; base += tile) {
             load_tile(base, va, a0, a1);
@@ -140,21 +176,60 @@
         accumulate(vb, b0, b1);
     }
     }
-
-    const int lane = threadIdx.x & 63, wave = threadIdx.x >> 6;
-#pragma unroll
-    for (int c = 0; c < NC; ++c) {
-        const double w = wave_sum(acc[c]);
-        if (lane == 0) red[wave][c] = w;
-    }
-    __syncthreads();
-    if (wave != 0) return false;
-    s = 0.0;
-    if (lane < NC) {
-#pragma unroll
-        for (int w = 0; w < kBlock / 64; ++w) s += red[w][lane];
-    }
-    return true;
+    return eps_block_tail<NC>(acc, red, s);
+}
+
+constexpr int kRoTiles = 5, kRoRegTiles = 4;
+template <int NC, typename F>
+__device__ __forceinline__ bool eps_block_sum_keep(const real_t *__restrict__ x, int64_t n, int cyc_C, int cyc_shift, int64_t base0, int nt,
+                                                   double (*red)[NC], double &s, r2_t (&held)[kRoRegTiles][kEpsU], r2_t (*spill)[kBlock],
+                                                   F &&on_tile)
+{
+    double acc[NC];
+#pragma unroll
+    for (int c = 0; c < NC; ++c) acc[c] = 0.0;
+    const int64_t tile = (int64_t)kEpsU * kBlock * 2;
+    const int du = (kBlock * 2) % cyc_C;
+    int rc = (int)((base0 + threadIdx.x * 2 + cyc_shift) % cyc_C);
+    {
+        int rl = 0, d0[kEpsU], d1[kEpsU];
+        if (nt > kRoRegTiles) {
+            r2_t v[kEpsU];
+            eps_load_tile<uint8_t, true, false>(x, nullptr, n, base0 + kRoRegTiles * tile, cyc_C, rl, du, v, d0, d1);
+#pragma unroll
+            for (int u = 0; u < kEpsU; ++u) spill[u][threadIdx.x] = v[u];
+        }
+#pragma unroll
+        for (int k = 0; k < kRoRegTiles; ++k) {
+            if (k < nt) eps_load_tile<uint8_t, true, false>(x, nullptr, n, base0 + k * tile, cyc_C, rl, du, held[k], d0, d1);
+            else {
+#pragma unroll
+                for (int u = 0; u < kEpsU; ++u) held[k][u] = r2_t{0, 0};
+            }
+        }
+    }
+    auto add_tile = [&](int k, const r2_t (&v)[kEpsU]) {
+        int c0[kEpsU], c1[kEpsU];
+#pragma unroll
+        for (int u = 0; u < kEpsU; ++u) {
+            eps_cyc_next(rc, du, cyc_C, c0[u], c1[u]);
+            const int64_t i = base0 + k * tile + (int64_t)u * kBlock * 2 + threadIdx.x * 2;
+            if (i + 1 >= n) c1[u] = -2;
+            if (i >= n) c0[u] = -2;
+        }
+        eps_accumulate_tile<NC>(acc, v, c0, c1, 0);
+        on_tile(k, v);
+    };
+#pragma unroll
+    for (int k = 0; k < kRoRegTiles; ++k)
+        if (k < nt) add_tile(k, held[k]);
+    if (nt > kRoRegTiles) {
+        r2_t v[kEpsU];
+#pragma unroll
+        for (int u = 0; u < kEpsU; ++u) v[u] = spill[u][threadIdx.x];
+        add_tile(kRoRegTiles, v);
+    }
+    return eps_block_tail<NC>(acc, red, s);
 }
 
 constexpr int kFzReplicas = 64;
@@ -201,6 +276,7 @@
     real_t *xw;
     long long own_begin, own_end;
     int halo;
+    int readonce;
 };
 __device__ __forceinline__ char *fz_cells(char *mailbox, const FusedEps &fz, int buf) { return mailbox + fz.fz_off + (long long)buf * kFzBufBytes; }
 __device__ __forceinline__ void fz_mark_min(const FusedEps &fz, int k)
@@ -228,6 +304,13 @@
                  : "memory");
 }
 
+__device__ __forceinline__ void fused_publish_block(const FusedEps &fz, int gblock, double s)
+{
+    const int lane = threadIdx.x & 63;
+    if (lane < fz.eg.C) __hip_atomic_store(fz.part + (int64_t)lane * fz.nblocks + gblock, s, __ATOMIC_RELAXED, __HIP_MEMORY_SCOPE_AGENT);
+    fz_mark_max(fz, 1);
+}
+
 template <int NC, bool PIPE, typename CT = uint8_t, bool CYC = true, bool NT = false>
 __device__ __forceinline__ void fused_eps_block(const real_t *__restrict__ x, int64_t n, const FusedEps &fz, int gblock, double (*red)[NC],
                                                 const CT *__restrict__ color = nullptr)
@@ -235,9 +318,7 @@
     double s;
     if (threadIdx.x == 0) fz_mark_min(fz, 0);
     if (!eps_block_sum<CT, NC, CYC, NT, PIPE>(x, color, n, fz.cyc_C, fz.cyc_shift, fz.g0 * fz.eg.bpg + gblock, fz.eg, fz.pair, red, s)) return;
-    const int lane = threadIdx.x & 63;
-    if (lane < fz.eg.C) __hip_atomic_store(fz.part + (int64_t)lane * fz.nblocks + gblock, s, __ATOMIC_RELAXED, __HIP_MEMORY_SCOPE_AGENT);
-    fz_mark_max(fz, 1);
+    fused_publish_block(fz, gblock, s);
 }
 
 constexpr int kFzMaxBlocks = kEpsGroups * kEpsBlocksPerGroup;
diff --git a/finitediff.jl_amd/csrc/fdjac_f_tridiag.hip b/finitediff.jl_amd/csrc/fdjac_f_tridiag.hip
--- a/finitediff.jl_amd/csrc/fdjac_f_tridiag.hip
+++ b/finitediff.jl_amd/csrc/fdjac_f_tridiag.hip
@@ -136,6 +136,31 @@
     return (int)(m < 0 ? m + bst.C : m);
 }
 
+__device__ __forceinline__ void tridiag_wave_eps(const real_t *eps, int64_t jw, const fd_band_store &bst, int lines, real_t &ea, real_t &eb, real_t &en)
+{
+    const int lane = threadIdx.x & 63;
+    const int c0w = tridiag_wave_color(jw, bst);
+    const int c0 = (int)((uint32_t)(c0w + 2 * lane) % (uint32_t)bst.C);
+    const int c1 = c0 + 1 == bst.C ? 0 : c0 + 1;
+    ea = eps[c0];
+    eb = eps[c1];
+    en = lines ? eps[(uint32_t)(c0w + 128) % (uint32_t)bst.C] : (real_t)0;
+}
+template <int MODE, bool NL>
+__device__ __forceinline__ void tridiag_wave_store(const fd_band_store &bst, real_t *win, int64_t jw, int lines, const r2_t &L, const r2_t &Cc,
+                                                   const r2_t &R, real_t ea, real_t eb, real_t en)
+{
+    real_t q[6];
+    tridiag_pair_quotients<MODE, NL>(L, Cc, R, ea, eb, q);
+    if (lines) {
+        real_t qn = 0;
+        if ((threadIdx.x & 63) == 63) qn = tridiag_next_quotient<MODE, NL>(Cc, R, en);
+        fd_band_emit_wave_lines<real_t, true>(&bst, win, jw, q, qn);
+        return;
+    }
+    fd_band_emit_wave<real_t, 3, true>(&bst, win, jw, q);
+}
+
 template <int MODE, bool NL>
 __global__ void __launch_bounds__(kBlock)
 k_f_tridiag_store_wave(const real_t *__restrict__ x, const real_t *__restrict__ eps, int64_t n, fd_band_store bst, int64_t jstart, int lines)
@@ -148,20 +173,9 @@
     const int64_t jw = jstart + gw * 128;
     const int64_t j = jw + 2 * lane;
     const r2_t Cc = ld_pair_guarded(x, j, n), L = ld_pair_guarded(x, j - 2, n), R = ld_pair_guarded(x, j + 2, n);
-    const int c0w = tridiag_wave_color(jw, bst);
-    const int c0 = (int)((uint32_t)(c0w + 2 * lane) % (uint32_t)bst.C);
-    const int c1 = c0 + 1 == bst.C ? 0 : c0 + 1;
-    const real_t ea = eps[c0], eb = eps[c1];
-    const real_t en = lines ? eps[(uint32_t)(c0w + 128) % (uint32_t)bst.C] : (real_t)0;
-    real_t q[6];
-    tridiag_pair_quotients<MODE, NL>(L, Cc, R, ea, eb, q);
-    if (lines) {
-        real_t qn = 0;
-        if (lane == 63) qn = tridiag_next_quotient<MODE, NL>(Cc, R, en);
-        fd_band_emit_wave_lines<real_t, true>(&bst, s_win[wave], jw, q, qn);
-        return;
-    }
-    fd_band_emit_wave<real_t, 3, true>(&bst, s_win[wave], jw, q);
+    real_t ea, eb, en;
+    tridiag_wave_eps(eps, jw, bst, lines, ea, eb, en);
+    tridiag_wave_store<MODE, NL>(bst, s_win[wave], jw, lines, L, Cc, R, ea, eb, en);
 }
 
 template <int MODE, bool NL, int NC, bool PIPE>
@@ -196,22 +210,108 @@
     if (wave == 0) fused_wait_eps(fz, cb, s_eps);
     __syncthreads();
     for (; gw < nwaves; gw += gstride) {
-        const int c0w = tridiag_wave_color(jw, bst);
-        const int c0 = (int)((uint32_t)(c0w + 2 * lane) % (uint32_t)bst.C);
-        const int c1 = c0 + 1 == bst.C ? 0 : c0 + 1;
-        real_t q[6];
-        tridiag_pair_quotients<MODE, NL>(L, Cc, R, s_eps[c0], s_eps[c1], q);
-        if (lines) {
-            real_t qn = 0;
-            if (lane == 63) qn = tridiag_next_quotient<MODE, NL>(Cc, R, s_eps[(uint32_t)(c0w + 128) % (uint32_t)bst.C]);
-            fd_band_emit_wave_lines<real_t, true>(&bst, s_win[wave], jw, q, qn);
-        } else {
-            fd_band_emit_wave<real_t, 3, true>(&bst, s_win[wave], jw, q);
-        }
+        real_t ea, eb, en;
+        tridiag_wave_eps(s_eps, jw, bst, lines, ea, eb, en);
+        tridiag_wave_store<MODE, NL>(bst, s_win[wave], jw, lines, L, Cc, R, ea, eb, en);
         jw = jstart + (gw + gstride) * 128;
         if (gw + gstride < nwaves) load_x(jw, Cc, L, R);
     }
     if (fz.trace && (blockIdx.x & 31) < 2) { asm volatile("s_waitcnt vmcnt(0)" ::: "memory"); fz_mark_max(fz, 8); }
+}
+
+constexpr int kRoSpans = kRoTiles * kEpsU * (kBlock / 64);
+template <bool NL, int NC>
+__global__ void __launch_bounds__(kBlock, 4)
+k_f_tridiag_readonce(const real_t *__restrict__ x, int64_t n, fd_band_store bst, int lines, FusedEps fz)
+{
+    constexpr int kWinBytes = (kBlock / 64) * FD_BAND_WAVE_LDS(3) * (int)sizeof(real_t);
+    constexpr int kFinBytes = (kFzMaxBlocks + 2 * kEpsGroups + 2) * 8;
+    __shared__ __attribute__((aligned(16))) char s_lds[kWinBytes > kFinBytes ? kWinBytes : kFinBytes];
+    __shared__ __attribute__((aligned(16))) r2_t s_first[kRoSpans + 2], s_last[kRoSpans + 2];
+    __shared__ real_t s_eps[64];
+    __shared__ __attribute__((aligned(16))) r2_t s_tile[kEpsU][kBlock];
+    real_t (*s_win)[FD_BAND_WAVE_LDS(3)] = reinterpret_cast<real_t (*)[FD_BAND_WAVE_LDS(3)]>(s_lds);
+    double *s_red = reinterpret_cast<double *>(s_lds);
+    const int b = (int)blockIdx.x, lane = threadIdx.x & 63, wave = threadIdx.x >> 6;
+    const int64_t tile = (int64_t)kEpsU * kBlock * 2;
+    int64_t base0, base_end;
+    eps_block_range(b, fz.eg, n, base0, base_end);
+    const int nt = base0 < base_end ? (int)((base_end - base0 + tile - 1) / tile) : 0;
+    if (threadIdx.x == 0) fz_mark_min(fz, 0);
+    if (wave == 1) {
+        const int64_t a = lane == 0 ? base0 - 2 : base0 + nt * tile;
+        const bool in0 = a >= 0 && a < n, in1 = a >= 0 && a + 1 < n;
+        const real_t v0 = x[in0 ? a : 0], v1 = x[in1 ? a + 1 : 0];
+        const r2_t v = {in0 ? v0 : (real_t)0, in1 ? v1 : (real_t)0};
+        if (lane == 0) s_last[0] = v;
+        if (lane == 1) s_first[nt * (kRoSpans / kRoTiles) + 1] = v;
+    }
+    r2_t held[kRoRegTiles][kEpsU];
+    double s;
+    const bool w0 = eps_block_sum_keep<NC>(x, n, fz.cyc_C, fz.cyc_shift, base0, nt, reinterpret_cast<double (*)[NC]>(s_red), s, held, s_tile,
+                                           [&](int k, const r2_t (&v)[kEpsU]) {
+#pragma unroll
+                                               for (int u = 0; u < kEpsU; ++u) {
+                                                   const int sp = (k * kEpsU + u) * (kBlock / 64) + wave;
+                                                   if (lane == 0) s_first[sp + 1] = v[u];
+                                                   if (lane == 63) s_last[sp + 1] = v[u];
+                                               }
+                                           });
+    if (w0) fused_publish_block(fz, b, s);
+    if (b < fz.eg.C) fused_finisher(fz, b, s_red, x, n);
+    if (nt == 0) return;
+    if (wave == 0) fused_wait_eps(fz, b, s_eps);
+    __syncthreads();
+#pragma unroll 1
+    for (int k = 0; k < nt; ++k) {
+#pragma unroll
+        for (int u = 0; u < kEpsU; ++u) {
+            const int sp = (k * kEpsU + u) * (kBlock / 64) + wave;
+            const int64_t jw = base0 + (int64_t)sp * 128;
+            if (jw < bst.col_end) {
+                const r2_t Cc = held[0][u];
+                const r2_t eL = s_last[sp], eR = s_first[sp + 2];
+                r2_t L = {__shfl_up(Cc.x, 1, 64), __shfl_up(Cc.y, 1, 64)}, R = {__shfl_down(Cc.x, 1, 64), __shfl_down(Cc.y, 1, 64)};
+                if (lane == 0) L = eL;
+                if (lane == 63) R = eR;
+                real_t ea, eb, en;
+                tridiag_wave_eps(s_eps, jw, bst, lines, ea, eb, en);
+                tridiag_wave_store<0, NL>(bst, s_win[wave], jw, lines, L, Cc, R, ea, eb, en);
+            }
+        }
+#pragma unroll
+        for (int kk = 0; kk + 1 < kRoRegTiles; ++kk)
+#pragma unroll
+            for (int u = 0; u < kEpsU; ++u) held[kk][u] = held[kk + 1][u];
+        if (k + 1 == kRoRegTiles) {
+#pragma unroll
+            for (int u = 0; u < kEpsU; ++u) held[0][u] = s_tile[u][threadIdx.x];
+        }
+    }
+    if (fz.trace && (blockIdx.x & 31) < 2) { asm volatile("s_waitcnt vmcnt(0)" ::: "memory"); fz_mark_max(fz, 8); }
+}
+
+template <typename K>
+static int64_t readonce_capacity(K kernel)
+{
+    static std::mutex mu;
+    static std::map<std::pair<int, const void *>, int64_t> cap;
+    int dev = 0;
+    if (hipGetDevice(&dev) != hipSuccess) { (void)hipGetLastError(); return 0; }
+    std::lock_guard<std::mutex> lock(mu);
+    const auto key = std::make_pair(dev, (const void *)kernel);
+    auto it = cap.find(key);
+    if (it == cap.end()) {
+        int nb = 0, cus = 0;
+        if (hipOccupancyMaxActiveBlocksPerMultiprocessor(&nb, kernel, kBlock, 0) != hipSuccess || nb < 1) nb = 0;
+        if (hipDeviceGetAttribute(&cus, hipDeviceAttributeMultiprocessorCount, dev) != hipSuccess || cus < 1) cus = 0;
+        (void)hipGetLastError();
+        it = cap.emplace(key, (int64_t)(nb < 6 ? nb : 6) * cus).first;
+    }
+    int64_t c = it->second;
+    const char *sw = fdjac::test_switch("FDJAC_READONCE_WGS");
+    if (sw && *sw && atoll(sw) < c) c = atoll(sw);
+    return c;
 }
 
 #ifdef FDJAC_F32
@@ -472,6 +572,24 @@
         const int wband = bst.l + bst.u + 1;
         const bool wave_ok = bst.l == 1 && bst.u == 1 && bst.M == bst.N && lp->c_lo == 0 &&
                              lp->ncolors == bst.C && bst.C >= 3 && (((uintptr_t)lp->x) & kPairMask) == 0 && bst.col_end > bst.col_begin;
+        if (lp->eps_job && ((const FusedEps *)lp->eps_job)->readonce) {
+            const FusedEps fz = *(const FusedEps *)lp->eps_job;
+            if (!wave_ok || mode != 0 || bst.col_begin != 0 || bst.col_end != bst.N || fz.nranks != 1 || fz.pair || fz.eg.tpb > kRoTiles ||
+                fz.cyc_C != bst.C || fz.cyc_shift != bst.shift || fz.nblocks > kFzMaxBlocks)
+                return FD_LAZY_DECLINED;
+            int64_t jstart = 0;
+            const int lines = (tridiag_lines_jstart(bst, &jstart) && jstart == 0) ? 1 : 0;
+            int rc = FD_LAZY_DECLINED;
+            fd_pick<false, true>(nl, [&](auto NL) {
+                fd_pick<4, kRegColors>(fz.eg.C <= 4 ? 4 : kRegColors, [&](auto NC) {
+                    const auto k = k_f_tridiag_readonce<NL(), NC()>;
+                    if ((int64_t)fz.nblocks > readonce_capacity(k)) return;
+                    hipLaunchKernelGGL(k, dim3((unsigned)fz.nblocks), dim3(kBlock), 0, s, (const real_t *)lp->x, b->prm[0], bst, lines, fz);
+                    rc = launch_rc();
+                });
+            });
+            return rc;
+        }
 #ifdef FDJAC_F32
         if (wave_ok && (((uintptr_t)lp->x) & 15) == 0) {
             const int64_t jstart = bst.col_begin & ~(int64_t)3;
diff --git a/finitediff.jl_amd/csrc/fdjac_internal.h b/finitediff.jl_amd/csrc/fdjac_internal.h
--- a/finitediff.jl_amd/csrc/fdjac_internal.h
+++ b/finitediff.jl_amd/csrc/fdjac_internal.h
@@ -468,6 +468,9 @@
     bool fz_flags_ok = true;
     bool fz_shared_ok = false;
     int64_t fz_max_n = (int64_t)1 << 21;
+    int ro_mode = 1;
+    bool ro_declined = false;
+    int step_form = 0;
     fd_comm *comm = nullptr;
     fd_p2p *p2p = nullptr;
     int eps_mode = 0;
diff --git a/finitediff.jl_amd/lib.py b/finitediff.jl_amd/lib.py
--- a/finitediff.jl_amd/lib.py
+++ b/finitediff.jl_amd/lib.py
@@ -22,7 +22,8 @@
  INFO_ROW_END, INFO_NCHUNKS, INFO_SCRATCH_BYTES, INFO_NNZ_LOCAL, INFO_FCALLS_LAST, INFO_ENTRY_BEGIN,
  INFO_SORTED_GATHER, INFO_LINES_DIRECT_X100, INFO_LINES_SORTED_X100, INFO_WINDOW,
  INFO_WIN_OVERREAD_X100, INFO_WINDOW2D, INFO_WIN_PERIOD, INFO_COLRANGE_WG, INFO_SMALL_FUSED, _INFO_23,
- INFO_EPS_CYCLIC, INFO_EPS_NT, _INFO_26, INFO_BUILT_ON_DEVICE, _INFO_28, INFO_LAZY_DIFF, _INFO_30, INFO_BAND_DESC, INFO_LAZY_STORE, INFO_STORE_CSC, INFO_STORE_LAUNCH, INFO_HANDOVER_ROWS) = range(36)
+ INFO_EPS_CYCLIC, INFO_EPS_NT, _INFO_26, INFO_BUILT_ON_DEVICE, _INFO_28, INFO_LAZY_DIFF, INFO_STEP_FORM, INFO_BAND_DESC, INFO_LAZY_STORE, INFO_STORE_CSC, INFO_STORE_LAUNCH, INFO_HANDOVER_ROWS) = range(36)
+STEP_FORM_SEPARATE, STEP_FORM_FUSED, STEP_FORM_READONCE = range(3)
 STORE_LAUNCH_NONE, STORE_LAUNCH_COLS, STORE_LAUNCH_COLS_WIN, STORE_LAUNCH_ROWS, STORE_LAUNCH_ENTS, STORE_LAUNCH_FAMILY = range(6)
 LAZY_CAP_IMAG_ONLY, LAZY_CAP_ROW_WINDOW, LAZY_CAP_DIFF, LAZY_CAP_STORE, LAZY_CAP_STORE_CSC, LAZY_CAP_STORE_CSC_BASE, LAZY_CAP_STORE_CSC_COMPLEX, LAZY_CAP_FUSED_EPS, LAZY_CAP_STORE_COLRANGE = 1, 2, 4, 8, 16, 32, 64, 128, 256
 PLAN_EPS_CONTIGUOUS, PLAN_COMPLEX_X, PLAN_FINGERPRINT, PLAN_STORE_CSC, PLAN_STORE_CSC_ALWAYS, PLAN_STORE_CSC_ROWS = 1, 2, 4, 8, 16, 32
diff --git a/include/fdjac.h b/include/fdjac.h
--- a/include/fdjac.h
+++ b/include/fdjac.h
@@ -156,6 +156,7 @@
     FD_INFO_BUILT_ON_DEVICE = 27,
     FD_INFO_STORE_CSC = 33,
     FD_INFO_STORE_LAUNCH = 34,
+    FD_INFO_STEP_FORM = 30,
     FD_INFO_HANDOVER_ROWS = 35
 };
 enum fd_store_launch {
@@ -165,6 +166,11 @@
     FD_STORE_LAUNCH_ROWS = 3,
     FD_STORE_LAUNCH_ENTS = 4,
     FD_STORE_LAUNCH_FAMILY = 5
+};
+enum fd_step_form {
+    FD_STEP_FORM_SEPARATE = 0,
+    FD_STEP_FORM_FUSED = 1,
+    FD_STEP_FORM_READONCE = 2
 };
 int fd_plan_info(const fd_plan *plan, int key, int64_t *value);
 int fd_plan_row_lists(const fd_plan *plan, const void **row_ptr_dev, const void **row_col_dev, const void **row_slot_dev, int64_t *entries,
```
